# krlong014/PySolvers

Hardware: AMD Instinct MI355X
Metric: CG iterations/sec + SpMV GB/s vs HBM roofline, 5-pt Laplacian N=10M (higher is better)
Workload: dtype f64

## Files before the change

### include/psk_lab.h

```cpp
#ifndef PSK_LAB_H
#define PSK_LAB_H

#include "psk.h"

#ifdef __cplusplus
extern "C" {
#endif

int psk_lab_occupy_begin(int32_t wgs, int32_t lds_bytes, double seconds);
int psk_lab_occupy_end(int32_t *timed_out);
int psk_lab_dispatch_probe(int32_t nwg, int32_t lds_bytes, double usec, int64_t *rec_out);
int psk_lab_occupy_xcc(int32_t *counts);
int psk_lab_trisolve_workers(const psk_prec *M, int32_t which, int32_t *enrolled, int32_t *grid);
int psk_lab_trisolve_plan(int64_t n, const int32_t *rowptr, const int32_t *colidx, const double *vals, int32_t upper,
                          int32_t unit, const int32_t *nat, int32_t num_cus, int64_t syncfree_waves, int32_t *schedule,
                          double *est, int64_t *info);
int psk_lab_dist_plan(int64_t n_global, const int64_t *row_starts, int32_t P, int32_t rank, const int64_t *rowptr,
                      const int32_t *colidx, int32_t *lcol, int64_t *halo, int64_t *nhalo, int32_t *pack, int64_t *npack,
                      int64_t *peers, int32_t *npeers);
int psk_lab_amg_gs_pair(psk_prec *M, int32_t set, int32_t *levels_on, int32_t *levels_eligible);
int psk_lab_spmv_rotate(const psk_csr *A, const double *const *xs, double *const *ys, int32_t nbuf, int32_t reps,
                        int32_t dot, double *avg_ms);
int psk_lab_spmv_after_write(const psk_csr *A, double *x, double *y, const double *src, double *scratch,
                             int32_t target, int32_t reps, int32_t dot, double *avg_ms);
int psk_lab_cheby_ab(const psk_prec *M, const double *v, int32_t reps, double *fused_ms, double *pieces_ms);
int psk_lab_pcg_stagger(int32_t *blocks, int32_t *ring);
int psk_lab_pcg_staggers(const psk_csr *A, const psk_prec *M, int32_t *on);
int psk_lab_pcg_flush_schedule(int32_t S, int64_t nv, int64_t tile, int64_t k, int32_t in_spmv, int32_t *blk,
                               int64_t *first_last);
int psk_lab_pcg_flush(int64_t n, int64_t k, int32_t stag, double *x, const double *ring, const double *alphas);
#define PSK_LAB_SOLVER_PCG 0
#define PSK_LAB_SOLVER_GMRES 1
#define PSK_LAB_SOLVER_VCYCLE 2
#define PSK_LAB_SOLVER_BICGSTAB 3
#define PSK_LAB_SOLVER_MINRES 5
#define PSK_LAB_SOLVER_PCG_MULTI 6
#define PSK_LAB_LAYOUT_GEN 1
#define PSK_LAB_LAYOUT_OWN_X 2
#define PSK_LAB_LAYOUT_DEV_IO 4
int psk_lab_solver_layout(int32_t solver, int64_t n, int64_t ncols, int64_t maxiter, int64_t restart, int32_t flags,
                          int32_t P, int64_t *offsets, int32_t *count, int64_t *bytes);
int psk_lab_gmres_internals(const psk_csr *A, int64_t maxiter, int32_t restart, int32_t gen, int32_t cols, double *Q,
                            double *H, double *R, double *CS, double *g, double *y, double *state);
int psk_lab_gmres_prefill(psk_csr *A, int64_t maxiter, int32_t restart, int32_t gen, int32_t byte);
int psk_lab_pcg_internals(const psk_csr *A, int64_t maxiter, int32_t gen, int32_t own_x, double *r, double *ring,
                          double *Ap, double *u, double *x, double *alphas, double *udr, double *hist, double *sums,
                          double *state);
int psk_lab_pcg_prefill(psk_csr *A, int64_t maxiter, int32_t gen, int32_t own_x, int32_t byte);
int psk_lab_pcg_multi_internals(const psk_csr *A, int64_t maxiter, int32_t nrhs, double *alphas, double *udr, double *pap,
                                double *r, double *p, double *Ap, double *x, double *state);
int psk_lab_ilu0_timing(double *out);
int psk_lab_iluk_timing(double *out);
#ifdef __cplusplus
}
#endif

#endif
```

### pysolvers_amd/_native.py

```python
import atexit
import ctypes
import os
import sys

import numpy as np

_HERE = os.path.dirname(os.path.abspath(__file__))
LIB_PATH = os.environ.get("PSK_LIBRARY", os.path.join(_HERE, "_lib", "libpsk.so"))

PSK_OK = 0
PSK_ERR_ARG, PSK_ERR_HIP, PSK_ERR_RCCL, PSK_ERR_ALLOC, PSK_ERR_UNSUPPORTED = -1, -2, -3, -4, -5
ABI_VERSION = 4
PSK_CONVERGED, PSK_MAXITER, PSK_BREAKDOWN, PSK_TRUE_RESID_FAIL = 0, 1, 2, 3
PSK_EXIT_NONE, PSK_EXIT_TOLERANCE, PSK_EXIT_ARNOLDI_BREAKDOWN, PSK_EXIT_MAXITER, PSK_EXIT_DOT_BREAKDOWN = 0, 1, 2, 3, 4
PSK_HOST, PSK_DEVICE = 0, 1
PSK_VCYCLE_X0_GIVEN = 1
PSK_PREC_IDENTITY, PSK_PREC_JACOBI, PSK_PREC_ILU, PSK_PREC_AMG, PSK_PREC_DENSE, PSK_PREC_CHEBYSHEV = 0, 1, 2, 3, 4, 5
PSK_PREC_FSAI = 6
PSK_FSAI_ROW_CAP = 64
PSK_FSAI_WAVE_ONLY = 1
PSK_PREC_MCGS = 7
PSK_MCGS_MAX_COLORS = 64
PSK_MCGS_SYMMETRIC = 1
PSK_LAYOUT_CSR, PSK_LAYOUT_SLICED, PSK_LAYOUT_SLICED_WIDE, PSK_LAYOUT_SLICED_DICT, PSK_LAYOUT_DIAG = 0, 1, 2, 3, 4
# ... 45 lines not shown
    "psk_csr_download": (ctypes.c_int, [P, P, P, P]),
    "psk_csr_destroy": (ctypes.c_int, [P]),
    "psk_spmv": (ctypes.c_int, [P, P, P, I32]),
    "psk_spmv_timed": (ctypes.c_int, [P, P, P, I32, ctypes.POINTER(F64)]),
    "psk_dot": (ctypes.c_int, [I64, P, P, I32, ctypes.POINTER(F64)]),
    "psk_nrm2": (ctypes.c_int, [I64, P, I32, ctypes.POINTER(F64)]),
    "psk_axpy": (ctypes.c_int, [I64, F64, P, P, I32]),
    "psk_prec_create": (ctypes.c_int, [P, I32, PP]),
    "psk_prec_apply": (ctypes.c_int, [P, I64, P, P, I32]),
    "psk_prec_jacobi_uniform": (ctypes.c_int, [P, ctypes.POINTER(I32), ctypes.POINTER(ctypes.c_double)]),
    "psk_prec_create_ilu": (ctypes.c_int, [I64, P, P, P, P, P, P, P, P, PP]),
    "psk_prec_destroy": (ctypes.c_int, [P]),
    "psk_prec_create_trisolve": (ctypes.c_int, [I64, P, P, P, I32, P, P, P, I32, P, P, PP]),
    "psk_prec_create_amg": (ctypes.c_int, [I32, PP, PP, PP, PP, P, I32, I32, I32, F64, PP]),
    "psk_prec_create_dense_inverse": (ctypes.c_int, [P, I32, PP]),
    "psk_prec_create_chebyshev": (ctypes.c_int, [P, I32, F64, F64, PP]),
    "psk_prec_chebyshev_info": (ctypes.c_int, [P, ctypes.POINTER(I32), ctypes.POINTER(F64), ctypes.POINTER(F64), P]),
    "psk_prec_trisolve_schedule": (ctypes.c_int, [P, I32, I32, ctypes.POINTER(I32), ctypes.POINTER(I64),
                                                   ctypes.POINTER(I32), ctypes.POINTER(F64), ctypes.POINTER(F64)]),
    "psk_prec_trisolve_grid_info": (ctypes.c_int, [P, I32, ctypes.POINTER(I64)]),
    "psk_prec_trisolve_sweeps": (ctypes.c_int, [P, I32, I32, ctypes.POINTER(I32)]),
    "psk_trisolve_grid_plan": (ctypes.c_int, [I64, P, P, P, I32, ctypes.POINTER(I64)]),
    "psk_prec_info": (ctypes.c_int, [P, ctypes.POINTER(I32)] + [ctypes.POINTER(I64)] * 5),
    "psk_mm_info": (ctypes.c_int, [ctypes.c_char_p] + [ctypes.POINTER(I64)] * 3),
    "psk_mm_read": (ctypes.c_int, [ctypes.c_char_p, P, P, P, ctypes.POINTER(I64)]),
    "psk_csr_create_mm": (ctypes.c_int, [ctypes.c_char_p, PP]),
    "psk_sa_aggregate": (ctypes.c_int, [I64, P, P, P, F64, P, ctypes.POINTER(I64), P]),
    "psk_csr_matmat": (ctypes.c_int, [P, P, PP]),
    "psk_csr_transpose": (ctypes.c_int, [P, PP]),
    "psk_sa_prolongator": (ctypes.c_int, [P, P, I64, P, F64, I32, PP]),
    "psk_csr_ilu0": (ctypes.c_int, [P, PP]),
    "psk_prec_create_ilu0": (ctypes.c_int, [P, PP]),
    "psk_csr_iluk_pattern": (ctypes.c_int, [P, I32, PP, PP]),
    "psk_prec_create_iluk": (ctypes.c_int, [P, I32, PP]),
    "psk_csr_fsai": (ctypes.c_int, [P, P, I32, PP, ctypes.POINTER(I32)]),
    "psk_prec_create_fsai": (ctypes.c_int, [P, P, I32, PP]),
    "psk_prec_fsai_info": (ctypes.c_int, [P, ctypes.POINTER(I32), ctypes.POINTER(I64), ctypes.POINTER(I32)]),
    "psk_color_plan": (ctypes.c_int, [I64, P, P, P, ctypes.POINTER(I32)]),
    "psk_prec_create_mcgs": (ctypes.c_int, [P, I32, I32, PP]),
    "psk_prec_mcgs_info": (ctypes.c_int, [P, ctypes.POINTER(I32), ctypes.POINTER(I32), ctypes.POINTER(I32), P]),
    "psk_pcg": (ctypes.c_int, [P, P, P, P, ctypes.POINTER(PskCtl), ctypes.POINTER(PskResult), P, I32]),
    "psk_gmres": (ctypes.c_int, [P, P, P, P, ctypes.POINTER(PskCtl), ctypes.POINTER(PskResult), P, I32]),
    "psk_bicgstab": (ctypes.c_int, [P, P, P, P, ctypes.POINTER(PskCtl), ctypes.POINTER(PskResult), P, I32]),
    "psk_minres": (ctypes.c_int, [P, P, P, P, ctypes.POINTER(PskCtl), ctypes.POINTER(PskResult), P, I32]),
    "psk_idrs": (ctypes.c_int, [P, P, P, P, ctypes.POINTER(PskCtl), I32, ctypes.POINTER(PskResult), P, I32]),
    "psk_pcg_multi": (ctypes.c_int, [P, P, I32, P, P, ctypes.POINTER(PskCtl), ctypes.POINTER(PskResult), P, I32]),
    "psk_vcycle": (ctypes.c_int, [P, P, P, ctypes.POINTER(PskCtl), ctypes.POINTER(PskResult), P, I32, I32]),
    "psk_comm_unique_id": (ctypes.c_int, [P]),
    "psk_comm_init": (ctypes.c_int, [I32, I32, P, PP]),
    "psk_comm_destroy": (ctypes.c_int, [P]),
    "psk_comm_init_dry": (ctypes.c_int, [I32, I32, PP]),
    "psk_comm_init_host": (ctypes.c_int, [I32, I32, ctypes.c_char_p, PP]),
    "psk_comm_mailbox": (ctypes.c_int, [P, ctypes.c_char_p]),
    "psk_comm_mailbox_check": (ctypes.c_int, [P, I32]),
    "psk_csr_create_fd2d_dist": (ctypes.c_int, [F64, F64, I64, P, PP, ctypes.POINTER(I64),
                                                ctypes.POINTER(I64)]),
    "psk_csr_create_dist": (ctypes.c_int, [I64, P, P, P, P, P, PP]),
    "psk_csr_halo_cols": (ctypes.c_int, [P, P, ctypes.POINTER(I64)]),
    "psk_csr_halo_peers": (ctypes.c_int, [P, P, P, P, P, ctypes.POINTER(I32)]),
    "psk_csr_halo_pack": (ctypes.c_int, [P, P, P]),
    "psk_fd2d_dist_plan": (ctypes.c_int, [I64, I32, I32] + [ctypes.POINTER(I64)] * 5),
}


LAB_PATH = os.path.join(os.path.dirname(LIB_PATH), "libpsk_lab.so")
LAB_SIGNATURES = {
    "psk_lab_occupy_begin": (ctypes.c_int, [I32, I32, F64]),
    "psk_lab_occupy_end": (ctypes.c_int, [ctypes.POINTER(I32)]),
    "psk_lab_occupy_xcc": (ctypes.c_int, [ctypes.POINTER(I32)]),
    "psk_lab_dispatch_probe": (ctypes.c_int, [I32, I32, F64, P]),
    "psk_lab_trisolve_workers": (ctypes.c_int, [P, I32, ctypes.POINTER(I32), ctypes.POINTER(I32)]),
    "psk_lab_trisolve_plan": (ctypes.c_int, [I64, P, P, P, I32, I32, P, I32, I64, ctypes.POINTER(I32),
                                             ctypes.POINTER(F64), ctypes.POINTER(I64)]),
    "psk_lab_dist_plan": (ctypes.c_int, [I64, P, I32, I32, P, P, P, P, ctypes.POINTER(I64), P, ctypes.POINTER(I64), P,
                                         ctypes.POINTER(I32)]),
    "psk_lab_amg_gs_pair": (ctypes.c_int, [P, I32, ctypes.POINTER(I32), ctypes.POINTER(I32)]),
    "psk_lab_spmv_rotate": (ctypes.c_int, [P, ctypes.POINTER(P), ctypes.POINTER(P), I32, I32, I32, ctypes.POINTER(F64)]),
    "psk_lab_cheby_ab": (ctypes.c_int, [P, P, I32, ctypes.POINTER(F64), ctypes.POINTER(F64)]),
    "psk_lab_spmv_after_write": (ctypes.c_int, [P, P, P, P, P, I32, I32, I32, ctypes.POINTER(F64)]),
    "psk_lab_pcg_stagger": (ctypes.c_int, [ctypes.POINTER(I32), ctypes.POINTER(I32)]),
    "psk_lab_pcg_staggers": (ctypes.c_int, [P, P, ctypes.POINTER(I32)]),
    "psk_lab_pcg_flush_schedule": (ctypes.c_int, [I32, I64, I64, I64, I32, ctypes.POINTER(I32), ctypes.POINTER(I64)]),
    "psk_lab_pcg_flush": (ctypes.c_int, [I64, I64, I32, P, P, P]),
    "psk_lab_solver_layout": (ctypes.c_int, [I32, I64, I64, I64, I64, I32, I32, ctypes.POINTER(I64),
                                            ctypes.POINTER(I32), ctypes.POINTER(I64)]),
    "psk_lab_gmres_internals": (ctypes.c_int, [P, I64, I32, I32, I32, P, P, P, P, P, P, P]),
    "psk_lab_gmres_prefill": (ctypes.c_int, [P, I64, I32, I32, I32]),
    "psk_lab_pcg_internals": (ctypes.c_int, [P, I64, I32, I32, P, P, P, P, P, P, P, P, P, P]),
    "psk_lab_pcg_prefill": (ctypes.c_int, [P, I64, I32, I32, I32]),
    "psk_lab_pcg_multi_internals": (ctypes.c_int, [P, I64, I32, P, P, P, P, P, P, P, P]),
    "psk_lab_ilu0_timing": (ctypes.c_int, [ctypes.POINTER(F64)]),
    "psk_lab_iluk_timing": (ctypes.c_int, [ctypes.POINTER(F64)]),
}
_lab = None


def load_lab():
    global _lab
    if _lab is None:
        if not os.path.exists(LAB_PATH):
            raise ImportError("libpsk_lab.so not found at %s (make -C pysolvers_amd/csrc)" % LAB_PATH)
        lab = ctypes.CDLL(LAB_PATH)
        for name, (res, args) in LAB_SIGNATURES.items():
            fn = getattr(lab, name)
            fn.restype = res
            fn.argtypes = args
        _lab = lab
    return _lab


def prec_info(h):
    k = I32()
    v = [I64() for _ in range(5)]
    check(lib.psk_prec_info(h, ctypes.byref(k), *[ctypes.byref(x) for x in v]), "psk_prec_info")
    return dict(kind=k.value, n=v[0].value, nnz_l=v[1].value, nnz_u=v[2].value, levels_l=v[3].value,
                levels_u=v[4].value)


def handle_array(hs):
    arr = (ctypes.c_void_p * max(len(hs), 1))()
    for i, h in enumerate(hs):
        arr[i] = h.value if isinstance(h, ctypes.c_void_p) else h
    return ctypes.cast(arr, PP), arr


def fd2d_dist_plan(m, nranks, rank):
    v = [I64() for _ in range(5)]
    check(lib.psk_fd2d_dist_plan(m, nranks, rank, *[ctypes.byref(x) for x in v]), "psk_fd2d_dist_plan")
    return tuple(x.value for x in v)


class PskError(RuntimeError):

    def __init__(self, code, where, text):
        super().__init__("%s failed (%d): %s" % (where, code, text))
        self.code = code


def _pin_runtime():
    import importlib.util
    if os.environ.get("PSK_NO_TORCH") == "1":
        return
    if importlib.util.find_spec("torch") is not None:
        import torch


def _load():
    if not os.path.exists(LIB_PATH):
        raise ImportError("libpsk.so not found at %s — build it with `python -c 'import __graft_entry__ as "
                          "g; g.build()'` (make -C pysolvers_amd/csrc)" % LIB_PATH)
    _pin_runtime()
    lib = ctypes.CDLL(LIB_PATH, mode=ctypes.RTLD_GLOBAL)
    for name, (res, args) in SIGNATURES.items():
        fn = getattr(lib, name)
        fn.restype = res
        fn.argtypes = args
    if lib.psk_abi_version() != ABI_VERSION:
        raise ImportError("libpsk ABI version mismatch (library %d, bindings %d)" % (lib.psk_abi_version(), ABI_VERSION))
    return lib


PSK_SHUTDOWN_RESET_DEVICE = 1
lib = _load()
shut_down = False


# ... 33 lines not shown
```

### pysolvers_amd/csrc/lab.hip

```cpp
#include "amg.hpp"
#include "dist.hpp"
#include "trisolve.hpp"
#include "pcg_state.hpp"
#include "solve_loop.hpp"
#include "../../include/psk_lab.h"

#include <algorithm>
#include <chrono>
#include <string>

namespace psk {

__global__ __launch_bounds__(1024) void occupy_kernel(uint32_t *flag, int64_t *started, uint64_t ticks,
                                                      int32_t *timed_out) {
    extern __shared__ unsigned char occ_lds[];
    if (threadIdx.x == 0) {
        occ_lds[0] = 1;
        __hip_atomic_fetch_add(started, (int64_t)1, __ATOMIC_RELAXED, __HIP_MEMORY_SCOPE_SYSTEM);
        const uint32_t xcc = __builtin_amdgcn_s_getreg((3 << 11) | 20) & 7u;
        __hip_atomic_fetch_add(reinterpret_cast<uint32_t *>(timed_out) + 32 + xcc, 1u, __ATOMIC_RELAXED,
                               __HIP_MEMORY_SCOPE_AGENT);
    }
    const uint64_t t0 = __builtin_amdgcn_s_memrealtime();
    while (__hip_atomic_load(flag, __ATOMIC_RELAXED, __HIP_MEMORY_SCOPE_AGENT) == 0) {
// ... 232 lines not shown
        rc = launch_spmv(A, mode, xs[r % nbuf], ys[r % nbuf], nullptr, nullptr, pp, nullptr, c->stream);
    if (rc == PSK_OK && hipEventRecord(e1, c->stream) != hipSuccess) rc = fail(PSK_ERR_HIP, "event record");
    float ms = 0.f;
    if (rc == PSK_OK && hipEventSynchronize(e1) != hipSuccess) rc = fail(PSK_ERR_HIP, "event sync");
    if (rc == PSK_OK && hipEventElapsedTime(&ms, e0, e1) != hipSuccess) rc = fail(PSK_ERR_HIP, "event time");
    (void)hipStreamSynchronize(c->stream);
    (void)hipEventDestroy(e0);
    (void)hipEventDestroy(e1);
    part.release();
    if (rc == PSK_OK) *avg_ms = (double)ms / reps;
    return rc;
}

extern "C" int psk_lab_spmv_after_write(const psk_csr *A, double *x, double *y, const double *src, double *scratch,
                                        int32_t target, int32_t reps, int32_t dot, double *avg_ms) {
    using namespace psk;
    if (!A || !x || !y || !src || !scratch || reps < 1 || reps > 256 || !avg_ms)
        return fail(PSK_ERR_ARG, "psk_lab_spmv_after_write: bad arguments");
    if (A->comm || A->ncols != A->n) return fail(PSK_ERR_UNSUPPORTED, "psk_lab_spmv_after_write: square unsharded only");
    Context *c;
    PSK_TRY(ctx(&c));
    std::vector<hipEvent_t> ea((size_t)reps), eb((size_t)reps);
    for (int32_t r = 0; r < reps; ++r) {
        PSK_HIP(hipEventCreateWithFlags(&ea[(size_t)r], hipEventDisableSystemFence));
        PSK_HIP(hipEventCreateWithFlags(&eb[(size_t)r], hipEventDisableSystemFence));
    }
    const int mode = dot ? kSpmvDot : kSpmvPlain;
    DevBuf part;
    int rc = part.ensure(64);
    double *pp = dot ? part.as<double>() : nullptr;
    const int64_t n = A->n;
    const unsigned g = (unsigned)((n + 511) / 512);
    double *dst = target == 1 ? x : scratch;
    rc = launch_spmv(A, mode, x, y, nullptr, nullptr, pp, nullptr, c->stream);
    for (int32_t r = 0; r < reps && rc == PSK_OK; ++r) {
        if (target > 0) {
            hipLaunchKernelGGL(lab_copy_kernel, dim3(g), dim3(256), 0, c->stream, n, src, dst);
            if (hipGetLastError() != hipSuccess) rc = fail(PSK_ERR_HIP, "lab copy");
        }
        if (rc == PSK_OK)
            rc = launch_spmv(A, mode, x, y, nullptr, nullptr, pp, nullptr, c->stream, ea[(size_t)r], eb[(size_t)r]);
    }
    double tot = 0.0;
    if (rc == PSK_OK && hipStreamSynchronize(c->stream) != hipSuccess) rc = fail(PSK_ERR_HIP, "sync");
    for (int32_t r = 0; r < reps && rc == PSK_OK; ++r) {
        float ms = 0.f;
        if (hipEventElapsedTime(&ms, ea[(size_t)r], eb[(size_t)r]) != hipSuccess) rc = fail(PSK_ERR_HIP, "event time");
        tot += ms;
    }
    (void)hipStreamSynchronize(c->stream);
    for (int32_t r = 0; r < reps; ++r) {
        (void)hipEventDestroy(ea[(size_t)r]);
        (void)hipEventDestroy(eb[(size_t)r]);
    }
    part.release();
    if (rc == PSK_OK) *avg_ms = tot / reps;
    return rc;
}

extern "C" int psk_lab_pcg_stagger(int32_t *blocks, int32_t *ring) {
    if (blocks) *blocks = psk::kPcgStagger;
    if (ring) *ring = psk::kPcgDefer;
    return PSK_OK;
}

extern "C" int psk_lab_pcg_staggers(const psk_csr *A, const psk_prec *M, int32_t *on) {
    if (!A || !on) return psk::fail(PSK_ERR_ARG, "psk_lab_pcg_staggers: NULL argument");
    *on = psk::pcg_staggers(A, M) ? 1 : 0;
    return PSK_OK;
}

extern "C" int psk_lab_pcg_flush_schedule(int32_t S, int64_t nv, int64_t tile, int64_t k, int32_t in_spmv,
                                          int32_t *blk, int64_t *first_last) {
    using namespace psk;
    if (S < 1 || nv < 1 || tile < 0 || tile >= nv || k < 0 || !blk || !first_last)
        return fail(PSK_ERR_ARG, "psk_lab_pcg_flush_schedule: bad arguments");
    *blk = pcg_block_of_tile(tile, nv, S);
    const PcgPend pd = pcg_flush_pending(S, *blk, k, in_spmv != 0);
    first_last[0] = pd.first;
    first_last[1] = pd.last;
    return PSK_OK;
}

extern "C" int psk_lab_pcg_flush(int64_t n, int64_t k, int32_t stag, double *x, const double *ring,
                                 const double *alphas) {
    using namespace psk;
    if (n < 1 || k < 1 || !x || !ring || !alphas) return fail(PSK_ERR_ARG, "psk_lab_pcg_flush: bad arguments");
    if (stag && kPcgStagger == 0) return fail(PSK_ERR_UNSUPPORTED, "psk_lab_pcg_flush: built without the staggered flush");
    Context *c;
    PSK_TRY(ctx(&c));
    const size_t vec = ((size_t)n * 8 + 255) / 256 * 256, al = ((size_t)k * 8 + 255) / 256 * 256;
    DevBuf buf;
    PSK_TRY(buf.ensure((kPcgDefer + 1) * vec + al));
    char *d = buf.as<char>();
    double *dx = reinterpret_cast<double *>(d), *da = reinterpret_cast<double *>(d + (kPcgDefer + 1) * vec);
    PRing pr;
    for (int t = 0; t < kPcgDefer; ++t) pr.b[t] = reinterpret_cast<double *>(d + (size_t)(t + 1) * vec);
    int rc = PSK_OK;
    if (hipMemcpyAsync(dx, x, (size_t)n * 8, hipMemcpyHostToDevice, c->stream) != hipSuccess ||
        hipMemcpyAsync(da, alphas, (size_t)k * 8, hipMemcpyHostToDevice, c->stream) != hipSuccess)
        rc = fail(PSK_ERR_HIP, "psk_lab_pcg_flush: copy");
    for (int t = 0; t < kPcgDefer && rc == PSK_OK; ++t)
        if (hipMemcpyAsync(pr.b[t], ring + (size_t)t * (size_t)n, (size_t)n * 8, hipMemcpyHostToDevice, c->stream) != hipSuccess)
            rc = fail(PSK_ERR_HIP, "psk_lab_pcg_flush: copy");
    if (rc == PSK_OK) rc = launch_pcg_flush(n, dx, pr, da, k, stag != 0, c->stream);
    if (rc == PSK_OK && hipMemcpyAsync(x, dx, (size_t)n * 8, hipMemcpyDeviceToHost, c->stream) != hipSuccess)
        rc = fail(PSK_ERR_HIP, "psk_lab_pcg_flush: copy back");
    if (hipStreamSynchronize(c->stream) != hipSuccess && rc == PSK_OK) rc = fail(PSK_ERR_HIP, "psk_lab_pcg_flush: sync");
    buf.release();
    return rc;
}

extern "C" int psk_lab_pcg_internals(const psk_csr *A, int64_t maxiter, int32_t gen, int32_t own_x, double *r,
                                     double *ring, double *Ap, double *u, double *x, double *alphas, double *udr,
                                     double *hist, double *sums, double *state) {
    using namespace psk;
    if (!A) return fail(PSK_ERR_ARG, "psk_lab_pcg_internals: bad arguments");
    PcgView v;
    PSK_TRY(pcg_work_view(const_cast<psk_csr *>(A), maxiter, gen != 0, own_x != 0, false, &v));
    Context *c;
    PSK_TRY(ctx(&c));
    PSK_HIP(hipStreamSynchronize(c->stream));
    const size_t vec = (size_t)v.n * 8, vecc = (size_t)v.ncols * 8, it = (size_t)(maxiter + 1) * 8;
    if (r && vec) PSK_HIP(hipMemcpy(r, v.r, vec, hipMemcpyDeviceToHost));
    if (Ap && vec) PSK_HIP(hipMemcpy(Ap, v.Ap, vec, hipMemcpyDeviceToHost));
    if (u && v.u && vec) PSK_HIP(hipMemcpy(u, v.u, vec, hipMemcpyDeviceToHost));
    if (x && v.x && vec) PSK_HIP(hipMemcpy(x, v.x, vec, hipMemcpyDeviceToHost));
    for (int t = 0; t < kPcgDefer; ++t)
        if (ring && v.ring[t] && vecc)
            PSK_HIP(hipMemcpy(ring + (size_t)t * (size_t)v.ncols, v.ring[t], vecc, hipMemcpyDeviceToHost));
    if (alphas) PSK_HIP(hipMemcpy(alphas, v.alphas, it, hipMemcpyDeviceToHost));
    if (udr) PSK_HIP(hipMemcpy(udr, v.udr, it, hipMemcpyDeviceToHost));
    if (hist) PSK_HIP(hipMemcpy(hist, v.hist, it, hipMemcpyDeviceToHost));
    if (sums) {
        PSK_HIP(hipMemcpy(&sums[0], v.part1, 8, hipMemcpyDeviceToHost));
        PSK_HIP(hipMemcpy(&sums[1], v.part2, 8, hipMemcpyDeviceToHost));
        PSK_HIP(hipMemcpy(&sums[2], gen ? v.part3 : v.part2 + 1, 8, hipMemcpyDeviceToHost));
    }
    if (state) {
        PcgState hs;
        PSK_HIP(hipMemcpy(&hs, v.st, sizeof(hs), hipMemcpyDeviceToHost));
        state[0] = (double)hs.done;
        state[1] = (double)hs.brk_kind;
        state[2] = (double)hs.iters;
        state[3] = hs.resid;
        state[4] = hs.normB;
        state[5] = hs.tauNormB;
        state[6] = (double)hs.live;
        state[7] = (double)hs.x_written;
    }
    return PSK_OK;
}

extern "C" int psk_lab_pcg_prefill(psk_csr *A, int64_t maxiter, int32_t gen, int32_t own_x, int32_t byte) {
    using namespace psk;
    if (!A || byte < 0 || byte > 255) return fail(PSK_ERR_ARG, "psk_lab_pcg_prefill: bad arguments");
    Context *c;
    PSK_TRY(ctx(&c));
    PSK_HIP(hipStreamSynchronize(c->stream));
    PcgView v;
    PSK_TRY(pcg_work_view(A, maxiter, gen != 0, own_x != 0, true, &v));
    PSK_HIP(hipMemsetAsync(v.big, byte, v.big_bytes, c->stream));
    PSK_HIP(hipMemsetAsync(v.small, byte, v.small_bytes, c->stream));
    PSK_HIP(hipStreamSynchronize(c->stream));
    return PSK_OK;
}
// ... 95 lines not shown
```

### pysolvers_amd/csrc/pcg.hip

```cpp
#include "psk_internal.hpp"
#include "dist.hpp"
#include "pcg_state.hpp"

#include <cstdlib>

#include <climits>
#include <cmath>
#include <cstdio>
#include <type_traits>

namespace psk {

template <int JAC, bool FUSED>
__global__ __launch_bounds__(kBlock) void pcg_init_kernel(int64_t n, const double *__restrict__ b,
                                                          const double *__restrict__ dinv, double ds,
                                                          double *__restrict__ p, GridSum gs, PcgInitFin fin,
                                                          int64_t ntiles) {
    constexpr int TPW = 2;
    const int tid = threadIdx.x;
    int64_t tl[TPW];
    bool tv[TPW];
    double acc[TPW][2];
    uint32_t ticket[TPW];
#pragma unroll
    for (int q = 0; q < TPW; ++q) {
        const int64_t t = (int64_t)blockIdx.x * TPW + q;
        tv[q] = t < ntiles;
        tl[q] = tv[q] ? t : ntiles - 1;
        const int64_t row = tl[q] * kBlock + tid;
        const bool has = tv[q] && row < n;
        const double bi = has ? __builtin_nontemporal_load(b + row) : 0.0;
        const double d = JAC == 1 ? (has ? dinv[row] : 0.0) : ds;
        const double u = JAC ? d * bi : bi;
        if (has) p[row] = u;
        acc[q][0] = has ? bi * bi : 0.0;
        acc[q][1] = has ? u * bi : 0.0;
    }
    __shared__ GridSumTile<2> gsl[TPW];
#pragma unroll
    for (int q = 0; q < TPW; ++q) {
        ticket[q] = 0;
        if (tv[q] && gs.grp_log2 >= 0 && tid == 0)
            ticket[q] = gridsum_draw(gridsum_counter(gs, gridsum_group_of(tl[q], gs.grp_log2)));
    }
    if (tid < TPW) gsl[tid].cnt = 0;
    if (tid == 0 && blockIdx.x == 0 && (gs.nt + TPW - 1) / TPW != gridDim.x) atomicOr(gs.err, 2);
    __syncthreads();
    if (FUSED)
        gridsum_tiles_publish<TPW, 2>(gs, gsl, acc, ticket, tl, tv, fin);
    else
        gridsum_tiles_publish<TPW, 2>(gs, gsl, acc, ticket, tl, tv);
}

__global__ void pcg_init_finish_kernel(const double *g, int P, double tau, PcgState *st, double *udr,
                                       int64_t *hdone, int64_t hgen) {
    if (threadIdx.x == 0) pcg_init_state(rank_sum(g, P, 2, 0), rank_sum(g, P, 2, 1), tau, st, udr, hdone, hgen, 0);
}

template <int JAC, bool FIRST>
__global__ __launch_bounds__(kBlock) void pcg_update_kernel(
    int64_t n, double *__restrict__ r, const double *__restrict__ b, const double *__restrict__ Ap,
    const double *__restrict__ dinv, double ds, const double *__restrict__ pap, int nparts, GridSum gs, PcgState *st,
    const double *__restrict__ udr, int64_t k, TileMap tm) {
    const double udk = udr[k];
    const int32_t dn = st->done;
    const double pap0 = pap[0];
    __asm__ volatile("" ::"s"(dn), "s"(pap0), "s"(udk));
    if (dn) return;
    double pTAp = pap0;
    for (int q = 1; q < nparts; ++q) pTAp += pap[q];
    __shared__ double sh[2 * kWaves];
    if (pTAp == 0.0) {
        if (blockIdx.x == 0 && threadIdx.x == 0) {
            st->brk_kind = 2;
            st->iters = k;
            set_done(st, 2, k + 2);
        }
        return;
    }
    const double alpha = udk / pTAp;
    if (blockIdx.x == 0 && threadIdx.x == 0) st->live = k;
    const int64_t tile = tile_of_block(tm);
    const int64_t i = tile * kVecTile + 2 * threadIdx.x;
    const bool pair = i + 1 < n;
    uint32_t ticket = 0;
    double rr = 0.0, ur = 0.0;
    if (pair) {
        const dv2 ro = FIRST ? ld2nt(b + i) : ld2(r + i), a = ld2nt(Ap + i);
        dv2 d{ds, ds};
        if (JAC == 1) d = ld2(dinv + i);
        ticket = gridsum_ticket(gs, tile);
        dv2 rn;
        rn.x = ro.x - alpha * a.x;
        rn.y = ro.y - alpha * a.y;
        double u0 = rn.x, u1 = rn.y;
        if (JAC) {
            u0 = d.x * rn.x;
            u1 = d.y * rn.y;
        }
        st2(r + i, rn);
        rr = fma(rn.x, rn.x, rr);
        rr = fma(rn.y, rn.y, rr);
        ur = fma(u0, rn.x, ur);
        ur = fma(u1, rn.y, ur);
    } else if (i < n) {
        ticket = gridsum_ticket(gs, tile);
        const double rn = (FIRST ? b[i] : r[i]) - alpha * Ap[i];
        const double u0 = JAC == 2 ? ds * rn : JAC ? dinv[i] * rn : rn;
        r[i] = rn;
        rr = rn * rn;
        ur = u0 * rn;
    }
    block_sum2(rr, ur, sh);
    const double v[2] = {rr, ur};
    if (threadIdx.x >= 64) return;
    const bool lane0 = threadIdx.x == 0;
    if (gs.grp_log2 < 0) {
        if (lane0) {
            gridsum_put(gs.gslots + tile * 2, v[0]);
            gridsum_put(gs.gslots + tile * 2 + 1, v[1]);
        }
        gridsum_final_wave<2>(gs);
        return;
    }
    if (lane0) {
        gridsum_put(gs.slots + gridsum_slot(gs, tile) * 2, v[0]);
        gridsum_put(gs.slots + gridsum_slot(gs, tile) * 2 + 1, v[1]);
    }
    const uint32_t tk = __builtin_amdgcn_readfirstlane(ticket);
    const int64_t g = gridsum_group_of(tile, gs.grp_log2);
    int64_t base;
    const int64_t cnt = gridsum_members(gs, g, base);
    if (tk != (uint32_t)(cnt - 1)) return;
    double gr[2];
// ... 23 lines not shown
        rr += rrur[2 * q];
        ur += rrur[2 * q + 1];
    }
    const int64_t tile = tile_base + tile_of_block(tm);
    const double *pcur = pr.b[k % kPcgDefer];
    double *pnext = pr.b[(k + 1) % kPcgDefer];
    constexpr int S = kPcgStagger > 0 ? kPcgStagger : 1;
    const PcgPend pd = STAG ? pcg_flush_pending(S, pcg_block_of_tile(tile, (n + kVecTile - 1) / kVecTile, S), k, false)
                            : pcg_uniform_pending(k);
    const int q = (int)(k - pd.first);
    double alpha, beta;
    if (!pcg_direction_scalars(n, x, pcur, pTAp, rr, ur, udk, tauNB, st, udr, hist, k, maxiter, fail_on_maxiter,
                               alpha, beta, tile, &pr, alphas, pd))
        return;
    const bool flush = (!STAG && q == kPcgDefer - 1) || k == maxiter - 1;
    const bool x0 = pd.first == 0;
    if (tile == 0 && threadIdx.x == 0) {
        alphas[k] = alpha;
        if (flush) st->x_written = 1;
    }
    const int64_t i = tile * kVecTile + 2 * threadIdx.x;
    if (i + 1 < n) {
        const dv2 ro = ld2nt(r + i), po = ld2(pcur + i);
        dv2 d{ds, ds};
        if (JAC == 1) d = ld2nt(dinv + i);
        double u0 = ro.x, u1 = ro.y;
        if (JAC) {
            u0 = d.x * ro.x;
            u1 = d.y * ro.y;
        }
        if (flush) {
            dv2 xo{0.0, 0.0};
            if (!x0) xo = ld2nt(x + i);
            dv2 pp[kPcgDefer > 1 ? kPcgDefer - 1 : 1];
#pragma unroll
            for (int t = 1; t < kPcgDefer; ++t)
                if (t <= q) pp[t - 1] = ld2nt(pr.b[(k - t) % kPcgDefer] + i);
#pragma unroll
            for (int t = kPcgDefer - 1; t >= 1; --t)
                if (t <= q) {
                    const double a = alphas[k - t];
                    xo.x = xo.x + a * pp[t - 1].x;
                    xo.y = xo.y + a * pp[t - 1].y;
                }
            dv2 xn;
            xn.x = xo.x + alpha * po.x;
            xn.y = xo.y + alpha * po.y;
            st2nt(x + i, xn);
        }
        dv2 pn;
        pn.x = u0 + beta * po.x;
        pn.y = u1 + beta * po.y;
        st2(pnext + i, pn);
    } else if (i < n) {
        const double u0 = JAC == 2 ? ds * r[i] : JAC ? dinv[i] * r[i] : r[i];
        const double pi = pcur[i];
        if (flush) x[i] = pcg_catch_up(x0 ? 0.0 : x[i], &pr, pd.first, k, alphas, i) + alpha * pi;
        pnext[i] = u0 + beta * pi;
    }
}

template <bool STAG>
__global__ void pcg_flush_kernel(int64_t n, double *__restrict__ x, PRing pr, const double *__restrict__ alphas,
                                 int64_t k) {
    const int64_t i = (int64_t)blockIdx.x * kBlock + threadIdx.x;
    constexpr int S = kPcgStagger > 0 ? kPcgStagger : 1;
    const PcgPend pd = STAG ? pcg_flush_pending(S, pcg_block_of_tile(i / kVecTile, (n + kVecTile - 1) / kVecTile, S), k,
                                                false)
                            : pcg_uniform_pending(k);
    if (i < n && pd.first <= pd.last) x[i] = pcg_catch_up(pd.first == 0 ? 0.0 : x[i], &pr, pd.first, k, alphas, i);
}

int launch_pcg_flush(int64_t n, double *x, const PRing &pr, const double *alphas, int64_t k, bool stag, hipStream_t s) {
    if (n <= 0) return PSK_OK;
    const dim3 g((unsigned)((n + kBlock - 1) / kBlock));
    if (stag && kPcgStagger > 0) hipLaunchKernelGGL(pcg_flush_kernel<true>, g, dim3(kBlock), 0, s, n, x, pr, alphas, k);
    else hipLaunchKernelGGL(pcg_flush_kernel<false>, g, dim3(kBlock), 0, s, n, x, pr, alphas, k);
    PSK_HIP(hipGetLastError());
    return PSK_OK;
}

constexpr int kPcgStateWords = (int)(sizeof(PcgState) / 8);
constexpr int kPcgFinishWord = 8;
static_assert(sizeof(PcgState) % 8 == 0 && kPcgFinishWord + kPcgStateWords + 1 <= 64, "SolveKit::hmap words");
__global__ __launch_bounds__(kBlock) void pcg_finish_kernel(const PcgState *st, const uint32_t *cnt, const int32_t *err,
                                                            int64_t *hw) {
    constexpr int kPer = (kGridSumMaxGroups + kBlock) / kBlock;
    uint32_t v[kPer];
#pragma unroll
    for (int i = 0; i < kPer; ++i) {
        const int g = (int)threadIdx.x + i * kBlock;
        v[i] = cnt[(int64_t)(g < kGridSumMaxGroups ? g : kGridSumMaxGroups) * kGridSumCntStride];
    }
    uint32_t any = 0;
#pragma unroll
    for (int i = 0; i < kPer; ++i) any |= v[i];
    const bool bad = __syncthreads_or(any != 0);
    if (threadIdx.x < kPcgStateWords)
        __hip_atomic_store(hw + threadIdx.x, reinterpret_cast<const int64_t *>(st)[threadIdx.x], __ATOMIC_RELAXED,
                           __HIP_MEMORY_SCOPE_SYSTEM);
    if (threadIdx.x == 0)
        __hip_atomic_store(hw + kPcgStateWords, (int64_t)(*err | (bad ? 4 : 0)), __ATOMIC_RELAXED,
                           __HIP_MEMORY_SCOPE_SYSTEM);
}

__global__ __launch_bounds__(kBlock) void pcg_gen_init_kernel(int64_t n, const double *__restrict__ b,
                                                              double *__restrict__ x, double *__restrict__ r) {
    const int64_t i = (int64_t)blockIdx.x * kBlock + threadIdx.x;
    if (i < n) {
        r[i] = b[i];
        x[i] = 0.0;
    }
}

__global__ __launch_bounds__(kBlock) void pcg_gen_init2_kernel(int64_t n, const double *__restrict__ r,
                                                               const double *__restrict__ u, double *__restrict__ p,
                                                               GridSum gs, PcgInitFin fin) {
    __shared__ double sh[kWaves];
    const int64_t i = (int64_t)blockIdx.x * kVecTile + 2 * threadIdx.x;
    const uint32_t ticket = gridsum_ticket(gs);
    double bb = 0.0, ur = 0.0;
    for (int64_t j = i; j < i + 2 && j < n; ++j) {
        const double rj = r[j], uj = u[j];
        p[j] = uj;
        bb = fma(rj, rj, bb);
        ur = fma(uj, rj, ur);
    }
    const double v[2] = {block_sum(bb, sh), block_sum(ur, sh)};
    gridsum_publish<2>(gs, v, sh, ticket, fin);
}

__global__ __launch_bounds__(kBlock) void pcg_dot_kernel(int64_t n, const double *__restrict__ a,
                                                         const double *__restrict__ c, GridSum gs,
                                                         const PcgState *st) {
    if (st->done) return;
    __shared__ double sh[kWaves];
    const int64_t i = (int64_t)blockIdx.x * kVecTile + threadIdx.x;
    const uint32_t ticket = gridsum_ticket(gs);
    double acc = 0.0;
    if (i < n) acc = a[i] * c[i];
    if (i + kBlock < n) acc = fma(a[i + kBlock], c[i + kBlock], acc);
    const double v = block_sum(acc, sh);
    gridsum_publish<1>(gs, &v, sh, ticket);
}

__global__ __launch_bounds__(kBlock) void pcg_gen_direction_kernel(
    int64_t n, double *__restrict__ x, const double *__restrict__ u, double *__restrict__ p,
    const double *__restrict__ pap, const double *__restrict__ rrur, const double *__restrict__ ur_gen, PcgState *st,
    double *__restrict__ udr, double *__restrict__ hist, int64_t k, int64_t maxiter, int fail_on_maxiter) {
    if (st->live != k) return;
    double alpha, beta;
    if (!pcg_direction_scalars(n, x, p, *pap, rrur[0], *ur_gen, udr[k], st->tauNormB, st, udr, hist, k, maxiter,
                               fail_on_maxiter, alpha, beta, blockIdx.x))
        return;
    const int64_t i = (int64_t)blockIdx.x * kVecTile + 2 * threadIdx.x;
    for (int64_t j = i; j < i + 2 && j < n; ++j) {
        const double pj = p[j];
        x[j] = x[j] + alpha * pj;
        p[j] = u[j] + beta * pj;
    }
}


struct PcgWork {
    double *x, *r, *p, *Ap, *u, *part1, *part2, *part3, *udr, *hist;
    PRing pr;
    double *alphas;
    double *pinit;
    double *part1g, *part2g, *initg;
    PcgState *st;
};

static void pcg_layout(Carve &big, Carve &sm, int64_t n, int64_t ncols, int64_t maxiter, bool gen, bool own_x, int P,
                       PcgWork &w) {
    const size_t vec = (size_t)n * 8, vecc = (size_t)ncols * 8, it = (size_t)(maxiter + 1) * 8;
    w.r = big.take<double>(vec);
    w.Ap = big.take<double>(vec);
    w.x = own_x ? big.take<double>(vec) : nullptr;
    for (int t = 0; t < kPcgDefer; ++t) w.pr.b[t] = gen && t > 0 ? nullptr : big.take<double>(vecc);
    w.p = w.pr.b[0];
    w.u = gen ? big.take<double>(vec) : nullptr;
    w.st = sm.take<PcgState>(sizeof(PcgState));
    w.part1 = sm.take<double>(kMaxGrid * 8);
    w.part3 = sm.take<double>(kMaxGrid * 8);
    w.part2 = sm.take<double>(2 * kMaxGrid * 8);
    w.udr = sm.take<double>(it + 8);
    w.hist = sm.take<double>(it);
    w.alphas = sm.take<double>(it);
    w.pinit = sm.take<double>(256);
    w.part1g = P > 1 ? sm.take<double>((size_t)P * 8) : w.part1;
    w.part2g = P > 1 ? sm.take<double>((size_t)P * 16) : w.part2;
    w.initg = P > 1 ? sm.take<double>((size_t)P * 16) : w.pinit;
}

void pcg_layout_probe(int64_t n, int64_t ncols, int64_t maxiter, bool gen, bool own_x, int P, std::vector<int64_t> *log,
                      int64_t *bytes) {
    Carve big, sm;
    big.log = sm.log = log;
    PcgWork w;
    pcg_layout(big, sm, n, ncols, maxiter, gen, own_x, P, w);
    bytes[0] = big.off > 0 ? (int64_t)big.off : 256;
    bytes[1] = (int64_t)sm.off;
}

static int pcg_workspace(psk_csr *A, int64_t maxiter, bool gen, bool own_x, int P, PcgWork &w) {
    int64_t need[2];
    pcg_layout_probe(A->n, A->ncols, maxiter, gen, own_x, P, nullptr, need);
    PSK_TRY(A->ws.ensure((size_t)need[0]));
    PSK_TRY(A->ws_small.ensure((size_t)need[1]));
    Carve big{A->ws.as<char>()}, sm{A->ws_small.as<char>()};
    pcg_layout(big, sm, A->n, A->ncols, maxiter, gen, own_x, P, w);
    return PSK_OK;
// ... 27 lines not shown
    v->hist = w.hist;
    v->alphas = w.alphas;
    v->st = w.st;
    v->big = A->ws.p;
    v->big_bytes = (size_t)need[0];
    v->small = A->ws_small.p;
    v->small_bytes = (size_t)need[1];
    return PSK_OK;
}

bool pcg_staggers(const psk_csr *A, const psk_prec *M) {
    return kPcgStagger > 0 && !prec_is_general(M) && !A->comm && A->n > 0 && spmv_flush_eligible(A);
}

struct PcgPlan {
    int64_t n, maxiter;
    bool gen;
    bool sharded;
    bool dev_io;
    int P, jac;
    const double *dinv;
    double ds;
    int64_t nv, nsl;
    bool init_diag;
    bool stag;
    bool overlap;
    int64_t ov_lo, ov_hi;
    int C;
    psk_comm *mbc;
};

static int pcg_plan(const psk_csr *A, const psk_prec *M, const psk_ctl *ctl, int32_t loc, PcgPlan &pl) {
    pl.n = A->n;
    pl.maxiter = ctl->maxiter;
    pl.gen = prec_is_general(M);
    if (pl.gen && A->comm) return fail(PSK_ERR_UNSUPPORTED, "psk_pcg: ILU preconditioning of a sharded matrix");
    pl.sharded = A->comm != nullptr;
    pl.P = pl.sharded ? A->comm->nranks : 1;
    pl.dev_io = loc == PSK_DEVICE;
    pl.dinv = (M && M->kind == PSK_PREC_JACOBI) ? M->dinv : nullptr;
    pl.jac = !pl.dinv ? 0 : M->dinv_uniform ? 2 : 1;
    pl.ds = pl.jac == 2 ? M->dinv_value : 0.0;
    pl.nv = pl.n > 0 ? (pl.n + kVecTile - 1) / kVecTile : 1;
    if (pl.nv > INT32_MAX) return fail(PSK_ERR_UNSUPPORTED, "psk_pcg: vector too long for a one-shot grid");
    pl.nsl = pl.n > 0 ? (pl.n + kBlock - 1) / kBlock : 1;
    pl.init_diag = !pl.gen && !pl.sharded && (pl.jac == 0 || pl.jac == 2) && pcg_init_diag_eligible(A);
    pl.stag = pcg_staggers(A, M);
    pl.C = ctl->check_every > 0 ? ctl->check_every : (pl.n >= (1 << 20) ? 2 : 16);
    static const bool overlap_on = [] {
        const char *e = std::getenv("PSK_HALO_OVERLAP");
        return !(e && std::atoi(e) == 0);
    }();
    pl.ov_lo = 0;
    pl.ov_hi = pl.nv;
    pl.overlap = overlap_on && pl.sharded && !pl.gen && halo_split(A, kVecTile, pl.nv, pl.ov_lo, pl.ov_hi);
    pl.mbc = pl.sharded && A->comm->mb ? A->comm : nullptr;
    return PSK_OK;
}

struct PcgRun {
    psk_csr *A;
    const psk_prec *M;
    const psk_ctl *ctl;
    Context *c;
    SolveKit *kit;
    hipStream_t s, cs;
    PcgPlan pl;
    PcgWork w;
    GridSum gs2, gs3;
    const double *bd;
    bool halo_pending = false;
};

template <class F> static void pcg_dispatch(int jac, bool flag, F &&f) {
    auto on = [&](auto J) {
        if (flag) f(J, std::true_type{});
        else f(J, std::false_type{});
    };
    if (jac == 2) on(std::integral_constant<int, 2>{});
    else if (jac == 1) on(std::integral_constant<int, 1>{});
    else on(std::integral_constant<int, 0>{});
}

struct PcgTimers {
    SolveKit *kit;
    int S;
    bool skip0;
    int64_t tk[kTimedSlots];
    bool tgat[kTimedSlots], thalo[kTimedSlots];
    std::vector<float> spmv_ms;
    double gat_sum = 0.0, halo_sum = 0.0;
    int64_t gat_n = 0, halo_n = 0;
    PcgTimers(SolveKit *k, int stride, bool init_diag, int64_t maxiter) : kit(k), S(stride > 0 ? stride : 0), skip0(init_diag) {
        for (int i = 0; i < kTimedSlots; ++i) {
            tk[i] = -1;
            tgat[i] = thalo[i] = false;
        }
        if (S) spmv_ms.assign((size_t)maxiter, -1.0f);
    }
    int sample(hipEvent_t a, hipEvent_t b, float *ms) {
        PSK_HIP(hipEventSynchronize(b));
        PSK_HIP(hipEventElapsedTime(ms, a, b));
        return PSK_OK;
    }
    int harvest(int slot) {
        if (tk[slot] < 0) return PSK_OK;
        float ms = 0.f;
        PSK_TRY(sample(kit->ta[slot], kit->tb[slot], &ms));
        spmv_ms[(size_t)tk[slot]] = ms;
        tk[slot] = -1;
        if (tgat[slot]) {
            PSK_TRY(sample(kit->ga[slot], kit->gb[slot], &ms));
            gat_sum += ms;
            ++gat_n;
            tgat[slot] = false;
        }
        if (thalo[slot]) {
            PSK_TRY(sample(kit->ha[slot], kit->hb[slot], &ms));
            halo_sum += ms;
            ++halo_n;
            thalo[slot] = false;
        }
        return PSK_OK;
    }
    int begin(int64_t k, int *slot, bool *timed) {
        *timed = S > 0 && k % S == 0 && !(skip0 && k == 0);
        *slot = (int)((k / (S > 0 ? S : 1)) % kTimedSlots);
        if (*timed) {
            PSK_TRY(harvest(*slot));
            tk[*slot] = k;
        }
        return PSK_OK;
    }
    void finish(int64_t nk, psk_result *res) const {
        if (!S) return;
        double tot = 0.0;
        const int64_t cnt = nk < (int64_t)spmv_ms.size() ? nk : (int64_t)spmv_ms.size();
        int64_t nt = 0;
        for (int64_t i = 0; i < cnt; i += S)
            if (spmv_ms[(size_t)i] >= 0.0f) {
                tot += spmv_ms[(size_t)i];
                ++nt;
            }
        res->spmv_launches = nt;
        res->spmv_ms = nt > 0 ? tot / (double)nt : 0.0;
        res->gather_ms = gat_n > 0 ? gat_sum / (double)gat_n : 0.0;
        res->halo_ms = halo_n > 0 ? halo_sum / (double)halo_n : 0.0;
        res->comm_samples = gat_n;
    }
};

static int pcg_init(PcgRun &r, const StampPoll &poll, const double *b, int32_t loc) {
    const PcgPlan &pl = r.pl;
    PcgWork &w = r.w;
    const int64_t n = pl.n;
    hipStream_t s = r.s;
    GridSum gs0;
    if (!pl.init_diag) PSK_TRY(gridsum_prepare(r.c, pl.gen ? pl.nv : pl.nsl, 2, w.pinit, &gs0));
    PSK_TRY(gridsum_prepare(r.c, pl.nv, 2, w.part2, &r.gs2));
    PSK_TRY(gridsum_prepare(r.c, pl.nv, 1, w.part3, &r.gs3));
    const PcgInitFin fin{r.ctl->tau, w.st, w.udr, poll.hdone(), poll.hgen(), pl.gen ? 1 : 0, 0};
    r.bd = b;
    if (!pl.dev_io) {
        PSK_TRY(to_device_vec(b, loc, n, pl.gen ? w.Ap : w.r, s));
        r.bd = pl.gen ? w.Ap : w.r;
    }
    const uint64_t seq0 = pl.mbc ? mbox_next(pl.mbc, &gs0) : 0;
    PSK_HIP(hipEventRecord(r.kit->ev0, s));
    if (pl.gen) {
        const unsigned nb = (unsigned)((n + kBlock - 1) / kBlock);
        if (n > 0) hipLaunchKernelGGL(pcg_gen_init_kernel, dim3(nb), dim3(kBlock), 0, s, n, r.bd, w.x, w.r);
        PSK_TRY(prec_apply_dev(r.M, n, w.r, w.u, s));
        hipLaunchKernelGGL(pcg_gen_init2_kernel, dim3((unsigned)pl.nv), dim3(kBlock), 0, s, n, w.r, w.u, w.p, gs0, fin);
    } else if (pl.init_diag) {
        PcgInitFin fin3 = fin;
        fin3.off = 1;
        PSK_TRY(launch_pcg_init_diag(r.A, r.bd, pl.jac == 2 ? pl.ds : 1.0, w.p, w.Ap, w.part1, fin3, s));
    } else {
        const dim3 gi((unsigned)((pl.nsl + 1) / 2));
        pcg_dispatch(pl.jac, !pl.sharded, [&](auto J, auto FUSED) {
            hipLaunchKernelGGL((pcg_init_kernel<decltype(J)::value, decltype(FUSED)::value>), gi, dim3(kBlock), 0, s, n,
                               r.bd, pl.dinv, pl.ds, w.p, gs0, fin, pl.nsl);
        });
    }
    PSK_HIP(hipGetLastError());
    if (pl.sharded) {
        if (pl.mbc) PSK_TRY(mbox_gather(pl.mbc, seq0, 2, w.initg, nullptr, s));
        else PSK_TRY(allgather(r.A, w.pinit, w.initg, 2, s));
        hipLaunchKernelGGL(pcg_init_finish_kernel, dim3(1), dim3(64), 0, s, w.initg, pl.P, r.ctl->tau, w.st, w.udr,
                           poll.hdone(), poll.hgen());
        PSK_HIP(hipGetLastError());
    }
    return PSK_OK;
}

static void pcg_k3(PcgRun &r, int64_t k, int64_t t0, int64_t t1) {
    if (t1 <= t0) return;
    const PcgPlan &pl = r.pl;
    PcgWork &w = r.w;
    const dim3 g3((unsigned)(t1 - t0));
    const TileMap tm3 = tile_map_for(t1 - t0, false);
    pcg_dispatch(pl.jac, pl.stag, [&](auto J, auto SG) {
        hipLaunchKernelGGL((pcg_direction_kernel<decltype(J)::value, decltype(SG)::value && (kPcgStagger > 0)>), g3,
                           dim3(kBlock), 0, r.s, pl.n, w.x, w.r, w.pr, pl.dinv, pl.ds, w.part1g, w.part2g, pl.P, w.st, w.udr,
                           w.hist, w.alphas, k, pl.maxiter, r.ctl->fail_on_maxiter, t0, tm3);
    });
}

static int pcg_iteration(PcgRun &r, PcgTimers &tm, int64_t k) {
    const PcgPlan &pl = r.pl;
    PcgWork &w = r.w;
    psk_csr *A = r.A;
    SolveKit *kit = r.kit;
    hipStream_t s = r.s;
    const int64_t n = pl.n;
    double *pk = pl.gen ? w.p : w.pr.b[k % kPcgDefer];
    double *pn = pl.gen ? w.p : w.pr.b[(k + 1) % kPcgDefer];
    int slot;
    bool timed;
    PSK_TRY(tm.begin(k, &slot, &timed));
    if (r.halo_pending) {
        PSK_HIP(hipStreamWaitEvent(s, kit->ev_b, 0));
        r.halo_pending = false;
    } else if (A->comm) {
        const bool th = timed && !A->comm->dry && !A->peers.empty();
        if (th) PSK_HIP(hipEventRecord(kit->ha[slot], s));
        PSK_TRY(halo_exchange(A, pk, s));
        if (th) {
            PSK_HIP(hipEventRecord(kit->hb[slot], s));
            tm.thalo[slot] = true;
        }
    }
    uint64_t seq1 = 0;
    const SpmvFlush fl{w.x, w.alphas, w.pr, k, pl.nv, 0, 0, 0, 0};
    if (!(pl.init_diag && k == 0))
        PSK_TRY(launch_spmv(A, kSpmvDot, pk, w.Ap, nullptr, nullptr, w.part1, &w.st->done, s, timed ? kit->ta[slot] : nullptr,
                            timed ? kit->tb[slot] : nullptr, 0, pl.mbc ? &seq1 : nullptr, pl.stag && k >= 1 ? &fl : nullptr));
    const TileMap tm2 = tile_map_for(pl.nv, false);
    if (pl.sharded) {
        hipEvent_t g0 = timed ? kit->ga[slot] : nullptr, g1 = timed ? kit->gb[slot] : nullptr;
        if (pl.mbc) {
            PSK_TRY(mbox_gather(pl.mbc, seq1, 1, w.part1g, &w.st->done, s, g0, g1));
        } else {
            if (g0) PSK_HIP(hipEventRecord(g0, s));
            PSK_TRY(allgather(A, w.part1, w.part1g, 1, s));
            if (g1) PSK_HIP(hipEventRecord(g1, s));
        }
        if (timed) tm.tgat[slot] = true;
    }
    GridSum gs2k = r.gs2;
    const uint64_t seq2 = pl.mbc ? mbox_next(pl.mbc, &gs2k) : 0;
    const dim3 gk((unsigned)pl.nv);
    pcg_dispatch(pl.jac, k == 0 && !pl.gen && pl.dev_io, [&](auto J, auto FIRST) {
        hipLaunchKernelGGL((pcg_update_kernel<decltype(J)::value, decltype(FIRST)::value>), gk, dim3(kBlock), 0, s, n, w.r,
                           r.bd, w.Ap, pl.dinv, pl.ds, w.part1g, pl.P, gs2k, w.st, w.udr, k, tm2);
    });
    if (pl.sharded) {
        if (pl.mbc) PSK_TRY(mbox_gather(pl.mbc, seq2, 2, w.part2g, &w.st->done, s));
        else PSK_TRY(allgather(A, w.part2, w.part2g, 2, s));
    }
    if (pl.gen) {
        PSK_TRY(prec_apply_dev(r.M, n, w.r, w.u, s));
        hipLaunchKernelGGL(pcg_dot_kernel, gk, dim3(kBlock), 0, s, n, w.u, w.r, r.gs3, w.st);
        hipLaunchKernelGGL(pcg_gen_direction_kernel, gk, dim3(kBlock), 0, s, n, w.x, w.u, w.p, w.part1, w.part2,
                           w.part3, w.st, w.udr, w.hist, k, pl.maxiter, r.ctl->fail_on_maxiter);
    } else if (pl.overlap && k + 1 < pl.maxiter) {
        pcg_k3(r, k, 0, pl.ov_lo);
        pcg_k3(r, k, pl.ov_hi, pl.nv);
        PSK_TRY(halo_exchange_async(A, pn, s, r.cs, kit->ev_a, kit->ev_b, timed ? kit->ha[slot] : nullptr,
                                    timed ? kit->hb[slot] : nullptr));
        if (timed) tm.thalo[slot] = true;
        pcg_k3(r, k, pl.ov_lo, pl.ov_hi);
        r.halo_pending = true;
    } else {
        pcg_k3(r, k, 0, pl.nv);
    }
    PSK_HIP(hipGetLastError());
    return PSK_OK;
}

static int pcg_finish(PcgRun &r, PcgTimers &tm, PcgState *hs, psk_result *res) {
    SolveKit *kit = r.kit;
    if (r.halo_pending) PSK_HIP(hipStreamWaitEvent(r.s, kit->ev_b, 0));
    r.halo_pending = false;
    PSK_HIP(hipEventRecord(kit->ev1, r.s));
    int64_t *hw = kit->hmap + kPcgFinishWord;
    hipLaunchKernelGGL(pcg_finish_kernel, dim3(1), dim3(kBlock), 0, r.s, r.w.st, r.c->gs_cnt, r.c->gs_err, hw);
    PSK_HIP(hipGetLastError());
    PSK_HIP(hipStreamSynchronize(r.s));
    std::memcpy(hs, hw, sizeof(PcgState));
    PSK_TRY(gridsum_check_result(r.c, (int32_t)hw[kPcgStateWords]));
    if (r.pl.gen) PSK_TRY(prec_check_error(r.M, r.s));
    for (int i = 0; i < kTimedSlots; ++i) PSK_TRY(tm.harvest(i));
    res->loop_ms = loop_ms(kit);
    return PSK_OK;
}

static int pcg_report(const PcgState &hs, const PcgPlan &pl, int64_t launched, const psk_ctl *ctl, const PcgWork &w,
                      hipStream_t s, psk_result *res, double *hist, double *xout, int32_t loc, int64_t *nk) {
    const int64_t n = pl.n, maxiter = pl.maxiter;
    res->norm_b = hs.normB;
    int64_t nhist = 0;
    if (hs.done == 1) {
        res->status = PSK_CONVERGED;
        res->success = 1;
        res->iters = hs.iters;
        res->resid = hs.resid;
        res->exit = hs.normB == 0.0 ? PSK_EXIT_NONE : hs.resid <= hs.tauNormB ? PSK_EXIT_TOLERANCE : PSK_EXIT_MAXITER;
        *nk = nhist = hs.normB == 0.0 ? 0 : hs.iters;
    } else if (hs.done == 2) {
        res->status = PSK_BREAKDOWN;
        res->exit = PSK_EXIT_DOT_BREAKDOWN;
        res->success = 0;
        res->iters = hs.iters;
        res->resid = NAN;
        result_msg(res, hs.brk_kind == 1 ? "breakdown dot(u,r)==0" : "breakdown dot(p, Ap)==0");
        *nk = hs.brk_kind == 1 ? 0 : hs.iters + 1;
        nhist = hs.brk_kind == 1 ? 0 : hs.iters;
    } else {
        res->status = PSK_MAXITER;
        res->exit = PSK_EXIT_MAXITER;
        res->success = 0;
        res->iters = maxiter > 0 ? maxiter - 1 : 0;
        result_msg(res, "failure to converge");
        *nk = nhist = launched;
    }
    const int64_t nh = nhist < maxiter ? nhist : maxiter;
    if (hist && nh > 0) PSK_HIP(hipMemcpy(hist, w.hist, (size_t)nh * 8, hipMemcpyDeviceToHost));
    res->hist_len = nh;
    res->resid_recursive = nh > 0 ? hs.last_hist : hs.normB;
    if (res->status == PSK_MAXITER) res->resid = maxiter > 0 ? res->resid_recursive : hs.normB;
    bool x_written = hs.x_written != 0;
    bool more = !pl.dev_io;
    if (!pl.gen && hs.done == 2 && hs.brk_kind != 1 && n > 0) {
        bool pending = false;
        const int nblk = pl.stag ? kPcgStagger : 1;
        for (int b = 0; b < nblk; ++b) {
            if (pl.stag && (int64_t)b * pcg_block_tiles(pl.nv, kPcgStagger) >= pl.nv) continue;
            const PcgPend pd = pl.stag ? pcg_flush_pending(kPcgStagger, b, hs.iters, false) : pcg_uniform_pending(hs.iters);
            pending = pending || pd.first <= pd.last;
            x_written = x_written || pd.first > 0;
        }
        if (pending) {
            PSK_TRY(launch_pcg_flush(n, w.x, w.pr, w.alphas, (int64_t)hs.iters, pl.stag, s));
            x_written = true;
            more = true;
        }
    }
    if (!x_written && n > 0) {
        PSK_HIP(hipMemsetAsync(w.x, 0, (size_t)n * 8, s));
        more = true;
    }
    if (!pl.dev_io) PSK_TRY(from_device_vec(w.x, loc, n, xout, s));
    if (more) PSK_HIP(hipStreamSynchronize(s));
    return PSK_OK;
}

static int pcg_solve(PcgRun &r, const double *b, double *xout, psk_result *res, double *hist, int32_t loc) {
    const PcgPlan &pl = r.pl;
    PSK_TRY(pcg_workspace(r.A, pl.maxiter, pl.gen, !pl.dev_io, pl.P, r.w));
    if (pl.dev_io) r.w.x = xout;
    PSK_TRY(solve_kit(r.c, r.ctl->time_kernels > 0, &r.kit));
    if (pl.overlap) PSK_TRY(comm_stream(r.c, &r.cs));
    StampPoll poll(r.kit);
    PcgTimers tm(r.kit, r.ctl->time_kernels, pl.init_diag, pl.maxiter);
    PSK_TRY(pcg_init(r, poll, b, loc));
    int64_t launched = 0, nk = 0;
    for (int64_t k = 0; k < pl.maxiter; ++k) {
        bool stop;
        PSK_TRY(poll.step<2>(k, pl.C, r.s, &stop));
        if (stop) break;
        PSK_TRY(pcg_iteration(r, tm, k));
        launched = k + 1;
    }
    PcgState hs;
    PSK_TRY(pcg_finish(r, tm, &hs, res));
    PSK_TRY(pcg_report(hs, pl, launched, r.ctl, r.w, r.s, res, hist, xout, loc, &nk));
    tm.finish(nk, res);
    return PSK_OK;
}

}

using namespace psk;

extern "C" int psk_pcg(const psk_csr *Ac, const psk_prec *M, const double *b, double *xout,
                       const psk_ctl *ctl, psk_result *res, double *hist, int32_t loc) {
    if (!Ac || !b || !xout || !ctl || !res) return fail(PSK_ERR_ARG, "psk_pcg: NULL argument");
    if (ctl->maxiter < 0) return fail(PSK_ERR_ARG, "psk_pcg: maxiter < 0");
    if (M && M->n != Ac->n) return fail(PSK_ERR_ARG, "psk_pcg: preconditioner size mismatch");
    if (!Ac->comm && Ac->ncols != Ac->n) return fail(PSK_ERR_ARG, "psk_pcg: matrix must be square");
    PcgRun r{};
    r.A = const_cast<psk_csr *>(Ac);
    r.M = M;
    r.ctl = ctl;
    PSK_TRY(ctx(&r.c));
    std::lock_guard<std::mutex> solve_lock(r.c->solve_mu);
    r.s = r.c->stream;
    std::memset(res, 0, sizeof(*res));
    PSK_TRY(pcg_plan(Ac, M, ctl, loc, r.pl));
    const int rc = pcg_solve(r, b, xout, res, hist, loc);
    if (rc != PSK_OK) {
        if (r.halo_pending) (void)hipStreamWaitEvent(r.s, r.kit->ev_b, 0);
        (void)hipStreamSynchronize(r.s);
    }
    return rc;
}
```

### pysolvers_amd/csrc/pcg_state.hpp

```cpp
#pragma once
#include "psk_internal.hpp"
#include "solve_loop.hpp"

namespace psk {

struct PcgState {
    int32_t done;
    int32_t brk_kind;
    int64_t iters;
    double resid;
    double normB;
    double tauNormB;
    int64_t live;
    int64_t *hdone;
    int64_t hgen;
    double last_hist;
    int32_t x_written;
    int32_t pad;
};

__device__ __forceinline__ void set_done(PcgState *st, int32_t v, int64_t stamp) {
    st->done = v;
    if (st->hdone) done_stamp_store(st->hdone, st->hgen, stamp);
}
// ... 45 lines not shown
struct PRing {
    double *b[kPcgDefer];
};
__host__ __device__ inline int pcg_pending(int64_t k) { return (int)(k % kPcgDefer); }

#ifndef PSK_PCG_STAGGER
#define PSK_PCG_STAGGER 1
#endif
#define PSK_PCG_STAGGER_ON (PSK_PCG_STAGGER && PSK_PCG_DEFER >= 2)
constexpr int kPcgStagger = PSK_PCG_STAGGER_ON ? kPcgDefer - 1 : 0;
static_assert(kPcgStagger >= 0 && kPcgStagger < kPcgDefer, "SpMV k reads p_{k-S} after K3 k-1 wrote p_k: S < ring");

struct PcgPend {
    int64_t first, last;
};
__host__ __device__ inline int64_t pcg_block_tiles(int64_t nv, int S) { return (nv + S - 1) / S; }
__host__ __device__ inline int pcg_block_of_tile(int64_t tile, int64_t nv, int S) {
    return (int)(tile / pcg_block_tiles(nv, S));
}
__host__ __device__ inline PcgPend pcg_flush_pending(int S, int blk, int64_t k, bool in_spmv) {
    const int64_t kk = in_spmv ? k - 1 : k;
    int64_t f = kk - ((kk - blk) % S + S) % S;
    if (f < 1) f = 0;
    return PcgPend{f, k - 1};
}
__host__ __device__ inline PcgPend pcg_uniform_pending(int64_t k) { return PcgPend{k - pcg_pending(k), k - 1}; }

__device__ __forceinline__ double pcg_catch_up(double xj, const PRing *pr, int64_t first, int64_t k,
                                               const double *__restrict__ alphas, int64_t j) {
    for (int64_t t = first; t < k; ++t) xj = xj + alphas[t] * pr->b[t % kPcgDefer][j];
    return xj;
}

struct SpmvFlush {
    double *x;
    const double *alphas;
    PRing pr;
    int64_t k;
    int64_t nv;
    uint32_t ost, ofl;
    uint32_t nfl;
    uint32_t mul;
};

__device__ inline bool pcg_direction_scalars(int64_t n, double *__restrict__ x, const double *__restrict__ p,
                                             double pTAp, double rr, double ur, double udk, double tauNB,
                                             PcgState *st, double *__restrict__ udr, double *__restrict__ hist, int64_t k,
                                             int64_t maxiter, int fail_on_maxiter, double &alpha, double &beta,
                                             int64_t tile, const PRing *pr = nullptr,
                                             const double *__restrict__ alphas = nullptr,
                                             PcgPend pd = PcgPend{0, -1}) {
    alpha = udk / pTAp;
    const double normR = sqrt(rr);
    if (tile == 0 && threadIdx.x == 0) {
        hist[k] = normR;
        st->last_hist = normR;
    }
    if (normR <= tauNB || (!fail_on_maxiter && k == maxiter - 1)) {
        const int64_t i = tile * kVecTile + 2 * threadIdx.x;
        const bool x0 = pr && pd.first == 0;
        for (int64_t j = i; j < i + 2 && j < n; ++j) {
            double xj = x0 ? 0.0 : x[j];
            if (pr) xj = pcg_catch_up(xj, pr, pd.first, k, alphas, j);
            x[j] = xj + alpha * p[j];
        }
        if (tile == 0 && threadIdx.x == 0) {
            st->iters = k + 1;
            st->resid = normR;
            st->x_written = 1;
            set_done(st, 1, k + 2);
        }
        return false;
    }
    beta = ur / udk;
    if (tile == 0 && threadIdx.x == 0) udr[k + 1] = ur;
    return true;
}

bool pcg_init_diag_eligible(const psk_csr *A);
bool spmv_flush_eligible(const psk_csr *A);
bool pcg_staggers(const psk_csr *A, const psk_prec *M);
int launch_pcg_flush(int64_t n, double *x, const PRing &pr, const double *alphas, int64_t k, bool stag, hipStream_t s);
int launch_pcg_init_diag(const psk_csr *A, const double *b, double xs, double *p, double *Ap, double *out3,
                         const PcgInitFin &fin, hipStream_t s);

struct PcgView {
    int64_t n, ncols;
    double *r, *Ap, *x, *u, *ring[kPcgDefer];
    double *part1, *part2, *part3, *udr, *hist, *alphas;
    const PcgState *st;
    void *big, *small;
    size_t big_bytes, small_bytes;
};
int pcg_work_view(psk_csr *A, int64_t maxiter, bool gen, bool own_x, bool grow, PcgView *v);

}
```

### pysolvers_amd/csrc/psk_internal.hpp

```cpp
#pragma once

#include <hip/hip_runtime.h>

#include <cstdint>
#include <cstring>
#include <mutex>
#include <string>
#include <vector>

#include "../../include/psk.h"

namespace psk {

constexpr int kBlock = 256;
constexpr int kWaves = kBlock / 64;
constexpr int kChunk = 1280;
constexpr int kMaxGrid = 2048;
constexpr int kVecTile = 2 * kBlock;
constexpr int64_t kMaxNnz = (int64_t)INT32_MAX - kChunk - kBlock;

void set_error(int code, const std::string &msg);
int fail(int code, const std::string &msg);
const char *hip_err_str(hipError_t e);

#define PSK_HIP(call)                                                                         \
    do {                                                                                      \
        hipError_t _e = (call);                                                               \
        if (_e != hipSuccess)                                                                 \
            return ::psk::fail(PSK_ERR_HIP, std::string(#call) + ": " + hipGetErrorString(_e)); \
    } while (0)

#define PSK_TRY(call)              \
    do {                           \
        int _rc = (call);          \
        if (_rc != PSK_OK) return _rc; \
    } while (0)

constexpr int kPollSlots = 4;
constexpr int kTimedSlots = 64;
struct SolveKit {
    bool ready = false;
    uint64_t solve_gen = 0;
    int64_t *hmap = nullptr;
    void *hstage = nullptr;
    hipEvent_t ev0 = nullptr, ev1 = nullptr;
    hipEvent_t fev[kPollSlots] = {};
    hipEvent_t ev_a = nullptr, ev_b = nullptr;
    bool timed_ready = false;
    hipEvent_t ta[kTimedSlots] = {}, tb[kTimedSlots] = {};
    hipEvent_t ga[kTimedSlots] = {}, gb[kTimedSlots] = {}, ha[kTimedSlots] = {}, hb[kTimedSlots] = {};
};
constexpr size_t kStageBytes = 4096;
struct Context {
    int device = -1;
    hipStream_t stream = nullptr;
    int num_cus = 256;
    int grid_cap = kMaxGrid;
    uint64_t *gs_slots = nullptr;
    int64_t gs_cap = 0;
    uint64_t *gs_gslots = nullptr;
    uint32_t *gs_cnt = nullptr;
    std::vector<uint64_t *> gs_retired;
    int32_t *gs_err = nullptr;
    hipStream_t comm_stream = nullptr;
    SolveKit kit;
    std::mutex solve_mu;
};
int ctx(Context **out);
int comm_stream(Context *c, hipStream_t *out);
int solve_kit(Context *c, bool timed, SolveKit **out);
bool lib_shut_down();

struct DevBuf {
    void *p = nullptr;
    size_t bytes = 0;
    int ensure(size_t need);
    void release();
    template <class T> T *as() const { return static_cast<T *>(p); }
};
struct DevBufRelease {
    DevBuf &b;
    ~DevBufRelease() { b.release(); }
};

struct HaloPeer {
    int rank;
    int64_t send_count;
    int64_t recv_count;
    int64_t recv_offset;
    bool packed;
    int64_t send_begin;
    int64_t pack_off;
};

struct DenseInverse;
struct Chebyshev;
struct Fsai;
struct Mcgs;
constexpr int64_t kDenseMaxN = 32768;

struct ShmComm;
struct Mailbox;
}

struct psk_comm;

struct psk_csr {
    int64_t n = 0;
    int64_t ncols = 0;
    int64_t nnz = 0;
    int tile_rows = 256;
    int32_t *rowptr = nullptr;
    int32_t *colidx = nullptr;
    double *vals = nullptr;
    int device = 0;
    int64_t *sl_off = nullptr;
    int64_t *sl_woff = nullptr;
    int8_t *sl_fmt = nullptr;
    int32_t *sl_col = nullptr;
    int32_t *sl_pcol = nullptr;
    double *sl_val = nullptr;
    double *sl_dict = nullptr;
    int32_t sl_dict_n = 0;
    int32_t sl_uniform_w = 0;
    int32_t sl_compact = 0;
    int64_t sl_slots = 0, sl_packed_slots = 0, sl_stream_bytes = 0;
    uint8_t *dg_mask = nullptr;
    int32_t dg_K = 0, dg_jd = -1;
    int32_t dg_d[8] = {};
    double dg_v[8] = {};
    int64_t dg_lo = 0, dg_hi = 0;
    psk_comm *comm = nullptr;
    int64_t n_global = 0, row_begin = 0, row_end = 0;
    std::vector<psk::HaloPeer> peers;
// ... 90 lines not shown
    psk::Mcgs *mcgs = nullptr;
};

namespace psk {


__device__ __forceinline__ double wave_sum(double v) {
#pragma unroll
    for (int o = 32; o > 0; o >>= 1) v += __shfl_xor(v, o, 64);
    return v;
}

template <int CTRL>
__device__ __forceinline__ double dpp_f64(double v) {
    const int lo = __builtin_amdgcn_update_dpp(0, __double2loint(v), CTRL, 0xF, 0xF, false);
    const int hi = __builtin_amdgcn_update_dpp(0, __double2hiint(v), CTRL, 0xF, 0xF, false);
    return __hiloint2double(hi, lo);
}

__device__ __forceinline__ double wave_total(double v) {
    v += dpp_f64<0xB1>(v);
    v += dpp_f64<0x4E>(v);
    v += dpp_f64<0x124>(v);
    v += dpp_f64<0x128>(v);
    auto lane = [](double x, int l) {
        return __hiloint2double(__builtin_amdgcn_readlane(__double2hiint(x), l),
                                __builtin_amdgcn_readlane(__double2loint(x), l));
    };
    return ((lane(v, 0) + lane(v, 16)) + lane(v, 32)) + lane(v, 48);
}

__device__ __forceinline__ double block_sum(double v, double *sh) {
    v = wave_sum(v);
    const int w = threadIdx.x >> 6;
    __syncthreads();
    if ((threadIdx.x & 63) == 0) sh[w] = v;
    __syncthreads();
    double r = sh[0];
#pragma unroll
    for (int i = 1; i < kWaves; ++i) r += sh[i];
    return r;
}

__device__ __forceinline__ void block_sum2(double &a, double &b, double *sh) {
#pragma unroll
    for (int o = 32; o > 0; o >>= 1) {
        a += __shfl_xor(a, o, 64);
        b += __shfl_xor(b, o, 64);
    }
    const int w = threadIdx.x >> 6;
    __syncthreads();
    if ((threadIdx.x & 63) == 0) {
        sh[2 * w] = a;
        sh[2 * w + 1] = b;
    }
    __syncthreads();
    double ra = sh[0], rb = sh[1];
#pragma unroll
    for (int i = 1; i < kWaves; ++i) {
        ra += sh[2 * i];
        rb += sh[2 * i + 1];
    }
    a = ra;
    b = rb;
}

__device__ __forceinline__ double rank_sum(const double *g, int nparts, int W, int c) {
    double s = g[c];
    for (int q = 1; q < nparts; ++q) s += g[q * W + c];
    return s;
}

__device__ __forceinline__ double reduce_partials(const double *part, int np, int stride, double *sh) {
    double v = 0.0;
    for (int i = threadIdx.x; i < np; i += kBlock) v += part[(int64_t)i * stride];
    return block_sum(v, sh);
}

__device__ __forceinline__ void done_stamp_store(int64_t *hdone, int64_t hgen, int64_t stamp) {
    __hip_atomic_store(hdone, hgen | stamp, __ATOMIC_RELAXED, __HIP_MEMORY_SCOPE_SYSTEM);
    __threadfence_system();
}

constexpr int kGridSumLLog = 8;
constexpr int64_t kGridSumL = (int64_t)1 << kGridSumLLog;
constexpr int kGridSumCntStride = 64;
constexpr uint64_t kGridSumSentinel = 0x7FF0000000000001ull;
constexpr int kGridSumMaxW = 8;
constexpr int64_t kGridSumMaxGroups = kMaxGrid;
constexpr uint64_t kGridSumWaitTicks = (uint64_t)1 << 27;

struct GridSum {
    uint64_t *slots;
    uint64_t *gslots;
    uint32_t *cnt;
    double *out;
    int64_t nt;
    int64_t ngroups;
    int32_t grp_log2;
    int32_t *err;
    uint64_t *mb;
    int64_t mb_q;
    int32_t mb_P;
};

template <int W>
__device__ __forceinline__ void gridsum_mail(const GridSum &gs, const double *r) {
    if (!gs.mb) return;
    for (int q = 0; q < gs.mb_P; ++q)
#pragma unroll
        for (int c = 0; c < W; ++c)
            __hip_atomic_store(gs.mb + q * gs.mb_q + c, (uint64_t)__double_as_longlong(r[c]), __ATOMIC_RELAXED,
                               __HIP_MEMORY_SCOPE_SYSTEM);
}

inline int32_t gridsum_grp_log2(int64_t nt) {
    if (nt <= kBlock) return -1;
    int32_t l = 0;
    while (((int64_t)1 << (2 * l)) < nt) ++l;
    auto ng = [&](int32_t g) { return ((nt + (kGridSumL << g) - 1) >> (kGridSumLLog + g)) * kGridSumL; };
    while (ng(l) > kGridSumMaxGroups) ++l;
    return l;
}
inline int64_t gridsum_ngroups(int64_t nt, int32_t gl) {
    if (gl < 0) return nt;
    const int64_t S = kGridSumL << gl, full = nt / S, tail = nt - full * S;
    return full * kGridSumL + (tail < kGridSumL ? tail : kGridSumL);
}

__device__ __forceinline__ int64_t gridsum_group_of(int64_t t, int32_t gl) {
    return ((t >> (kGridSumLLog + gl)) << kGridSumLLog) | (t & (kGridSumL - 1));
}
__device__ __forceinline__ int64_t gridsum_members(const GridSum &gs, int64_t g, int64_t &base) {
    const int32_t gl = gs.grp_log2;
    const int64_t sb = g >> kGridSumLLog, l = g & (kGridSumL - 1), S = kGridSumL << gl;
    base = sb * S + l;
    const int64_t t = gs.nt - sb * S;
    return t >= S ? ((int64_t)1 << gl) : (t - l + kGridSumL - 1) >> kGridSumLLog;
}

__device__ __forceinline__ void gridsum_put(uint64_t *sl, double v) {
    __hip_atomic_store(sl, (uint64_t)__double_as_longlong(v), __ATOMIC_RELAXED, __HIP_MEMORY_SCOPE_AGENT);
}
__device__ __forceinline__ uint32_t gridsum_draw(uint32_t *c) {
    return __hip_atomic_fetch_add(c, 1u, __ATOMIC_RELAXED, __HIP_MEMORY_SCOPE_AGENT);
}
__device__ __forceinline__ void gridsum_reset(uint32_t *c) {
    __hip_atomic_store(c, 0u, __ATOMIC_RELAXED, __HIP_MEMORY_SCOPE_AGENT);
}
__device__ __forceinline__ uint32_t *gridsum_counter(const GridSum &gs, int64_t g) {
    return gs.cnt + g * kGridSumCntStride;
}
__device__ __forceinline__ uint64_t gridsum_wait(const uint64_t *sl, int32_t *err) {
    uint64_t bits = __hip_atomic_load(sl, __ATOMIC_RELAXED, __HIP_MEMORY_SCOPE_AGENT);
    if (bits != kGridSumSentinel) return bits;
    const uint64_t t0 = __builtin_amdgcn_s_memrealtime();
    while ((bits = __hip_atomic_load(sl, __ATOMIC_RELAXED, __HIP_MEMORY_SCOPE_AGENT)) == kGridSumSentinel) {
        if (__builtin_amdgcn_s_memrealtime() - t0 > kGridSumWaitTicks) {
            atomicOr(err, 1);
            return 0x7FF8000000000000ull;
        }
        __builtin_amdgcn_s_sleep(1);
    }
    return bits;
}

// ... 288 lines not shown
__device__ __forceinline__ dv2 ld2(const double *p) { return *reinterpret_cast<const dv2 *>(p); }
__device__ __forceinline__ dv2 ld2nt(const double *p) {
    return __builtin_nontemporal_load(reinterpret_cast<const dv2 *>(p));
}
__device__ __forceinline__ void st2(double *p, dv2 v) { *reinterpret_cast<dv2 *>(p) = v; }
__device__ __forceinline__ void st2nt(double *p, dv2 v) { __builtin_nontemporal_store(v, reinterpret_cast<dv2 *>(p)); }

__device__ __forceinline__ void block_range(int64_t ntiles, int64_t &t0, int64_t &t1) {
    const int64_t g = gridDim.x, b = blockIdx.x;
    t0 = ntiles * b / g;
    t1 = ntiles * (b + 1) / g;
}

inline int grid_for_rows(const Context *c, int64_t rows, int per_tile) {
    int64_t tiles = (rows + per_tile - 1) / per_tile;
    if (tiles < 1) tiles = 1;
    return (int)(tiles < c->grid_cap ? tiles : c->grid_cap);
}

int to_device_vec(const double *src, int32_t loc, int64_t n, double *dst, hipStream_t s);
int from_device_vec(const double *src, int32_t loc, int64_t n, double *dst, hipStream_t s);

enum SpmvMode : int {
    kSpmvPlain = 0,
    kSpmvDot = 1,
    kSpmvJacobiDot = 2,
    kSpmvPlainDot = 3,
    kSpmvResid = 4,
    kSpmvAdd = 5,
};
int fd2d_fill(psk_csr *A, int64_t m, double a, double b, int64_t row_begin, int64_t row_end,
              int64_t halo_lo_start, hipStream_t s);
int prec_apply_dev(const psk_prec *M, int64_t n, const double *v, double *out, hipStream_t s);
int ilu_apply(const psk_prec *M, const double *v, double *out, hipStream_t s);
int ilu_apply_add(const psk_prec *M, const double *v, double *x, hipStream_t s);
int ilu_check_error(const psk_prec *M, hipStream_t s);
int dense_apply(const psk_prec *M, const double *v, double *out, hipStream_t s);
int dense_check_error(const psk_prec *M, hipStream_t s);
void dense_free(DenseInverse *d);
int cheby_apply(const psk_prec *M, const double *v, double *out, hipStream_t s);
void cheby_free(Chebyshev *ch);
int cheby_ab(const psk_prec *M, const double *v, int reps, double *fused_ms, double *pieces_ms);
int fsai_apply(const psk_prec *M, const double *v, double *out, hipStream_t s);
void fsai_free(Fsai *f);
int64_t fsai_nnz(const Fsai *f);
int mcgs_apply(const psk_prec *M, const double *v, double *out, hipStream_t s);
void mcgs_free(Mcgs *m);
int64_t mcgs_nnz(const Mcgs *m);
int64_t mcgs_ncolors(const Mcgs *m);
struct Ilu0Timing {
    double sort_ms = 0.0, levels_ms = 0.0, numeric_ms = 0.0, split_ms = 0.0, plan_ms = 0.0;
    int64_t levels = 0;
    int width = 0;
};
const Ilu0Timing &ilu0_last_timing();
struct IlukTiming {
    double symbolic_ms = 0.0;
    int32_t level = 0, rounds = 0, wide_rounds = 0;
    int width = 0;
    int64_t nnz_a = 0, nnz_p = 0;
};
const IlukTiming &iluk_last_timing();
inline bool prec_is_general(const psk_prec *M) {
    return M && (M->kind == PSK_PREC_ILU || M->kind == PSK_PREC_AMG || M->kind == PSK_PREC_DENSE ||
                 M->kind == PSK_PREC_CHEBYSHEV || M->kind == PSK_PREC_FSAI || M->kind == PSK_PREC_MCGS);
}
inline const double *prec_jacobi_dinv(const psk_prec *M) {
    return (M && M->kind == PSK_PREC_JACOBI) ? M->dinv : nullptr;
}
int prec_check_error(const psk_prec *M, hipStream_t s);
int tile_rows_for(int64_t n, int64_t nnz);
int csr_choose_layout(psk_csr *A, hipStream_t s);
int csr_new_device(int64_t n, int64_t ncols, int64_t nnz, psk_csr **out);
int csr_finish_device(psk_csr *A, hipStream_t s);
void csr_discard(psk_csr *A);
constexpr int kScanTile = 4 * kBlock;
inline int64_t exscan_tiles(int64_t n) { return (n + kScanTile - 1) / kScanTile; }
int exscan_total(int64_t n, const int32_t *counts, int64_t *tiles, int64_t nt, hipStream_t s, int64_t *total);
int exscan_finish(int64_t n, const int32_t *counts, const int64_t *tiles, int64_t nt, int32_t *rowptr, hipStream_t s);
struct SpmvFlush;
int launch_spmv(const psk_csr *A, int mode, const double *x, double *y, const double *aux_d,
                const double *aux_q, double *partial, const int32_t *done_flag, hipStream_t s,
                hipEvent_t ev0 = nullptr, hipEvent_t ev1 = nullptr, int rev = 0, uint64_t *mail_seq = nullptr,
                const SpmvFlush *flush = nullptr);

}
```

### pysolvers_amd/csrc/runtime.hip

```cpp
#include "psk_internal.hpp"
#include "dist.hpp"

#include <mutex>
#include <atomic>

namespace psk {

static thread_local std::string g_last_error;

void set_error(int code, const std::string &msg) {
    g_last_error = "psk error " + std::to_string(code) + ": " + msg;
}

int fail(int code, const std::string &msg) {
    set_error(code, msg);
    return code;
}

static std::mutex g_ctx_mu;
static Context g_ctx[64];
static std::atomic<bool> g_shut{false};

bool lib_shut_down() { return g_shut.load(std::memory_order_acquire); }
static std::atomic<int> g_live_rccl{0};
void rccl_comm_count(int delta) { g_live_rccl += delta; }

int solve_kit(Context *c, bool timed, SolveKit **out) {
    SolveKit &k = c->kit;
    if (!k.ready) {
        PSK_HIP(hipHostMalloc(&k.hmap, 64 * sizeof(int64_t), hipHostMallocCoherent));
        std::memset(k.hmap, 0, 64 * sizeof(int64_t));
        PSK_HIP(hipHostMalloc(&k.hstage, kStageBytes, hipHostMallocDefault));
        PSK_HIP(hipEventCreate(&k.ev0));
        PSK_HIP(hipEventCreate(&k.ev1));
        for (auto &e : k.fev) PSK_HIP(hipEventCreateWithFlags(&e, hipEventDisableTiming));
        PSK_HIP(hipEventCreateWithFlags(&k.ev_a, hipEventDisableTiming));
        PSK_HIP(hipEventCreateWithFlags(&k.ev_b, hipEventDisableTiming));
        k.ready = true;
    }
    if (timed && !k.timed_ready) {
        for (int i = 0; i < kTimedSlots; ++i) {
            PSK_HIP(hipEventCreateWithFlags(&k.ta[i], hipEventDisableSystemFence));
            PSK_HIP(hipEventCreateWithFlags(&k.tb[i], hipEventDisableSystemFence));
            for (hipEvent_t *e : {&k.ga[i], &k.gb[i], &k.ha[i], &k.hb[i]})
                PSK_HIP(hipEventCreateWithFlags(e, hipEventDisableSystemFence));
        }
        k.timed_ready = true;
    }
    *out = &k;
    return PSK_OK;
}

int comm_stream(Context *c, hipStream_t *out) {
    std::lock_guard<std::mutex> lk(g_ctx_mu);
    if (c->comm_stream == nullptr) PSK_HIP(hipStreamCreateWithFlags(&c->comm_stream, hipStreamNonBlocking));
    *out = c->comm_stream;
    return PSK_OK;
}

int ctx(Context **out) {
    if (g_shut) return fail(PSK_ERR_ARG, "libpsk was shut down (psk_shutdown)");
    int dev = 0;
    PSK_HIP(hipGetDevice(&dev));
    if (dev < 0 || dev >= 64) return fail(PSK_ERR_ARG, "device index out of range");
    std::lock_guard<std::mutex> lk(g_ctx_mu);
    if (g_shut) return fail(PSK_ERR_ARG, "libpsk was shut down (psk_shutdown)");
    Context &c = g_ctx[dev];
    if (c.stream == nullptr) {
        PSK_HIP(hipStreamCreateWithFlags(&c.stream, hipStreamNonBlocking));
        hipDeviceProp_t prop;
        PSK_HIP(hipGetDeviceProperties(&prop, dev));
        c.device = dev;
        c.num_cus = prop.multiProcessorCount;
        int cap = c.num_cus * 4;
        c.grid_cap = cap < kMaxGrid ? cap : kMaxGrid;
        c.grid_cap -= c.grid_cap % 8;
        if (c.grid_cap < 8) c.grid_cap = 8;
    }
    *out = &c;
    return PSK_OK;
}

int DevBuf::ensure(size_t need) {
    if (need <= bytes && p != nullptr) return PSK_OK;
    if (p) {
        hipError_t e = hipFree(p);
        p = nullptr;
        bytes = 0;
        if (e != hipSuccess) return fail(PSK_ERR_HIP, std::string("hipFree: ") + hipGetErrorString(e));
    }
    if (need == 0) return PSK_OK;
    hipError_t e = hipMalloc(&p, need);
    if (e != hipSuccess) {
        p = nullptr;
        return fail(PSK_ERR_ALLOC, "hipMalloc(" + std::to_string(need) + "): " + hipGetErrorString(e));
    }
    bytes = need;
    return PSK_OK;
}

void DevBuf::release() {
    if (p) (void)hipFree(p);
    p = nullptr;
    bytes = 0;
}

__global__ void gridsum_arm_kernel(uint64_t *slots, int64_t n) {
    const int64_t i = (int64_t)blockIdx.x * blockDim.x + threadIdx.x;
    if (i < n) slots[i] = kGridSumSentinel;
}

// ... 91 lines not shown
    return PSK_OK;
}

int from_device_vec(const double *src, int32_t loc, int64_t n, double *dst, hipStream_t s) {
    if (n <= 0) return PSK_OK;
    PSK_HIP(hipMemcpyAsync(dst, src, (size_t)n * sizeof(double),
                           loc == PSK_HOST ? hipMemcpyDeviceToHost : hipMemcpyDeviceToDevice, s));
    return PSK_OK;
}

}

using namespace psk;

extern "C" {

int psk_abi_version(void) { return PSK_ABI_VERSION; }

const char *psk_last_error(void) { return g_last_error.c_str(); }

int psk_device_count(int32_t *n) {
    if (!n) return fail(PSK_ERR_ARG, "n is NULL");
    int c = 0;
    hipError_t e = hipGetDeviceCount(&c);
    if (e != hipSuccess) c = 0;
    *n = c;
    return PSK_OK;
}

int psk_set_device(int32_t dev) {
    PSK_HIP(hipSetDevice(dev));
    return PSK_OK;
}

int psk_synchronize(void) {
    Context *c;
    PSK_TRY(ctx(&c));
    PSK_HIP(hipStreamSynchronize(c->stream));
    return PSK_OK;
}

int psk_dmalloc(int64_t bytes, void **dptr) {
    if (!dptr || bytes < 0) return fail(PSK_ERR_ARG, "psk_dmalloc: bad arguments");
    *dptr = nullptr;
    if (bytes == 0) return PSK_OK;
    hipError_t e = hipMalloc(dptr, (size_t)bytes);
    if (e != hipSuccess) return fail(PSK_ERR_ALLOC, std::string("hipMalloc: ") + hipGetErrorString(e));
    return PSK_OK;
}

int psk_dfree(void *dptr) {
    if (g_shut) return PSK_OK;
    if (dptr) PSK_HIP(hipFree(dptr));
    return PSK_OK;
}

int psk_shutdown(void) { return psk_shutdown_ex(0); }

int psk_shutdown_ex(int32_t flags) {
    {
        std::lock_guard<std::mutex> lk(g_ctx_mu);
        if (g_shut.exchange(true, std::memory_order_acq_rel)) return PSK_OK;
    }
    int rc = PSK_OK;
    int cur = 0;
    (void)hipGetDevice(&cur);
    for (int d = 0; d < 64; ++d) {
        Context &c = g_ctx[d];
        if (c.stream == nullptr) continue;
        if (hipSetDevice(d) != hipSuccess) continue;
        std::lock_guard<std::mutex> solve_lk(c.solve_mu);
        if (hipStreamSynchronize(c.stream) != hipSuccess && rc == PSK_OK) rc = fail(PSK_ERR_HIP, "psk_shutdown: sync");
        if (c.comm_stream) (void)hipStreamSynchronize(c.comm_stream);
        SolveKit &k = c.kit;
        if (k.ready) {
            (void)hipEventDestroy(k.ev0);
            (void)hipEventDestroy(k.ev1);
            for (auto e : k.fev) (void)hipEventDestroy(e);
            (void)hipEventDestroy(k.ev_a);
            (void)hipEventDestroy(k.ev_b);
            (void)hipHostFree(k.hmap);
            (void)hipHostFree(k.hstage);
        }
        if (k.timed_ready)
            for (int i = 0; i < kTimedSlots; ++i) {
                (void)hipEventDestroy(k.ta[i]);
                (void)hipEventDestroy(k.tb[i]);
                for (hipEvent_t e : {k.ga[i], k.gb[i], k.ha[i], k.hb[i]}) (void)hipEventDestroy(e);
            }
        k = SolveKit{};
        for (uint64_t *p : c.gs_retired) (void)hipFree(p);
        c.gs_retired.clear();
        void *bufs[] = {c.gs_slots, c.gs_gslots, c.gs_cnt, c.gs_err};
        for (void *p : bufs)
            if (p) (void)hipFree(p);
        c.gs_slots = nullptr;
        c.gs_gslots = nullptr;
        c.gs_cnt = nullptr;
        c.gs_err = nullptr;
        c.gs_cap = 0;
        if (c.comm_stream) (void)hipStreamDestroy(c.comm_stream);
        (void)hipStreamDestroy(c.stream);
        c.comm_stream = nullptr;
        c.stream = nullptr;
        if ((flags & PSK_SHUTDOWN_RESET_DEVICE) && g_live_rccl.load() == 0) (void)hipDeviceReset();
    }
    (void)hipSetDevice(cur);
    return rc;
}

int psk_h2d(void *dst, const void *src, int64_t bytes) {
    Context *c;
    PSK_TRY(ctx(&c));
    if (bytes <= 0) return PSK_OK;
    PSK_HIP(hipMemcpyAsync(dst, src, (size_t)bytes, hipMemcpyHostToDevice, c->stream));
    PSK_HIP(hipStreamSynchronize(c->stream));
    return PSK_OK;
}

int psk_d2h(void *dst, const void *src, int64_t bytes) {
    Context *c;
    PSK_TRY(ctx(&c));
    if (bytes <= 0) return PSK_OK;
    PSK_HIP(hipMemcpyAsync(dst, src, (size_t)bytes, hipMemcpyDeviceToHost, c->stream));
    PSK_HIP(hipStreamSynchronize(c->stream));
    return PSK_OK;
}

int psk_dmemset0(void *dst, int64_t bytes) {
    Context *c;
    PSK_TRY(ctx(&c));
    if (bytes <= 0) return PSK_OK;
    PSK_HIP(hipMemsetAsync(dst, 0, (size_t)bytes, c->stream));
    PSK_HIP(hipStreamSynchronize(c->stream));
    return PSK_OK;
}

}
```

### pysolvers_amd/csrc/spmv.hip

```cpp
#include "spmv.hpp"
#include "dist.hpp"
#include "pcg_state.hpp"

#include <cstdlib>

namespace psk {

int csr_choose_layout(psk_csr *A, hipStream_t s) {
    const char *e = std::getenv("PSK_SPMV_LAYOUT");
    if (e && std::strcmp(e, "csr") == 0) return PSK_OK;
    const char *de = std::getenv("PSK_SPMV_DIAG");
    const bool diag_env = e && std::strcmp(e, "diag") == 0;
    if ((!e || diag_env) && !(de && std::atoi(de) == 0)) {
        PSK_TRY(diag_build(A, s, false));
        if (A->dg_mask) return PSK_OK;
    }
    if (diag_env) e = nullptr;
    const bool wide = e && std::strcmp(e, "sliced_wide") == 0;
    const bool plain = e && std::strcmp(e, "sliced") == 0;
    const bool force = e && (plain || wide || std::strcmp(e, "sliced_dict") == 0);
    int rc = sliced_build(A, s, force, !wide, !wide && !plain, false);
    if (rc != PSK_OK) sliced_free(A);
    return rc;
}

int tile_rows_for(int64_t n, int64_t nnz) {
    const double avg = n > 0 ? (double)nnz / (double)n : 1.0;
    int r = kBlock;
    while (r > 32 && avg * r > kChunk) r >>= 1;
    return r;
}

__global__ void spmv_empty_dot_kernel(GridSum gs, const int32_t *done) {
    if (threadIdx.x != 0 || (done && *done)) return;
    const double z[1] = {0.0};
    gs.out[0] = 0.0;
    gridsum_mail<1>(gs, z);
}

int launch_spmv(const psk_csr *A, int mode, const double *x, double *y, const double *aux_d,
                const double *aux_q, double *partial, const int32_t *done_flag, hipStream_t s, hipEvent_t ev0,
                hipEvent_t ev1, int rev, uint64_t *mail_seq, const SpmvFlush *flush) {
    Context *c;
    PSK_TRY(ctx(&c));
    if (flush && (mode != kSpmvDot || !partial || !spmv_flush_eligible(A) || kPcgStagger == 0 || flush->k < 1))
        return fail(PSK_ERR_ARG, "launch_spmv: the flush role needs the PCG loop's launch in the diagonal pair layout");
    const bool sliced = A->sl_off != nullptr || A->dg_mask != nullptr;
    const int64_t nwg = sliced ? (A->n + kSlice - 1) / kSlice : (A->n + A->tile_rows - 1) / A->tile_rows;
    GridSum gs{nullptr, nullptr, nullptr, nullptr, 0, 0, -1, nullptr, nullptr, 0, 0};
    if (partial && nwg > 0) PSK_TRY(gridsum_prepare(c, nwg, 1, partial, &gs));
    if (partial && nwg == 0) gs.out = partial;
    if (mail_seq) {
        if (!partial || !A->comm || !A->comm->mb) return fail(PSK_ERR_ARG, "launch_spmv: mailbox without a dot");
        *mail_seq = mbox_next(A->comm, &gs);
    }
    if (A->n == 0) {
        if (partial) {
            hipLaunchKernelGGL(spmv_empty_dot_kernel, dim3(1), dim3(64), 0, s, gs, done_flag);
            PSK_HIP(hipGetLastError());
        }
        return PSK_OK;
    }
    const SpmvLaunch L{x, y, aux_d, aux_q, gs, done_flag, s, ev0, ev1, rev != 0, nwg};
    if (A->dg_mask) return launch_spmv_diag(A, mode, L, flush);
    if (A->sl_off) return launch_spmv_sliced(A, mode, L);
    return launch_spmv_csr(A, mode, L);
}

}

using namespace psk;

extern "C" {

int psk_spmv(const psk_csr *Ac, const double *x, double *y, int32_t loc) {
    if (!Ac || !x || !y) return fail(PSK_ERR_ARG, "psk_spmv: NULL argument");
    psk_csr *A = const_cast<psk_csr *>(Ac);
    Context *c;
    PSK_TRY(ctx(&c));
    const double *dx = x;
    double *dy = y;
    DevBuf tmp;
    if (loc == PSK_HOST || A->comm) {
        PSK_TRY(tmp.ensure((size_t)(A->ncols + A->n) * sizeof(double)));
        double *tx = tmp.as<double>();
        const bool dry = A->comm && A->comm->dry;
        const int64_t nx = (A->comm && !dry) ? A->n : A->ncols;
        PSK_TRY(to_device_vec(x, loc, nx, tx, c->stream));
        if (A->comm) PSK_TRY(halo_exchange(A, tx, c->stream));
        dx = tx;
        dy = (loc == PSK_HOST) ? tx + A->ncols : y;
    }
    PSK_TRY(launch_spmv(A, kSpmvPlain, dx, dy, nullptr, nullptr, nullptr, nullptr, c->stream));
    if (loc == PSK_HOST) PSK_TRY(from_device_vec(dy, PSK_HOST, A->n, y, c->stream));
    PSK_HIP(hipStreamSynchronize(c->stream));
    tmp.release();
    return PSK_OK;
}

int psk_spmv_timed(const psk_csr *A, const double *x, double *y, int32_t reps, double *avg_ms) {
    if (!A || !x || !y || reps < 1 || !avg_ms) return fail(PSK_ERR_ARG, "psk_spmv_timed: bad arguments");
    if (A->comm) return fail(PSK_ERR_UNSUPPORTED, "psk_spmv_timed: sharded matrix");
    Context *c;
    PSK_TRY(ctx(&c));
    hipEvent_t e0, e1;
    PSK_HIP(hipEventCreateWithFlags(&e0, hipEventDisableSystemFence));
    PSK_HIP(hipEventCreateWithFlags(&e1, hipEventDisableSystemFence));
    constexpr int mode = kSpmvPlain;
    DevBuf part;
    if (mode == kSpmvDot) PSK_TRY(part.ensure(64));
    double *pp = mode == kSpmvDot ? part.as<double>() : nullptr;
    int rc = launch_spmv(A, mode, x, y, nullptr, nullptr, pp, nullptr, c->stream);
    if (rc == PSK_OK && hipEventRecord(e0, c->stream) != hipSuccess) rc = fail(PSK_ERR_HIP, "event record");
    for (int r = 0; r < reps && rc == PSK_OK; ++r)
        rc = launch_spmv(A, mode, x, y, nullptr, nullptr, pp, nullptr, c->stream);
    if (rc == PSK_OK && hipEventRecord(e1, c->stream) != hipSuccess) rc = fail(PSK_ERR_HIP, "event record");
    float ms = 0.f;
    if (rc == PSK_OK && hipEventSynchronize(e1) != hipSuccess) rc = fail(PSK_ERR_HIP, "event sync");
    if (rc == PSK_OK && hipEventElapsedTime(&ms, e0, e1) != hipSuccess) rc = fail(PSK_ERR_HIP, "event time");
    (void)hipEventDestroy(e0);
    (void)hipEventDestroy(e1);
    if (mode == kSpmvDot) (void)hipStreamSynchronize(c->stream);
    part.release();
    if (rc == PSK_OK) *avg_ms = (double)ms / reps;
    return rc;
}

}
```

### pysolvers_amd/csrc/spmv.hpp

```cpp
#pragma once
#include "psk_internal.hpp"

#include <hip/hip_ext.h>

#include <type_traits>

namespace psk {

constexpr int kSlice = kBlock;

__device__ __forceinline__ bool same_bits(double a, double b) {
    return __double_as_longlong(a) == __double_as_longlong(b);
}

struct SpmvLaunch {
    const double *x;
    double *y;
    const double *aux_d, *aux_q;
    GridSum gs;
    const int32_t *done;
    hipStream_t s;
    hipEvent_t ev0, ev1;
    bool rev;
    int64_t nwg;
};
struct SpmvFlush;
int launch_spmv_csr(const psk_csr *A, int mode, const SpmvLaunch &L);
int launch_spmv_sliced(const psk_csr *A, int mode, const SpmvLaunch &L);
int launch_spmv_diag(const psk_csr *A, int mode, const SpmvLaunch &L, const SpmvFlush *flush);

int sliced_build(psk_csr *A, hipStream_t s, bool force, bool pack, bool use_dict, bool force_dict);
void sliced_free(psk_csr *A);
int sliced_shape(const psk_csr *A, hipStream_t s, int32_t *width, int32_t *span);
int diag_build(psk_csr *A, hipStream_t s, bool force);
void diag_free(psk_csr *A);

template <int V>
using SpmvInt = std::integral_constant<int, V>;
template <class F>
int spmv_for_mode(int mode, F &&f) {
    switch (mode) {
    case kSpmvPlain: f(SpmvInt<kSpmvPlain>{}); break;
    case kSpmvDot: f(SpmvInt<kSpmvDot>{}); break;
    case kSpmvJacobiDot: f(SpmvInt<kSpmvJacobiDot>{}); break;
    case kSpmvPlainDot: f(SpmvInt<kSpmvPlainDot>{}); break;
    case kSpmvResid: f(SpmvInt<kSpmvResid>{}); break;
    case kSpmvAdd: f(SpmvInt<kSpmvAdd>{}); break;
    default:
        return fail(PSK_ERR_ARG, "unknown spmv mode");
    }
    PSK_HIP(hipGetLastError());
    return PSK_OK;
}


__device__ __forceinline__ int32_t ld_stream(const int32_t *p) { return __builtin_nontemporal_load(p); }
__device__ __forceinline__ double ld_stream(const double *p) { return __builtin_nontemporal_load(p); }

template <int MODE>
__device__ __forceinline__ bool spmv_publishes(const GridSum &gs) {
    return MODE != kSpmvPlain && MODE != kSpmvAdd && (MODE != kSpmvResid || gs.out != nullptr);
}
template <int MODE>
__device__ __forceinline__ uint32_t spmv_begin(const GridSum &gs, GridSumTile<1> &L, int64_t t) {
    return spmv_publishes<MODE>(gs) ? gridsum_tile_begin<1>(gs, L, t) : 0u;
}
__device__ __forceinline__ void spmv_publish(const GridSum &gs, GridSumTile<1> &L, double acc, uint32_t ticket,
                                             int64_t t) {
    const double ws = wave_total(acc);
    gridsum_tile_publish<1>(gs, L, &ws, ticket, t);
}

template <int MODE>
__device__ __forceinline__ double spmv_row_value(bool has, double sum, double eq, double &acc) {
    const double yv = MODE == kSpmvResid ? eq - sum : MODE == kSpmvAdd ? eq + sum : sum;
    acc = 0.0;
    if (has && MODE != kSpmvPlain && MODE != kSpmvAdd) acc = MODE == kSpmvResid ? yv * yv : eq * sum;
    return yv;
}
template <int MODE>
__device__ __forceinline__ void spmv_store_row(bool has, int64_t row, double yv, double *__restrict__ y) {
    if (!has) return;
    if (MODE == kSpmvResid || MODE == kSpmvAdd) y[row] = yv;
    else __builtin_nontemporal_store(yv, y + row);
}

template <int TPW>
__device__ __forceinline__ void spmv_publish_multi(const GridSum &gs, GridSumTile<1> *L, const double *acc,
                                                   const uint32_t *ticket, const int64_t *tl, const bool *tv) {
    const bool lane0 = (threadIdx.x & 63) == 0;
    const int wave = __builtin_amdgcn_readfirstlane(threadIdx.x >> 6);
    bool mine[TPW];
    uint32_t tk[TPW];
#pragma unroll
    for (int q = 0; q < TPW; ++q) {
        mine[q] = false;
        tk[q] = 0;
        if (!tv[q]) continue;
        const double ws = wave_total(acc[q]);
        uint32_t old = 0;
        if (lane0) {
            L[q].part[wave] = ws;
            if (threadIdx.x == 0) L[q].ticket = ticket[q];
            __builtin_amdgcn_fence(__ATOMIC_RELEASE, "workgroup", "local");
            old = atomicAdd(&L[q].cnt, 1u);
        }
        if (__builtin_amdgcn_readfirstlane(old) != kWaves - 1) continue;
// ... 32 lines not shown
```

### pysolvers_amd/csrc/spmv_csr.hip

```cpp
#include "spmv.hpp"

namespace psk {

template <int MODE>
__global__ __launch_bounds__(kBlock) void spmv_kernel(
    int64_t n, int trows, const int32_t *__restrict__ rowptr, const int32_t *__restrict__ colidx,
    const double *__restrict__ vals, const double *__restrict__ x, double *__restrict__ y,
    const double *__restrict__ aux_d, const double *__restrict__ aux_q, GridSum gs,
    const int32_t *__restrict__ done, int32_t nnz, TileMap tm) {
    if (done != nullptr && *done != 0) return;
    constexpr int KU = kChunk / kBlock;
    __shared__ double prod[kChunk + kBlock];
    const int tid = threadIdx.x;
    const int64_t t = tile_of_block(tm);
    const int64_t r0 = t * trows;
    const int64_t r1 = (r0 + trows < n) ? r0 + trows : n;
    const int32_t last = nnz > 0 ? nnz - 1 : 0;
    const int32_t e0 = rowptr[r0], e1 = rowptr[r1];
    int32_t cc[KU];
    double vv[KU];
    {
        const int32_t c1 = (e1 - e0 > kChunk) ? e0 + kChunk : e1;
        const int32_t base = e0 < last ? e0 : last;
#pragma unroll
        for (int k = 0; k < KU; ++k) {
            const int32_t e = e0 + k * kBlock + tid;
            const int32_t ee = e < c1 ? e : base;
            cc[k] = ld_stream(colidx + ee);
            vv[k] = ld_stream(vals + ee);
        }
    }
    __shared__ GridSumTile<1> gsl;
    const uint32_t ticket = spmv_begin<MODE>(gs, gsl, t);
    const int64_t row = r0 + tid;
    const bool has = tid < trows && row < r1;
    const int64_t rowc = has ? row : r0;
    const int32_t rs = rowptr[rowc], re = rowptr[rowc + 1];
    double eq = 0.0;
    if (MODE == kSpmvDot) eq = x[rowc];
    if (MODE == kSpmvResid || MODE == kSpmvAdd || MODE == kSpmvJacobiDot || MODE == kSpmvPlainDot)
        eq = aux_q[rowc];
    double sum = 0.0;
    {
        const int32_t c0 = e0, c1 = (e1 - c0 > kChunk) ? c0 + kChunk : e1;
        double pv[KU];
#pragma unroll
        for (int k = 0; k < KU; ++k) {
            double xx = x[cc[k]];
            if (MODE == kSpmvJacobiDot) xx = aux_d[cc[k]] * xx;
            pv[k] = vv[k] * xx;
        }
#pragma unroll
        for (int k = 0; k < KU; ++k) {
            const int32_t e = c0 + k * kBlock + tid;
            prod[(e < c1 ? k * kBlock : kChunk) + tid] = pv[k];
        }
        __syncthreads();
        const int32_t a = rs > c0 ? rs : c0;
        const int32_t bnd = re < c1 ? re : c1;
        if (has)
            for (int32_t e = a; e < bnd; ++e) sum = sum + prod[e - c0];
        __syncthreads();
    }
    for (int32_t c0 = e0 + kChunk; c0 < e1; c0 += kChunk) {
        const int32_t c1 = (e1 - c0 > kChunk) ? c0 + kChunk : e1;
        double pv[KU];
#pragma unroll
        for (int k = 0; k < KU; ++k) {
            const int32_t e = c0 + k * kBlock + tid;
            const int32_t ee = e < c1 ? e : c0;
            const int32_t c = ld_stream(colidx + ee);
            double xx = x[c];
            if (MODE == kSpmvJacobiDot) xx = aux_d[c] * xx;
            pv[k] = ld_stream(vals + ee) * xx;
        }
#pragma unroll
        for (int k = 0; k < KU; ++k) {
            const int32_t e = c0 + k * kBlock + tid;
            if (e < c1) prod[k * kBlock + tid] = pv[k];
        }
        __syncthreads();
        const int32_t a = rs > c0 ? rs : c0;
        const int32_t bnd = re < c1 ? re : c1;
        if (has)
            for (int32_t e = a; e < bnd; ++e) sum = sum + prod[e - c0];
        __syncthreads();
    }
    double acc;
    const double yv = spmv_row_value<MODE>(has, sum, eq, acc);
    if (spmv_publishes<MODE>(gs)) spmv_publish(gs, gsl, acc, ticket, t);
    spmv_store_row<MODE>(has, row, yv, y);
}

constexpr int64_t kCsrChunk = 128;

int launch_spmv_csr(const psk_csr *A, int mode, const SpmvLaunch &L) {
    const dim3 gd((unsigned)L.nwg), bd(kBlock);
    const TileMap tm = tile_map_chunked(L.nwg, kCsrChunk);
    const int tr = A->tile_rows;
    const int32_t nz = (int32_t)A->nnz;
    return spmv_for_mode(mode, [&](auto m) {
        hipExtLaunchKernelGGL(spmv_kernel<decltype(m)::value>, gd, bd, 0, L.s, L.ev0, L.ev1, 0, A->n, tr, A->rowptr,
                              A->colidx, A->vals, L.x, L.y, L.aux_d, L.aux_q, L.gs, L.done, nz, tm);
    });
}

}
```

### pysolvers_amd/csrc/spmv_diag.hip

```cpp
#include "spmv.hpp"
#include "pcg_state.hpp"

#include <algorithm>
#include <climits>

namespace psk {

static __device__ int32_t g_spmv_never_done = 0;

constexpr int kDiagMax = 8;
constexpr int kDiagTpw = 2;
struct DiagDesc {
    int32_t d[kDiagMax];
    double v[kDiagMax];
    int64_t lo, hi;
    int64_t ncols;
    int32_t K, jd;
};

__device__ __forceinline__ int64_t diag_col(const DiagDesc &dd, int64_t n, int64_t row, int j) {
    int64_t c = row + dd.d[j];
    c += c < 0 ? dd.lo : (c >= n ? dd.hi : 0);
    return c < 0 ? 0 : (c >= dd.ncols ? dd.ncols - 1 : c);
}

__device__ __forceinline__ int32_t spmv_vzero() {
    int32_t z;
    __asm__ volatile("v_mov_b32 %0, 0" : "=v"(z));
    return z;
}

template <bool SHR>
__device__ __forceinline__ double wave_shift1(double v, double edge) {
    constexpr int ctrl = SHR ? 0x138 : 0x130;
    const int lo = __builtin_amdgcn_update_dpp(__double2loint(edge), __double2loint(v), ctrl, 0xF, 0xF, false);
    const int hi = __builtin_amdgcn_update_dpp(__double2hiint(edge), __double2hiint(v), ctrl, 0xF, 0xF, false);
    return __hiloint2double(hi, lo);
}

__device__ __forceinline__ int64_t diag_col_off(const DiagDesc &dd, int64_t n, int64_t row, int64_t off) {
    int64_t c = row + off;
    c += c < 0 ? dd.lo : (c >= n ? dd.hi : 0);
    return c < 0 ? 0 : (c >= dd.ncols ? dd.ncols - 1 : c);
}

template <int MODE, int KM, int TPW, int NB = 0>
__global__ __launch_bounds__(kBlock) void spmv_diag_kernel(
    int64_t n, const uint8_t *__restrict__ mask, DiagDesc dd, const double *__restrict__ x, double *__restrict__ y,
    const double *__restrict__ aux_d, const double *__restrict__ aux_q, GridSum gs, const int32_t *__restrict__ done,
    TileMap tm, int64_t ntiles) {
    constexpr int JD = NB == 1 ? 0 : NB == 2 ? 2 : -1, JM1 = NB == 1 ? 3 : NB == 2 ? 1 : -1,
                  JP1 = NB == 1 ? 4 : NB == 2 ? 3 : -1;
    static_assert(NB == 0 || KM == 5, "NB: the 5-diagonal patterns only");
    const int32_t dnv = (done ? done : &g_spmv_never_done)[spmv_vzero()];
    const int tid = threadIdx.x;
    const int64_t grp = tile_of_block(tm);
    int64_t tl[TPW];
    bool tv[TPW];
    uint32_t mk[TPW];
    double xv[TPW][KM], eq[TPW], xe[TPW];
#pragma unroll
    for (int q = 0; q < TPW; ++q) {
        const int64_t t = grp * TPW + q;
        tv[q] = t < ntiles;
        tl[q] = tv[q] ? t : ntiles - 1;
        mk[q] = __builtin_nontemporal_load(mask + tl[q] * kSlice + tid);
    }
#pragma unroll
    for (int q = 0; q < TPW; ++q) {
        const int64_t row = tl[q] * kSlice + tid;
#pragma unroll
        for (int j = 0; j < KM; ++j) {
            if (NB && (j == JM1 || j == JP1)) continue;
            const int64_t c = diag_col(dd, n, row, j);
            xv[q][j] = x[c];
            if (MODE == kSpmvJacobiDot) xv[q][j] = aux_d[c] * xv[q][j];
        }
        if (NB) {
            const int lane = tid & 63;
            const int64_t c = diag_col_off(dd, n, row, lane == 0 ? -1 : (lane == 63 ? 1 : 0));
            xe[q] = x[c];
            if (MODE == kSpmvJacobiDot) xe[q] = aux_d[c] * xe[q];
        }
        eq[q] = 0.0;
        if (MODE == kSpmvResid || MODE == kSpmvAdd || MODE == kSpmvJacobiDot || MODE == kSpmvPlainDot)
            eq[q] = aux_q[row < n ? row : 0];
    }
    constexpr bool PUB = MODE != kSpmvPlain && MODE != kSpmvAdd;
    const bool pub = PUB && spmv_publishes<MODE>(gs);
    uint32_t ticket[TPW];
#pragma unroll
    for (int q = 0; q < TPW; ++q) {
        ticket[q] = 0;
        if (pub && tv[q] && gs.grp_log2 >= 0 && tid == 0)
            ticket[q] = gridsum_draw(gridsum_counter(gs, gridsum_group_of(tl[q], gs.grp_log2)));
    }
    if (__builtin_amdgcn_readfirstlane(dnv) != 0) {
#pragma unroll
        for (int q = 0; q < TPW; ++q) {
            __asm__ volatile("" ::"v"(mk[q]));
            if (NB) __asm__ volatile("" ::"v"(xe[q]));
#pragma unroll
            for (int j = 0; j < KM; ++j)
                if (!(NB && (j == JM1 || j == JP1))) __asm__ volatile("" ::"v"(xv[q][j]));
            if (pub && tv[q] && gs.grp_log2 >= 0 && tid == 0)
                __hip_atomic_fetch_sub(gridsum_counter(gs, gridsum_group_of(tl[q], gs.grp_log2)), 1u, __ATOMIC_RELAXED,
                                       __HIP_MEMORY_SCOPE_AGENT);
        }
        return;
    }
    __shared__ GridSumTile<1> gsl[TPW];
    if (pub) {
        if (tid < TPW) gsl[tid].cnt = 0;
        if (tid == 0 && blockIdx.x == 0 && (gs.nt + TPW - 1) / TPW != gridDim.x) atomicOr(gs.err, 2);
        __syncthreads();
    }
    double acc[TPW], yv[TPW];
    if (NB) {
#pragma unroll
        for (int q = 0; q < TPW; ++q) {
            xv[q][JM1] = wave_shift1<true>(xv[q][JD], xe[q]);
            xv[q][JP1] = wave_shift1<false>(xv[q][JD], xe[q]);
        }
    }
#pragma unroll
    for (int q = 0; q < TPW; ++q) {
        const int64_t row = tl[q] * kSlice + tid;
        const bool has = tv[q] && row < n;
        double sum = 0.0;
#pragma unroll
        for (int j = 0; j < KM; ++j) {
            const double t = sum + dd.v[j] * xv[q][j];
            sum = ((mk[q] >> j) & 1u) ? t : sum;
        }
        if (MODE == kSpmvDot) {
            double d = 0.0;
            bool found = false;
#pragma unroll
            for (int j = 0; j < KM; ++j) {
                const bool here = j == dd.jd && ((mk[q] >> j) & 1u);
                d = here ? xv[q][j] : d;
                found = found || here;
            }
            if (!found && has) d = x[row];
            eq[q] = d;
        }
        yv[q] = spmv_row_value<MODE>(has, sum, eq[q], acc[q]);
    }
    if (pub) spmv_publish_multi<TPW>(gs, gsl, acc, ticket, tl, tv);
#pragma unroll
    for (int q = 0; q < TPW; ++q) {
        const int64_t row = tl[q] * kSlice + tid;
        spmv_store_row<MODE>(tv[q] && row < n, row, yv[q], y);
    }
}


typedef double dv2u __attribute__((ext_vector_type(2), aligned(8)));
__device__ __forceinline__ dv2 ldu2(const double *p) {
    const dv2u v = *reinterpret_cast<const dv2u *>(p);
    return dv2{v.x, v.y};
}
__device__ __forceinline__ dv2 ldu2nt(const double *p) {
    const dv2u v = __builtin_nontemporal_load(reinterpret_cast<const dv2u *>(p));
    return dv2{v.x, v.y};
}
__device__ __forceinline__ void stu2(double *p, dv2 v) { *reinterpret_cast<dv2u *>(p) = dv2u{v.x, v.y}; }
__device__ __forceinline__ void stu2nt(double *p, dv2 v) {
    __builtin_nontemporal_store(dv2u{v.x, v.y}, reinterpret_cast<dv2u *>(p));
}

__device__ __forceinline__ double lane_f64(double x, int l) {
    return __hiloint2double(__builtin_amdgcn_readlane(__double2hiint(x), l),
                            __builtin_amdgcn_readlane(__double2loint(x), l));
}
__device__ __forceinline__ void diag_pair_totals(double v, double &t0, double &t1) {
    v += dpp_f64<0xB1>(v);
    v += dpp_f64<0x141>(v);
    v += dpp_f64<0x104>(v);
    t0 = ((lane_f64(v, 0) + lane_f64(v, 8)) + lane_f64(v, 16)) + lane_f64(v, 24);
    t1 = ((lane_f64(v, 32) + lane_f64(v, 40)) + lane_f64(v, 48)) + lane_f64(v, 56);
}

struct PairFix {
    int64_t c0, c1;
    bool bad;
};
__device__ __forceinline__ dv2 diag_pair_x(const DiagDesc &dd, int64_t n, int64_t r, int64_t d,
                                           const double *__restrict__ x, PairFix &f) {
    int64_t c0 = r + d, c1 = c0 + 1;
    c0 += c0 < 0 ? dd.lo : (c0 >= n ? dd.hi : 0);
    c1 += c1 < 0 ? dd.lo : (c1 >= n ? dd.hi : 0);
    f.bad = !(c1 == c0 + 1 && c0 >= 0 && c1 < dd.ncols);
    f.c0 = c0 < 0 ? 0 : (c0 >= dd.ncols ? dd.ncols - 1 : c0);
    f.c1 = c1 < 0 ? 0 : (c1 >= dd.ncols ? dd.ncols - 1 : c1);
    const int64_t a = c0 < 0 ? 0 : (c0 > dd.ncols - 2 ? dd.ncols - 2 : c0);
    return ldu2(x + a);
}
__device__ __forceinline__ void diag_pair_fix(dv2 &v, const PairFix &f, const double *__restrict__ x) {
    if (f.bad) {
        v.x = x[f.c0];
        v.y = x[f.c1];
    }
}

__host__ __device__ inline uint32_t spmv_flush_octets_before(const SpmvFlush &f, uint32_t o) {
    if (f.mul == 0) return o > f.ost ? o - f.ost : 0;
    return (uint32_t)(((uint64_t)o * f.mul) >> 16);
}
__device__ __forceinline__ const SpmvFlush &spmv_flush_arg(const SpmvFlush &f) { return f; }

template <int S>
__device__ __forceinline__ void spmv_flush_tile(const SpmvFlush &fl, uint32_t f, int64_t n) {
    const int64_t k = fl.k;
    const int blk = (int)(k % S);
    const PcgPend pd = pcg_flush_pending(S, blk, k, true);
    const int q = (int)(k - pd.first);
    const bool x0 = pd.first == 0;
    const int64_t i = ((int64_t)blk * pcg_block_tiles(fl.nv, S) + f) * kVecTile + 2 * threadIdx.x;
    double *__restrict__ x = fl.x;
    if (i + 1 < n) {
        dv2 xo{0.0, 0.0};
        if (!x0) xo = ld2nt(x + i);
        dv2 pp[S];
#pragma unroll
        for (int t = 1; t <= S; ++t)
            if (t <= q) pp[t - 1] = ld2nt(fl.pr.b[(k - t) % kPcgDefer] + i);
#pragma unroll
        for (int t = S; t >= 1; --t)
            if (t <= q) {
                const double a = fl.alphas[k - t];
                xo.x = xo.x + a * pp[t - 1].x;
                xo.y = xo.y + a * pp[t - 1].y;
            }
        st2nt(x + i, xo);
    } else if (i < n) {
        x[i] = pcg_catch_up(x0 ? 0.0 : x[i], &fl.pr, pd.first, k, fl.alphas, i);
    }
}

template <int MODE, int NB, typename... FLUSH>
__global__ __launch_bounds__(kBlock, (MODE != kSpmvPlain && MODE != kSpmvDot) ? 4 : 8) void spmv_diagp_kernel(
    int64_t n, const uint8_t *__restrict__ mask, DiagDesc dd, const double *__restrict__ x, double *__restrict__ y,
    const double *__restrict__ aux_d, const double *__restrict__ aux_q, GridSum gs, const int32_t *__restrict__ done,
    TileMap tm, int64_t ntiles, FLUSH... flush) {
    constexpr int KM = 5;
    constexpr int H = 2;
    constexpr bool FL = sizeof...(FLUSH) == 1;
    static_assert(sizeof...(FLUSH) <= 1 && (!FL || (MODE == kSpmvDot && kPcgStagger > 0)),
                  "the flush role rides on the PCG loop's launch only");
    static_assert(NB == 1 || NB == 2, "the 5-diagonal DPP orders");
    constexpr int JD = NB == 1 ? 0 : 2, JM1 = NB == 1 ? 3 : 1, JP1 = NB == 1 ? 4 : 3;
    constexpr int GD = NB == 1 ? 0 : 1;
    constexpr int TPB = kWaves;
    constexpr bool JX = MODE == kSpmvJacobiDot;
    constexpr bool EQ = MODE == kSpmvResid || MODE == kSpmvAdd || MODE == kSpmvJacobiDot || MODE == kSpmvPlainDot;
    const int32_t dnv = (done ? done : &g_spmv_never_done)[spmv_vzero()];
    const int lane = threadIdx.x & 63;
    const int wave = __builtin_amdgcn_readfirstlane(threadIdx.x >> 6);
    int64_t sidx = blockIdx.x, scnt = gridDim.x;
    if constexpr (FL) {
        const SpmvFlush &fl = spmv_flush_arg(flush...);
        const uint32_t o = blockIdx.x >> 3, fb = spmv_flush_octets_before(fl, o);
        if (spmv_flush_octets_before(fl, o + 1) != fb) {
            const uint32_t f = fb * 8 + (blockIdx.x & 7);
            if (f >= fl.nfl || __builtin_amdgcn_readfirstlane(dnv) != 0) return;
            spmv_flush_tile<kPcgStagger>(fl, f, n);
            return;
        }
        sidx = (int64_t)(o - fb) * 8 + (blockIdx.x & 7);
        scnt = (gs.nt + TPB - 1) / TPB;
        if (sidx >= scnt) return;
    }
    const int64_t grp = tile_of_index(tm, sidx, scnt);
    const int64_t t = grp * TPB + wave;
    const bool tv = t < ntiles;
    const int64_t tl = tv ? t : ntiles - 1;
    const int64_t r0 = tl * kSlice;
    uint32_t mk[H];
    dv2 xv[H][3], dg[H][3], eq[H];
    PairFix fx[H][3];
    double xe, de = 1.0;
#pragma unroll
    for (int h = 0; h < H; ++h) {
        const int64_t row = r0 + 128 * h + 2 * lane;
        mk[h] = __builtin_nontemporal_load(reinterpret_cast<const uint16_t *>(mask + row));
    }
#pragma unroll
    for (int h = 0; h < H; ++h) {
        const int64_t row = r0 + 128 * h + 2 * lane;
        int g = 0;
#pragma unroll
        for (int j = 0; j < KM; ++j) {
            if (j == JM1 || j == JP1) continue;
            xv[h][g] = diag_pair_x(dd, n, row, dd.d[j], x, fx[h][g]);
            if (JX) dg[h][g] = diag_pair_x(dd, n, row, dd.d[j], aux_d, fx[h][g]);
            ++g;
        }
        eq[h] = dv2{0.0, 0.0};
        if (EQ) eq[h] = ldu2(aux_q + (row + 1 < n ? row : (n >= 2 ? n - 2 : 0)));
    }
    {
        const int64_t er = lane == 0 ? r0 - 1 : (lane == 63 ? r0 + 128 * H : r0 + 2 * lane);
        const int64_t c = diag_col_off(dd, n, er, 0);
        xe = x[c];
        if (JX) de = aux_d[c];
    }
    constexpr bool PUB = MODE != kSpmvPlain && MODE != kSpmvAdd;
    const bool pub = PUB && spmv_publishes<MODE>(gs);
    uint32_t ticket = 0;
    if (pub && tv && gs.grp_log2 >= 0 && lane == 0)
        ticket = gridsum_draw(gridsum_counter(gs, gridsum_group_of(tl, gs.grp_log2)));
    if (__builtin_amdgcn_readfirstlane(dnv) != 0) {
#pragma unroll
        for (int h = 0; h < H; ++h) {
            __asm__ volatile("" ::"v"(mk[h]));
#pragma unroll
            for (int g = 0; g < 3; ++g) {
                __asm__ volatile("" ::"v"(xv[h][g].x), "v"(xv[h][g].y));
                if (JX) __asm__ volatile("" ::"v"(dg[h][g].x), "v"(dg[h][g].y));
            }
            if (EQ) __asm__ volatile("" ::"v"(eq[h].x), "v"(eq[h].y));
        }
        __asm__ volatile("" ::"v"(xe), "v"(de));
        if (pub && tv && gs.grp_log2 >= 0 && lane == 0)
            __hip_atomic_fetch_sub(gridsum_counter(gs, gridsum_group_of(tl, gs.grp_log2)), 1u, __ATOMIC_RELAXED,
                                   __HIP_MEMORY_SCOPE_AGENT);
        return;
    }
    if constexpr (FL) {
        const SpmvFlush &fl = spmv_flush_arg(flush...);
        const uint32_t ot = gridDim.x >> 3;
        if (pub && threadIdx.x == 0 && sidx == 0 &&
            ((gridDim.x & 7) != 0 || (scnt + 7) / 8 != (int64_t)(ot - spmv_flush_octets_before(fl, ot))))
            atomicOr(gs.err, 2);
    } else {
        if (pub && threadIdx.x == 0 && blockIdx.x == 0 && (gs.nt + TPB - 1) / TPB != gridDim.x) atomicOr(gs.err, 2);
    }
#pragma unroll
    for (int h = 0; h < H; ++h)
#pragma unroll
        for (int g = 0; g < 3; ++g) {
            diag_pair_fix(xv[h][g], fx[h][g], x);
            if (JX) {
                diag_pair_fix(dg[h][g], fx[h][g], aux_d);
                xv[h][g].x = dg[h][g].x * xv[h][g].x;
                xv[h][g].y = dg[h][g].y * xv[h][g].y;
            }
        }
    if (JX) xe = de * xe;
// ... 6 lines not shown
    double acc[H];
    dv2 yv[H];
#pragma unroll
    for (int h = 0; h < H; ++h) {
        const int64_t row = r0 + 128 * h + 2 * lane;
        double c0[KM], c1[KM];
        int g = 0;
#pragma unroll
        for (int j = 0; j < KM; ++j) {
            if (j == JM1) {
                c0[j] = xl[h];
                c1[j] = xv[h][GD].x;
            } else if (j == JP1) {
                c0[j] = xv[h][GD].y;
                c1[j] = xr[h];
            } else {
                c0[j] = xv[h][g].x;
                c1[j] = xv[h][g].y;
                ++g;
            }
        }
        const uint32_t m0 = mk[h] & 0xffu, m1 = mk[h] >> 8;
        double s0 = 0.0, s1 = 0.0;
#pragma unroll
        for (int j = 0; j < KM; ++j) {
            const double u0 = s0 + dd.v[j] * c0[j], u1 = s1 + dd.v[j] * c1[j];
            s0 = ((m0 >> j) & 1u) ? u0 : s0;
            s1 = ((m1 >> j) & 1u) ? u1 : s1;
        }
        const bool has0 = tv && row < n, has1 = tv && row + 1 < n;
        double e0 = eq[h].x, e1 = eq[h].y;
        if (EQ && row + 1 >= n) {
            e0 = eq[h].y;
            e1 = 0.0;
        }
        if (MODE == kSpmvDot) {
            const bool f0 = (m0 >> JD) & 1u, f1 = (m1 >> JD) & 1u;
            e0 = f0 ? c0[JD] : 0.0;
            e1 = f1 ? c1[JD] : 0.0;
            if (!f0 && has0) e0 = x[row];
            if (!f1 && has1) e1 = x[row + 1];
        }
        double a0, a1;
        yv[h].x = spmv_row_value<MODE>(has0, s0, e0, a0);
        yv[h].y = spmv_row_value<MODE>(has1, s1, e1, a1);
        acc[h] = a0 + a1;
    }
    if (pub && tv) {
        double w[2 * H];
#pragma unroll
        for (int h = 0; h < H; ++h) diag_pair_totals(acc[h], w[2 * h], w[2 * h + 1]);
        const double s = ((w[0] + w[1]) + w[2]) + w[3];
        const uint32_t tk = __builtin_amdgcn_readfirstlane(ticket);
        if (gs.grp_log2 < 0) {
            if (lane == 0) gridsum_put(gs.gslots + tl, s);
            gridsum_final_wave<1>(gs);
        } else {
            if (lane == 0) gridsum_put(gs.slots + gridsum_slot(gs, tl), s);
            const int64_t g = gridsum_group_of(tl, gs.grp_log2);
            int64_t base;
            const int64_t cnt = gridsum_members(gs, g, base);
            if (tk == (uint32_t)(cnt - 1)) {
                double r[1];
                gridsum_take<1, 64>(gs.slots, g << gs.grp_log2, cnt, gs.err, nullptr, r);
                if (lane == 0) {
                    gridsum_reset(gridsum_counter(gs, g));
                    gridsum_put(gs.gslots + g, r[0]);
                }
                gridsum_final_wave<1>(gs);
            }
        }
    }
#pragma unroll
    for (int h = 0; h < H; ++h) {
        const int64_t row = r0 + 128 * h + 2 * lane;
        if (!tv || row >= n) continue;
        if (row + 1 < n) {
            if (MODE == kSpmvResid || MODE == kSpmvAdd) stu2(y + row, yv[h]);
            else stu2nt(y + row, yv[h]);
        } else {
            spmv_store_row<MODE>(true, row, yv[h].x, y);
        }
    }
}

template <int NB>
__global__ __launch_bounds__(kBlock) void pcg_init_diag_kernel(int64_t n, const uint8_t *__restrict__ mask, DiagDesc dd,
                                                               const double *__restrict__ b, double xs,
                                                               double *__restrict__ p, double *__restrict__ y,
                                                               GridSum gs, PcgInitFin fin, TileMap tm, int64_t ntiles) {
    constexpr int TPW = kDiagTpw, KM = 5;
    static_assert(NB == 1 || NB == 2, "the DPP orders of spmv_diag_kernel");
    constexpr int JD = NB == 1 ? 0 : 2, JM1 = NB == 1 ? 3 : 1, JP1 = NB == 1 ? 4 : 3;
    const int tid = threadIdx.x, lane = tid & 63;
    const int64_t grp = tile_of_block(tm);
    int64_t tl[TPW];
    bool tv[TPW];
    uint32_t mk[TPW];
    double xv[TPW][KM], xe[TPW];
#pragma unroll
    for (int q = 0; q < TPW; ++q) {
        const int64_t t = grp * TPW + q;
        tv[q] = t < ntiles;
        tl[q] = tv[q] ? t : ntiles - 1;
        mk[q] = __builtin_nontemporal_load(mask + tl[q] * kSlice + tid);
    }
#pragma unroll
    for (int q = 0; q < TPW; ++q) {
        const int64_t row = tl[q] * kSlice + tid;
#pragma unroll
        for (int j = 0; j < KM; ++j) {
            if (j == JM1 || j == JP1) continue;
            xv[q][j] = b[diag_col(dd, n, row, j)];
        }
        xe[q] = b[diag_col_off(dd, n, row, lane == 0 ? -1 : (lane == 63 ? 1 : 0))];
    }
    uint32_t ticket[TPW];
#pragma unroll
    for (int q = 0; q < TPW; ++q) {
        ticket[q] = 0;
        if (tv[q] && gs.grp_log2 >= 0 && tid == 0)
            ticket[q] = gridsum_draw(gridsum_counter(gs, gridsum_group_of(tl[q], gs.grp_log2)));
    }
    __shared__ GridSumTile<3> gsl[TPW];
    if (tid < TPW) gsl[tid].cnt = 0;
    if (tid == 0 && blockIdx.x == 0 && (gs.nt + TPW - 1) / TPW != gridDim.x) atomicOr(gs.err, 2);
    __syncthreads();
    double acc[TPW][3], yv[TPW], pv[TPW];
#pragma unroll
    for (int q = 0; q < TPW; ++q) {
        const int64_t row = tl[q] * kSlice + tid;
        const bool has = tv[q] && row < n;
        const double braw = xv[q][JD];
#pragma unroll
        for (int j = 0; j < KM; ++j)
            if (j != JM1 && j != JP1) xv[q][j] = xs * xv[q][j];
        xe[q] = xs * xe[q];
        xv[q][JM1] = wave_shift1<true>(xv[q][JD], xe[q]);
        xv[q][JP1] = wave_shift1<false>(xv[q][JD], xe[q]);
        double sum = 0.0;
#pragma unroll
        for (int j = 0; j < KM; ++j) {
            const double t = sum + dd.v[j] * xv[q][j];
            sum = ((mk[q] >> j) & 1u) ? t : sum;
        }
        pv[q] = xv[q][JD];
        yv[q] = sum;
        acc[q][0] = has ? pv[q] * sum : 0.0;
        acc[q][1] = has ? braw * braw : 0.0;
        acc[q][2] = has ? pv[q] * braw : 0.0;
    }
    gridsum_tiles_publish<TPW, 3>(gs, gsl, acc, ticket, tl, tv, fin);
#pragma unroll
    for (int q = 0; q < TPW; ++q) {
        const int64_t row = tl[q] * kSlice + tid;
        if (tv[q] && row < n) {
            __builtin_nontemporal_store(yv[q], y + row);
            p[row] = pv[q];
        }
    }
}



__global__ __launch_bounds__(kBlock) void diag_detect_kernel(int64_t n, const int32_t *__restrict__ rowptr,
                                                             const int32_t *__restrict__ colidx,
                                                             const double *__restrict__ vals, DiagDesc dd,
                                                             uint8_t *__restrict__ mask, int64_t npad,
                                                             int32_t *__restrict__ bad) {
    const int64_t row = (int64_t)blockIdx.x * kBlock + threadIdx.x;
    if (row >= npad) return;
    uint32_t mk = 0;
    if (row < n) {
        int j = 0;
        bool ok = true;
        for (int32_t e = rowptr[row]; e < rowptr[row + 1] && ok; ++e) {
            const int64_t c = colidx[e];
            const double v = vals[e];
            while (j < dd.K) {
                int64_t cj = row + dd.d[j];
                cj += cj < 0 ? dd.lo : (cj >= n ? dd.hi : 0);
                if (cj == c && same_bits(v, dd.v[j])) break;
                ++j;
            }
            if (j == dd.K) ok = false;
            else mk |= 1u << j++;
        }
        if (!ok) atomicOr(bad, 1);
    }
    mask[row] = (uint8_t)mk;
}

void diag_free(psk_csr *A) {
    if (A->dg_mask) (void)hipFree(A->dg_mask);
    A->dg_mask = nullptr;
    A->dg_K = 0;
    A->dg_jd = -1;
}

static DiagDesc diag_desc(const psk_csr *A) {
    DiagDesc dd{};
    for (int j = 0; j < kDiagMax; ++j) {
        dd.d[j] = A->dg_d[j];
        dd.v[j] = A->dg_v[j];
    }
    dd.lo = A->dg_lo;
    dd.hi = A->dg_hi;
    dd.ncols = A->ncols;
    dd.K = A->dg_K;
    dd.jd = A->dg_jd;
    return dd;
}

int diag_build(psk_csr *A, hipStream_t s, bool force) {
    auto no = [&](const char *why) { return force ? fail(PSK_ERR_UNSUPPORTED, std::string("diagonal layout: ") + why) : PSK_OK; };
    const int64_t n = A->n, nt = (n + kSlice - 1) / kSlice;
    if (n == 0 || A->nnz == 0) return no("empty matrix");
    if (nt > INT32_MAX) return no("too many slices");
    DevBuf tmp;
    DevBufRelease rel{tmp};
    PSK_TRY(tmp.ensure((size_t)nt * 2 * sizeof(int32_t) + 64));
    int32_t *dw = tmp.as<int32_t>(), *dspan = dw + nt;
    int32_t *dbad = dw + 2 * nt;
    PSK_TRY(sliced_shape(A, s, dw, dspan));
    std::vector<int32_t> wd((size_t)nt);
    PSK_HIP(hipMemcpyAsync(wd.data(), dw, (size_t)nt * sizeof(int32_t), hipMemcpyDeviceToHost, s));
    PSK_HIP(hipStreamSynchronize(s));
    const int32_t K = *std::max_element(wd.begin(), wd.end());
    if (K < 1 || K > kDiagMax) return no("rows wider than 8 entries");
    std::vector<int32_t> rp(kSlice + 1), cols(K);
    std::vector<double> vals(K);
    int64_t trow = -1;
    for (int64_t tries = 0, i = 0; i < nt && tries < 64 && trow < 0; ++i) {
        const int64_t t = (nt / 2 + i) % nt;
        if (wd[(size_t)t] != K) continue;
        ++tries;
        const int64_t r0 = t * kSlice, nr = std::min<int64_t>(kSlice, n - r0);
        PSK_HIP(hipMemcpy(rp.data(), A->rowptr + r0, (size_t)(nr + 1) * sizeof(int32_t), hipMemcpyDeviceToHost));
        for (int64_t r = 0; r < nr && trow < 0; ++r) {
            if (rp[(size_t)r + 1] - rp[(size_t)r] != K) continue;
            PSK_HIP(hipMemcpy(cols.data(), A->colidx + rp[(size_t)r], (size_t)K * 4, hipMemcpyDeviceToHost));
            bool owned = true;
            for (int j = 0; j < K; ++j) owned = owned && cols[(size_t)j] >= 0 && cols[(size_t)j] < n;
// ... 20 lines not shown
    dd.lo = halo > 0 ? n - dmin : 0;
    dd.hi = halo > 0 && halo == -2 * dmin ? -dmin : 0;
    dd.ncols = A->ncols;
    uint8_t *mask = nullptr;
    if (hipMalloc(&mask, (size_t)nt * kSlice) != hipSuccess) {
        (void)hipGetLastError();
        return force ? fail(PSK_ERR_ALLOC, "diagonal layout: hipMalloc") : PSK_OK;
    }
    PSK_HIP(hipMemsetAsync(dbad, 0, sizeof(int32_t), s));
    hipLaunchKernelGGL(diag_detect_kernel, dim3((unsigned)nt), dim3(kBlock), 0, s, n, A->rowptr, A->colidx, A->vals, dd,
                       mask, nt * kSlice, dbad);
    int32_t bad = 0;
    hipError_t e = hipGetLastError();
    if (e == hipSuccess) e = hipMemcpyAsync(&bad, dbad, sizeof(int32_t), hipMemcpyDeviceToHost, s);
    if (e == hipSuccess) e = hipStreamSynchronize(s);
    if (e != hipSuccess || bad) {
        (void)hipFree(mask);
        if (e != hipSuccess) return fail(PSK_ERR_HIP, std::string("diagonal layout: ") + hipGetErrorString(e));
        return no("an entry off the diagonals or with another value");
    }
    sliced_free(A);
    diag_free(A);
    A->dg_mask = mask;
    A->dg_K = K;
    A->dg_jd = dd.jd;
    for (int j = 0; j < kDiagMax; ++j) {
        A->dg_d[j] = j < K ? dd.d[j] : 0;
        A->dg_v[j] = j < K ? dd.v[j] : 0.0;
    }
    A->dg_lo = dd.lo;
    A->dg_hi = dd.hi;
    return PSK_OK;
}

static int diag_nb(const psk_csr *A) {
    if (!A->dg_mask || A->dg_K != 5) return 0;
    if (A->dg_d[0] == 0 && A->dg_d[3] == -1 && A->dg_d[4] == 1) return 1;
    if (A->dg_d[2] == 0 && A->dg_d[1] == -1 && A->dg_d[3] == 1) return 2;
    return 0;
}

static bool diag_pair_rows(const psk_csr *A) { return diag_nb(A) != 0 && A->n >= 2 && A->ncols >= 2; }

bool pcg_init_diag_eligible(const psk_csr *A) { return !A->comm && A->n > 0 && diag_nb(A) != 0; }
bool spmv_flush_eligible(const psk_csr *A) { return !A->comm && diag_pair_rows(A); }

static uint32_t spmv_flush_grid(SpmvFlush &fl, int64_t nwgp) {
    constexpr int S = kPcgStagger > 0 ? kPcgStagger : 1;
    const int64_t per = pcg_block_tiles(fl.nv, S), t0 = (fl.k % S) * per;
    const int64_t nf = std::min(fl.nv, t0 + per) - t0;
    fl.nfl = nf > 0 ? (uint32_t)nf : 0;
    if (fl.nfl == 0) return 0;
    const int64_t ost = (nwgp + 7) / 8, ofl = (nf + 7) / 8;
    if ((ost + ofl + 2) * 8 > (int64_t)INT32_MAX) return 0;
    fl.ost = (uint32_t)ost;
    fl.ofl = (uint32_t)ofl;
    uint32_t ot = (uint32_t)(ost + ofl);
    const int64_t mul = (ofl * 65536 + ot - 1) / ot;
    fl.mul = (uint32_t)std::min<int64_t>(std::max<int64_t>(mul, 1), 65535);
    while (ot < (uint32_t)(ost + ofl + 2) * 2 &&
           (spmv_flush_octets_before(fl, ot) < fl.ofl || ot - spmv_flush_octets_before(fl, ot) < fl.ost))
        ++ot;
    if (spmv_flush_octets_before(fl, ot) < fl.ofl || ot - spmv_flush_octets_before(fl, ot) != fl.ost) {
        fl.mul = 0;
        ot = (uint32_t)(ost + ofl);
    }
    return ot * 8;
}

int launch_spmv_diag(const psk_csr *A, int mode, const SpmvLaunch &L, const SpmvFlush *flush) {
    const DiagDesc dd = diag_desc(A);
    const dim3 bd(kBlock);
    const int nb = diag_nb(A);
    if (diag_pair_rows(A)) {
        const int64_t nwgp = (L.nwg + kWaves - 1) / kWaves;
        const dim3 gdp((unsigned)nwgp);
        const TileMap tmp = tile_map_for(nwgp, true, L.rev);
#if PSK_PCG_STAGGER_ON
        if (flush) {
            SpmvFlush fl = *flush;
            const uint32_t grid = spmv_flush_grid(fl, nwgp);
            if (fl.nfl > 0) {
                if (grid == 0) return fail(PSK_ERR_UNSUPPORTED, "launch_spmv: grid too large for the flush role");
                if (nb == 1)
                    hipExtLaunchKernelGGL((spmv_diagp_kernel<kSpmvDot, 1, SpmvFlush>), dim3(grid), bd, 0, L.s, L.ev0,
                                          L.ev1, 0, A->n, A->dg_mask, dd, L.x, L.y, L.aux_d, L.aux_q, L.gs, L.done, tmp,
                                          L.nwg, fl);
                else
                    hipExtLaunchKernelGGL((spmv_diagp_kernel<kSpmvDot, 2, SpmvFlush>), dim3(grid), bd, 0, L.s, L.ev0,
                                          L.ev1, 0, A->n, A->dg_mask, dd, L.x, L.y, L.aux_d, L.aux_q, L.gs, L.done, tmp,
                                          L.nwg, fl);
                PSK_HIP(hipGetLastError());
                return PSK_OK;
            }
        }
#endif
        return spmv_for_mode(mode, [&](auto m) {
            constexpr int M = decltype(m)::value;
            if (nb == 1)
                hipExtLaunchKernelGGL((spmv_diagp_kernel<M, 1>), gdp, bd, 0, L.s, L.ev0, L.ev1, 0, A->n, A->dg_mask, dd,
                                      L.x, L.y, L.aux_d, L.aux_q, L.gs, L.done, tmp, L.nwg);
            else
                hipExtLaunchKernelGGL((spmv_diagp_kernel<M, 2>), gdp, bd, 0, L.s, L.ev0, L.ev1, 0, A->n, A->dg_mask, dd,
                                      L.x, L.y, L.aux_d, L.aux_q, L.gs, L.done, tmp, L.nwg);
        });
    }
    const int64_t nwgd = (L.nwg + kDiagTpw - 1) / kDiagTpw;
    const dim3 gdd((unsigned)(nwgd > 0 ? nwgd : 1));
    const TileMap tmd = tile_map_for(nwgd, true, L.rev);
    return spmv_for_mode(mode, [&](auto m) {
        constexpr int M = decltype(m)::value;
        auto one_row = [&](auto kmc, auto nbc) {
            hipExtLaunchKernelGGL((spmv_diag_kernel<M, decltype(kmc)::value, kDiagTpw, decltype(nbc)::value>), gdd, bd,
                                  0, L.s, L.ev0, L.ev1, 0, A->n, A->dg_mask, dd, L.x, L.y, L.aux_d, L.aux_q, L.gs,
                                  L.done, tmd, L.nwg);
        };
        if (nb == 1) one_row(SpmvInt<5>{}, SpmvInt<1>{});
        else if (nb == 2) one_row(SpmvInt<5>{}, SpmvInt<2>{});
        else if (A->dg_K <= 3) one_row(SpmvInt<3>{}, SpmvInt<0>{});
        else if (A->dg_K <= 5) one_row(SpmvInt<5>{}, SpmvInt<0>{});
        else one_row(SpmvInt<8>{}, SpmvInt<0>{});
    });
}

int launch_pcg_init_diag(const psk_csr *A, const double *b, double xs, double *p, double *Ap, double *out3,
                         const PcgInitFin &fin, hipStream_t s) {
    if (!pcg_init_diag_eligible(A)) return fail(PSK_ERR_ARG, "launch_pcg_init_diag: not eligible");
    Context *c;
    PSK_TRY(ctx(&c));
    const int64_t nwg = (A->n + kSlice - 1) / kSlice, nwgd = (nwg + kDiagTpw - 1) / kDiagTpw;
    GridSum gs;
    PSK_TRY(gridsum_prepare(c, nwg, 3, out3, &gs));
    const DiagDesc dd = diag_desc(A);
    const TileMap tmd = tile_map_for(nwgd, true);
    if (diag_nb(A) == 1)
        hipLaunchKernelGGL(pcg_init_diag_kernel<1>, dim3((unsigned)nwgd), dim3(kBlock), 0, s, A->n, A->dg_mask, dd, b, xs,
                           p, Ap, gs, fin, tmd, nwg);
    else
        hipLaunchKernelGGL(pcg_init_diag_kernel<2>, dim3((unsigned)nwgd), dim3(kBlock), 0, s, A->n, A->dg_mask, dd, b, xs,
                           p, Ap, gs, fin, tmd, nwg);
    PSK_HIP(hipGetLastError());
    return PSK_OK;
}

}
```

### pysolvers_amd/csrc/spmv_sliced.hip

```cpp
#include "spmv.hpp"

#include <algorithm>
#include <climits>

namespace psk {

constexpr int kDictMax = 8;
constexpr int kDictCand = 64;
constexpr int kSliceRegs = 8;
constexpr int16_t kPad16 = INT16_MIN;
constexpr int64_t kMaxDelta16 = 32767;

__device__ __forceinline__ int64_t sliced_vpos(int64_t o, int j, int w, int l) {
    return (j | 1) < w ? o + (int64_t)(j & ~1) * kSlice + 2 * l + (j & 1) : o + (int64_t)j * kSlice + l;
}

__device__ __forceinline__ int32_t unpack_delta(int32_t row, int16_t d) { return d == kPad16 ? -1 : row + (int32_t)d; }

struct DictRegs {
    double d0, d1, d2, d3, d4, d5, d6, d7;
};

template <int DK>
__device__ __forceinline__ double dict_pick(const DictRegs dv, uint32_t idx) {
    if (DK == 2) return (idx & 1) ? dv.d1 : dv.d0;
    const double a0 = (idx & 1) ? dv.d1 : dv.d0, a1 = (idx & 1) ? dv.d3 : dv.d2;
    const double b0 = (idx & 2) ? a1 : a0;
    if (DK == 4) return b0;
    const double a2 = (idx & 1) ? dv.d5 : dv.d4, a3 = (idx & 1) ? dv.d7 : dv.d6;
    const double b1 = (idx & 2) ? a3 : a2;
    return (idx & 4) ? b1 : b0;
}

static __device__ int32_t g_spmv_never_done = 0;

template <int DK>
__device__ __forceinline__ DictRegs load_dict(const double *__restrict__ sdict) {
    DictRegs dv{};
    if (DK >= 2) {
        dv.d0 = sdict[0];
        dv.d1 = sdict[1];
    }
    if (DK >= 4) {
        dv.d2 = sdict[2];
        dv.d3 = sdict[3];
    }
    if (DK >= 8) {
        dv.d4 = sdict[4];
        dv.d5 = sdict[5];
        dv.d6 = sdict[6];
        dv.d7 = sdict[7];
    }
    return dv;
}

template <int NS>
__device__ __forceinline__ double diag_x(const int32_t *cc, const double *xv, int32_t row, const double *__restrict__ x,
                                         bool has) {
    double d = 0.0;
    bool found = false;
#pragma unroll
    for (int j = 0; j < NS; ++j)
        if (cc[j] == row) {
            d = xv[j];
            found = true;
        }
    if (!found && has) d = x[row];
    return d;
}

template <int MODE, int DK, int UW>
__global__ __launch_bounds__(kBlock) void spmv_uniform_kernel(
    int64_t n, const int32_t *__restrict__ spcol, const double *__restrict__ sval, const double *__restrict__ sdict,
    const double *__restrict__ x, double *__restrict__ y, const double *__restrict__ aux_d,
    const double *__restrict__ aux_q, GridSum gs, const int32_t *__restrict__ done, TileMap tm) {
    constexpr int NP = (UW + 1) / 2;
    constexpr int NI = DK > 0 ? (UW + 3) / 4 : 0;
    const int32_t dn = *(done ? done : &g_spmv_never_done);
    const int tid = threadIdx.x;
    const int64_t t = tile_of_block(tm), row = t * kSlice + tid;
    const bool has = row < n;
    const int32_t *pword = spcol + t * (int64_t)((NP + NI) * kSlice) + tid;
    uint32_t cw[NP], iw[NI > 0 ? NI : 1];
    double vv[UW];
#pragma unroll
    for (int p = 0; p < NP; ++p) cw[p] = (uint32_t)ld_stream(pword + p * kSlice);
    if (DK > 0) {
#pragma unroll
        for (int q = 0; q < NI; ++q) iw[q] = (uint32_t)ld_stream(pword + (NP + q) * kSlice);
    } else {
        const double *v0 = sval + t * (int64_t)(UW * kSlice);
#pragma unroll
        for (int p = 0; p < UW / 2; ++p) {
            const dv2 v2 = __builtin_nontemporal_load(reinterpret_cast<const dv2 *>(v0 + 2 * p * kSlice) + tid);
            vv[2 * p] = v2.x;
            vv[2 * p + 1] = v2.y;
        }
        if (UW & 1) vv[UW - 1] = ld_stream(v0 + (UW - 1) * kSlice + tid);
    }
    const int64_t rowc = has ? row : 0;
    double eq = 0.0;
    if (MODE == kSpmvResid || MODE == kSpmvAdd || MODE == kSpmvJacobiDot || MODE == kSpmvPlainDot) eq = aux_q[rowc];
    const DictRegs dv = load_dict<DK>(sdict);
    if (dn != 0) {
#pragma unroll
        for (int p = 0; p < NP; ++p) __asm__ volatile("" ::"v"(cw[p]));
        if (DK > 0) {
#pragma unroll
            for (int q = 0; q < NI; ++q) __asm__ volatile("" ::"v"(iw[q]));
        } else {
#pragma unroll
            for (int j = 0; j < UW; ++j) __asm__ volatile("" ::"v"(vv[j]));
        }
        return;
    }
    __shared__ GridSumTile<1> gsl;
    const uint32_t ticket = spmv_begin<MODE>(gs, gsl, t);
    const int32_t row32 = (int32_t)row;
    int32_t cc[UW];
    double xv[UW];
#pragma unroll
    for (int j = 0; j < UW; ++j) {
        cc[j] = unpack_delta(row32, (int16_t)((j & 1) ? (cw[j >> 1] >> 16) : (cw[j >> 1] & 0xffff)));
        const int32_t cl = cc[j] >= 0 ? cc[j] : 0;
        xv[j] = x[cl];
        if (MODE == kSpmvJacobiDot) xv[j] = aux_d[cl] * xv[j];
    }
    if (DK > 0) {
#pragma unroll
        for (int j = 0; j < UW; ++j) vv[j] = dict_pick<DK>(dv, (iw[j >> 2] >> (8 * (j & 3))) & 0xff);
    }
    double sum = 0.0;
#pragma unroll
    for (int j = 0; j < UW; ++j)
        if (cc[j] >= 0) sum = sum + vv[j] * xv[j];
    if (MODE == kSpmvDot) eq = diag_x<UW>(cc, xv, row32, x, has);
    double acc;
    const double yv = spmv_row_value<MODE>(has, sum, eq, acc);
    if (spmv_publishes<MODE>(gs)) spmv_publish(gs, gsl, acc, ticket, t);
    spmv_store_row<MODE>(has, row, yv, y);
}

template <int MODE, int DK, int UW, int TPW>
__global__ __launch_bounds__(kBlock) void spmv_uniform_multi_kernel(
    int64_t n, const int32_t *__restrict__ spcol, const double *__restrict__ sval, const double *__restrict__ sdict,
    const double *__restrict__ x, double *__restrict__ y, const double *__restrict__ aux_d,
    const double *__restrict__ aux_q, GridSum gs, const int32_t *__restrict__ done, TileMap tm, int64_t ntiles) {
    constexpr int NP = (UW + 1) / 2;
    static_assert(DK == 2 && (UW & 1), "compact stream: odd width, 2-entry dictionary");
    const int32_t dn = *(done ? done : &g_spmv_never_done);
    const int tid = threadIdx.x;
    const int64_t grp = tile_of_block(tm);
    int64_t tl[TPW];
    bool tv[TPW];
#pragma unroll
    for (int q = 0; q < TPW; ++q) {
        const int64_t t = grp * TPW + q;
        tv[q] = t < ntiles;
        tl[q] = tv[q] ? t : ntiles - 1;
    }
    uint32_t cw[TPW][NP];
    double vv[TPW][UW];
#pragma unroll
    for (int q = 0; q < TPW; ++q) {
        const int32_t *pword = spcol + tl[q] * (int64_t)(NP * kSlice) + tid;
#pragma unroll
        for (int p = 0; p < NP; ++p) cw[q][p] = (uint32_t)ld_stream(pword + p * kSlice);
    }
    double eq[TPW];
#pragma unroll
    for (int q = 0; q < TPW; ++q) {
        const int64_t row = tl[q] * kSlice + tid;
        eq[q] = 0.0;
        if (MODE == kSpmvResid || MODE == kSpmvAdd || MODE == kSpmvJacobiDot || MODE == kSpmvPlainDot)
            eq[q] = aux_q[row < n ? row : 0];
    }
    const DictRegs dv = load_dict<DK>(sdict);
    if (dn != 0) {
#pragma unroll
        for (int q = 0; q < TPW; ++q) {
#pragma unroll
            for (int p = 0; p < NP; ++p) __asm__ volatile("" ::"v"(cw[q][p]));
        }
        return;
    }
    constexpr bool PUB = MODE != kSpmvPlain && MODE != kSpmvAdd;
    __shared__ GridSumTile<1> gsl[TPW];
    uint32_t ticket[TPW];
    const bool pub = PUB && spmv_publishes<MODE>(gs);
    if (pub) {
        if (tid < TPW) gsl[tid].cnt = 0;
        if (tid == 0 && blockIdx.x == 0 && (gs.nt + TPW - 1) / TPW != gridDim.x) atomicOr(gs.err, 2);
        __syncthreads();
#pragma unroll
        for (int q = 0; q < TPW; ++q) {
            ticket[q] = 0;
            if (tv[q] && gs.grp_log2 >= 0 && tid == 0)
                ticket[q] = gridsum_draw(gridsum_counter(gs, gridsum_group_of(tl[q], gs.grp_log2)));
        }
    }
    int32_t cc[TPW][UW];
    double xv[TPW][UW], acc[TPW], yv[TPW];
#pragma unroll
    for (int q = 0; q < TPW; ++q) {
        const int32_t row32 = (int32_t)(tl[q] * kSlice + tid);
#pragma unroll
        for (int j = 0; j < UW; ++j) {
            cc[q][j] = unpack_delta(row32, (int16_t)((j & 1) ? (cw[q][j >> 1] >> 16) : (cw[q][j >> 1] & 0xffff)));
            const int32_t cl = cc[q][j] >= 0 ? cc[q][j] : 0;
            xv[q][j] = x[cl];
            if (MODE == kSpmvJacobiDot) xv[q][j] = aux_d[cl] * xv[q][j];
        }
    }
#pragma unroll
    for (int q = 0; q < TPW; ++q) {
        const int64_t row = tl[q] * kSlice + tid;
        const bool has = tv[q] && row < n;
#pragma unroll
        for (int j = 0; j < UW; ++j) vv[q][j] = dict_pick<DK>(dv, (cw[q][NP - 1] >> (16 + j)) & 1u);
        double sum = 0.0;
#pragma unroll
        for (int j = 0; j < UW; ++j)
            if (cc[q][j] >= 0) sum = sum + vv[q][j] * xv[q][j];
        if (MODE == kSpmvDot) eq[q] = diag_x<UW>(cc[q], xv[q], (int32_t)row, x, has);
        yv[q] = spmv_row_value<MODE>(has, sum, eq[q], acc[q]);
    }
    if (pub) spmv_publish_multi<TPW>(gs, gsl, acc, ticket, tl, tv);
#pragma unroll
    for (int q = 0; q < TPW; ++q) {
        const int64_t row = tl[q] * kSlice + tid;
        spmv_store_row<MODE>(tv[q] && row < n, row, yv[q], y);
    }
}

template <int MODE, int DK>
__global__ __launch_bounds__(kBlock) void spmv_sliced_kernel(
    int64_t n, const int64_t *__restrict__ soff, const int64_t *__restrict__ swoff, const int8_t *__restrict__ sfmt,
    const int32_t *__restrict__ scol, const int32_t *__restrict__ spcol, const double *__restrict__ sval,
    const double *__restrict__ sdict,
    const double *__restrict__ x, double *__restrict__ y, const double *__restrict__ aux_d,
    const double *__restrict__ aux_q, GridSum gs, const int32_t *__restrict__ done, TileMap tm) {
    if (done != nullptr && *done != 0) return;
    const int tid = threadIdx.x;
    const int64_t t = tile_of_block(tm), row = t * kSlice + tid;
    const bool has = row < n;
    const int64_t o = soff[t];
    const int w = (int)((soff[t + 1] - o) / kSlice);
    const bool packed = sfmt[t] != 0;
    const int64_t wo = swoff[t];
    const int32_t *pword = spcol + wo;
    const int32_t *vword = pword + (packed ? (int64_t)((w + 1) / 2) * kSlice : 0);
    const DictRegs dv = load_dict<DK>(sdict);
    __shared__ GridSumTile<1> gsl;
    const uint32_t ticket = spmv_begin<MODE>(gs, gsl, t);
    const int32_t row32 = (int32_t)row;
    double eq = 0.0;
    if (has) {
        if (MODE == kSpmvDot && w > kSliceRegs) eq = x[row];
        if (MODE == kSpmvResid || MODE == kSpmvAdd || MODE == kSpmvJacobiDot || MODE == kSpmvPlainDot)
            eq = aux_q[row];
    }
    double sum = 0.0;
    if (w <= kSliceRegs) {
        int32_t cc[kSliceRegs];
        double vv[kSliceRegs], xv[kSliceRegs];
#pragma unroll
        for (int j = 0; j < kSliceRegs; ++j) {
            cc[j] = -1;
            vv[j] = 0.0;
        }
        int32_t vw[kSliceRegs / 4];
        if (DK > 0) {
#pragma unroll
            for (int q = 0; q < kSliceRegs / 4; ++q) vw[q] = 4 * q < w ? ld_stream(vword + q * kSlice + tid) : 0;
        } else {
#pragma unroll
            for (int p = 0; p < kSliceRegs / 2; ++p) {
                if (2 * p + 1 < w) {
                    const dv2 v2 =
                        __builtin_nontemporal_load(reinterpret_cast<const dv2 *>(sval + o + 2 * p * kSlice) + tid);
                    vv[2 * p] = v2.x;
                    vv[2 * p + 1] = v2.y;
                } else if (2 * p < w) {
                    vv[2 * p] = ld_stream(sval + o + 2 * p * kSlice + tid);
                }
            }
        }
        if (packed) {
#pragma unroll
            for (int p = 0; p < kSliceRegs / 2; ++p)
                if (2 * p < w) {
                    const int32_t word = ld_stream(pword + p * kSlice + tid);
                    cc[2 * p] = unpack_delta(row32, (int16_t)(word & 0xffff));
                    cc[2 * p + 1] = unpack_delta(row32, (int16_t)(word >> 16));
                }
        } else {
#pragma unroll
            for (int j = 0; j < kSliceRegs; ++j)
                if (j < w) cc[j] = ld_stream(scol + o + j * kSlice + tid);
        }
        if (DK > 0) {
#pragma unroll
            for (int j = 0; j < kSliceRegs; ++j)
                if (j < w) vv[j] = dict_pick<DK>(dv, ((uint32_t)vw[j >> 2] >> (8 * (j & 3))) & 0xff);
        }
#pragma unroll
        for (int j = 0; j < kSliceRegs; ++j) {
            xv[j] = 0.0;
            if (cc[j] >= 0) {
                xv[j] = x[cc[j]];
                if (MODE == kSpmvJacobiDot) xv[j] = aux_d[cc[j]] * xv[j];
            }
        }
#pragma unroll
        for (int j = 0; j < kSliceRegs; ++j)
            if (cc[j] >= 0) sum = sum + vv[j] * xv[j];
        if (MODE == kSpmvDot) eq = diag_x<kSliceRegs>(cc, xv, row32, x, has);
    } else {
        for (int j = 0; j < w; ++j) {
            int32_t c;
            if (packed) {
                const int32_t word = ld_stream(pword + (int64_t)(j >> 1) * kSlice + tid);
                c = unpack_delta(row32, (int16_t)((j & 1) ? (word >> 16) : (word & 0xffff)));
            } else {
                c = ld_stream(scol + o + (int64_t)j * kSlice + tid);
            }
            if (c < 0) break;
            double xx = x[c];
            if (MODE == kSpmvJacobiDot) xx = aux_d[c] * xx;
            const double v =
                DK > 0 ? dict_pick<DK>(dv, ((uint32_t)ld_stream(vword + (int64_t)(j >> 2) * kSlice + tid) >> (8 * (j & 3))) &
                                               0xff)
                       : ld_stream(sval + sliced_vpos(o, j, w, tid));
            sum = sum + v * xx;
        }
    }
    double acc;
    const double yv = spmv_row_value<MODE>(has, sum, eq, acc);
    if (spmv_publishes<MODE>(gs)) spmv_publish(gs, gsl, acc, ticket, t);
    spmv_store_row<MODE>(has, row, yv, y);
}

__global__ __launch_bounds__(kBlock) void sliced_shape_kernel(int64_t n, const int32_t *__restrict__ rowptr,
                                                              const int32_t *__restrict__ colidx,
                                                              int32_t *__restrict__ width, int32_t *__restrict__ span) {
    __shared__ int32_t sh[2 * kWaves];
    const int64_t row = (int64_t)blockIdx.x * kSlice + threadIdx.x;
    int32_t len = 0, dmax = 0;
    if (row < n) {
        const int32_t a = rowptr[row], b = rowptr[row + 1];
        len = b - a;
        for (int32_t e = a; e < b; ++e) {
            int64_t d = (int64_t)colidx[e] - row;
            d = d < 0 ? -d : d;
            const int32_t ds = d > INT32_MAX ? INT32_MAX : (int32_t)d;
            dmax = ds > dmax ? ds : dmax;
        }
    }
#pragma unroll
    for (int o = 32; o > 0; o >>= 1) {
        const int32_t v = __shfl_xor(len, o, 64), u = __shfl_xor(dmax, o, 64);
        len = v > len ? v : len;
        dmax = u > dmax ? u : dmax;
    }
    if ((threadIdx.x & 63) == 0) {
        sh[threadIdx.x >> 6] = len;
        sh[kWaves + (threadIdx.x >> 6)] = dmax;
    }
    __syncthreads();
    if (threadIdx.x == 0) {
        int32_t m = sh[0], dm = sh[kWaves];
        for (int i = 1; i < kWaves; ++i) {
            m = sh[i] > m ? sh[i] : m;
            dm = sh[kWaves + i] > dm ? sh[kWaves + i] : dm;
        }
        width[blockIdx.x] = m;
        span[blockIdx.x] = dm;
    }
}

int sliced_shape(const psk_csr *A, hipStream_t s, int32_t *width, int32_t *span) {
    const int64_t nt = (A->n + kSlice - 1) / kSlice;
    hipLaunchKernelGGL(sliced_shape_kernel, dim3((unsigned)nt), dim3(kBlock), 0, s, A->n, A->rowptr, A->colidx, width,
                       span);
    PSK_HIP(hipGetLastError());
    return PSK_OK;
}

__global__ __launch_bounds__(kBlock) void dict_scan_kernel(int64_t nnz, const double *__restrict__ vals,
                                                           const double *__restrict__ dict, int nd,
                                                           int32_t *__restrict__ ncand, double *__restrict__ cand) {
    __shared__ double dl[kDictMax];
    if (threadIdx.x < nd) dl[threadIdx.x] = dict[threadIdx.x];
    __syncthreads();
    double mine = 0.0;
    bool has = false;
    for (int64_t i = (int64_t)blockIdx.x * kBlock + threadIdx.x; i < nnz; i += (int64_t)gridDim.x * kBlock) {
        const double v = vals[i];
        bool found = false;
        for (int k = 0; k < nd && !found; ++k) found = same_bits(v, dl[k]);
        if (!found) {
            mine = v;
            has = true;
            break;
        }
    }
    const uint64_t m = __ballot(has);
    if (m != 0 && (threadIdx.x & 63) == __builtin_ctzll(m)) {
        const int32_t slot = atomicAdd(ncand, 1);
        if (slot < kDictCand) cand[slot] = mine;
    }
}

__global__ __launch_bounds__(kBlock) void sliced_fill_kernel(int64_t n, const int32_t *__restrict__ rowptr,
                                                             const int32_t *__restrict__ colidx,
                                                             const double *__restrict__ vals,
                                                             const int64_t *__restrict__ soff,
                                                             const int64_t *__restrict__ swoff,
                                                             const int8_t *__restrict__ sfmt, int32_t *__restrict__ scol,
                                                             int32_t *__restrict__ spcol, double *__restrict__ sval,
                                                             const double *__restrict__ sdict, int nd,
                                                             int compact) {
    const int tid = threadIdx.x;
// ... 106 lines not shown
    PSK_TRY(tmp.ensure((size_t)nt * 2 * sizeof(int32_t)));
    int32_t *dw = tmp.as<int32_t>(), *dspan = dw + nt;
    PSK_TRY(sliced_shape(A, s, dw, dspan));
    std::vector<int32_t> wd((size_t)nt * 2);
    PSK_HIP(hipMemcpyAsync(wd.data(), tmp.p, (size_t)nt * 2 * sizeof(int32_t), hipMemcpyDeviceToHost, s));
    PSK_HIP(hipStreamSynchronize(s));
    int64_t wmax = 0, wsum = 0;
    bool all_pack = pack;
    for (int64_t t = 0; t < nt; ++t) {
        wmax = std::max<int64_t>(wmax, wd[(size_t)t]);
        wsum += wd[(size_t)t];
        all_pack = all_pack && wd[(size_t)(nt + t)] <= kMaxDelta16;
    }
    const bool uniform = all_pack && wmax > 0 && wmax <= kSliceRegs && wmax * nt * 100 <= wsum * 101;
    if (uniform)
        for (int64_t t = 0; t < nt; ++t) wd[(size_t)t] = (int32_t)wmax;
    const bool compact = uniform && !dict.empty() && dict.size() <= 2 && (wmax & 1) && wmax <= 15;
    std::vector<int64_t> off((size_t)nt + 1), woff((size_t)nt + 1);
    std::vector<int8_t> fmt((size_t)nt);
    off[0] = 0;
    woff[0] = 0;
    int64_t packed_slots = 0, col_bytes = 0, val_bytes = 0;
    for (int64_t t = 0; t < nt; ++t) {
        const int64_t w = wd[(size_t)t];
        off[(size_t)t + 1] = off[(size_t)t] + w * kSlice;
        fmt[(size_t)t] = (pack && wd[(size_t)(nt + t)] <= kMaxDelta16) ? 1 : 0;
        if (fmt[(size_t)t]) packed_slots += w * kSlice;
        col_bytes += (fmt[(size_t)t] ? 4 * ((w + 1) / 2) : 4 * w) * kSlice;
        val_bytes += (dict.empty() ? 8 * w : compact ? 0 : 4 * ((w + 3) / 4)) * kSlice;
        const int64_t words = (fmt[(size_t)t] ? (w + 1) / 2 : 0) + (dict.empty() || compact ? 0 : (w + 3) / 4);
        woff[(size_t)t + 1] = woff[(size_t)t] + words * kSlice;
    }
    const int64_t slots = off[(size_t)nt], nwords = woff[(size_t)nt];
    const int64_t wide_slots = slots - packed_slots;
    const int64_t stream = val_bytes + 8 * (int64_t)dict.size() + col_bytes + (uniform ? 0 : 17 * nt + 16);
    if (!force && stream > 12 * A->nnz + 4 * (A->n + 1)) return PSK_OK;
    const size_t ms = slots > 0 ? (size_t)slots : 1;
    bool ok = hipMalloc(&A->sl_off, (size_t)(nt + 1) * 8) == hipSuccess &&
              hipMalloc(&A->sl_woff, (size_t)(nt + 1) * 8) == hipSuccess &&
              hipMalloc(&A->sl_fmt, (size_t)nt) == hipSuccess;
    if (ok && dict.empty()) ok = hipMalloc(&A->sl_val, ms * 8) == hipSuccess;
    if (ok && wide_slots > 0) ok = hipMalloc(&A->sl_col, ms * 4) == hipSuccess;
    if (ok && nwords > 0) ok = hipMalloc(&A->sl_pcol, (size_t)nwords * 4) == hipSuccess;
    if (ok && !dict.empty()) ok = hipMalloc(&A->sl_dict, kDictMax * 8) == hipSuccess;
    if (!ok) {
        (void)hipGetLastError();
        sliced_free(A);
        return force ? fail(PSK_ERR_ALLOC, "sliced layout: hipMalloc") : PSK_OK;
    }
    PSK_HIP(hipMemcpyAsync(A->sl_off, off.data(), (size_t)(nt + 1) * 8, hipMemcpyHostToDevice, s));
    PSK_HIP(hipMemcpyAsync(A->sl_woff, woff.data(), (size_t)(nt + 1) * 8, hipMemcpyHostToDevice, s));
    PSK_HIP(hipMemcpyAsync(A->sl_fmt, fmt.data(), (size_t)nt, hipMemcpyHostToDevice, s));
    if (!dict.empty()) {
        std::vector<double> padded(dict);
        padded.resize(kDictMax, 0.0);
        PSK_HIP(hipMemcpyAsync(A->sl_dict, padded.data(), kDictMax * 8, hipMemcpyHostToDevice, s));
    }
    A->sl_dict_n = (int32_t)dict.size();
    A->sl_uniform_w = uniform ? (int32_t)wmax : 0;
    A->sl_compact = compact ? 1 : 0;
    hipLaunchKernelGGL(sliced_fill_kernel, dim3((unsigned)nt), dim3(kBlock), 0, s, A->n, A->rowptr, A->colidx, A->vals,
                       A->sl_off, A->sl_woff, A->sl_fmt, A->sl_col, A->sl_pcol, A->sl_val, A->sl_dict,
                       A->sl_dict_n, compact ? 1 : 0);
    PSK_HIP(hipGetLastError());
    PSK_HIP(hipStreamSynchronize(s));
    A->sl_slots = slots;
    A->sl_packed_slots = packed_slots;
    A->sl_stream_bytes = stream;
    (void)wide_slots;
    return PSK_OK;
}

int launch_spmv_sliced(const psk_csr *A, int mode, const SpmvLaunch &L) {
    const dim3 bd(kBlock);
    const int uw = A->sl_uniform_w;
    if (A->sl_compact) {
        const int64_t nwg2 = (L.nwg + 1) / 2;
        const dim3 gd2((unsigned)(nwg2 > 0 ? nwg2 : 1));
        const TileMap tm2 = tile_map_for(nwg2, true, L.rev);
        return spmv_for_mode(mode, [&](auto m) {
            auto go = [&](auto w) {
                hipExtLaunchKernelGGL((spmv_uniform_multi_kernel<decltype(m)::value, 2, decltype(w)::value, 2>), gd2,
                                      bd, 0, L.s, L.ev0, L.ev1, 0, A->n, A->sl_pcol, A->sl_val, A->sl_dict, L.x, L.y,
                                      L.aux_d, L.aux_q, L.gs, L.done, tm2, L.nwg);
            };
            switch (uw) {
            case 1: go(SpmvInt<1>{}); break;
            case 3: go(SpmvInt<3>{}); break;
            case 5: go(SpmvInt<5>{}); break;
            default: go(SpmvInt<7>{}); break;
            }
        });
    }
    const dim3 gd((unsigned)L.nwg);
    const TileMap tm = tile_map_for(L.nwg, true, L.rev);
    const int dk = !A->sl_dict ? 0 : A->sl_dict_n <= 2 ? 2 : A->sl_dict_n <= 4 ? 4 : 8;
    return spmv_for_mode(mode, [&](auto m) {
        auto with_dk = [&](auto dkc) {
            constexpr int M = decltype(m)::value, DK = decltype(dkc)::value;
            auto uni = [&](auto w) {
                hipExtLaunchKernelGGL((spmv_uniform_kernel<M, DK, decltype(w)::value>), gd, bd, 0, L.s, L.ev0, L.ev1, 0,
                                      A->n, A->sl_pcol, A->sl_val, A->sl_dict, L.x, L.y, L.aux_d, L.aux_q, L.gs, L.done,
                                      tm);
            };
            switch (uw) {
            case 0:
                hipExtLaunchKernelGGL((spmv_sliced_kernel<M, DK>), gd, bd, 0, L.s, L.ev0, L.ev1, 0, A->n, A->sl_off,
                                      A->sl_woff, A->sl_fmt, A->sl_col, A->sl_pcol, A->sl_val, A->sl_dict, L.x, L.y,
                                      L.aux_d, L.aux_q, L.gs, L.done, tm);
                break;
            case 1: uni(SpmvInt<1>{}); break;
            case 2: uni(SpmvInt<2>{}); break;
            case 3: uni(SpmvInt<3>{}); break;
            case 4: uni(SpmvInt<4>{}); break;
            case 5: uni(SpmvInt<5>{}); break;
            case 6: uni(SpmvInt<6>{}); break;
            case 7: uni(SpmvInt<7>{}); break;
            default: uni(SpmvInt<8>{}); break;
            }
        };
        switch (dk) {
        case 0: with_dk(SpmvInt<0>{}); break;
        case 2: with_dk(SpmvInt<2>{}); break;
        case 4: with_dk(SpmvInt<4>{}); break;
        default: with_dk(SpmvInt<8>{}); break;
        }
    });
}

}
```

Before: 7524.

## Replace hipEvent kernel timing with in-kernel wall-clock stamps harvested on device

Per-iteration SpMV timing and the loop timer switch from hipEvent records on the stream to in-kernel wall_clock64 stamps written into a strided device buffer. A device harvest kernel copies them to host-mapped memory, and the finish kernel computes the loop clock. The intent is to remove event-record and event-synchronize overhead from the solve loop, which otherwise adds stream bubbles and host syncs. In exchange every instrumented kernel carries extra stamp loads, stores and atomics. The measured loop time now comes from device clocks rather than events, so it changes how the benchmark's own metric is computed.

New measurement: 7431. 0.988x the previous value.

```diff
diff --git a/include/psk_lab.h b/include/psk_lab.h
--- a/include/psk_lab.h
+++ b/include/psk_lab.h
@@ -29,6 +29,8 @@
 int psk_lab_pcg_flush_schedule(int32_t S, int64_t nv, int64_t tile, int64_t k, int32_t in_spmv, int32_t *blk,
                                int64_t *first_last);
 int psk_lab_pcg_flush(int64_t n, int64_t k, int32_t stag, double *x, const double *ring, const double *alphas);
+int psk_lab_stamp_interval(const uint64_t *lo, const uint64_t *hi, int64_t stride, int32_t *lines, int32_t *touched,
+                           double *ms);
 #define PSK_LAB_SOLVER_PCG 0
 #define PSK_LAB_SOLVER_GMRES 1
 #define PSK_LAB_SOLVER_VCYCLE 2
diff --git a/pysolvers_amd/_native.py b/pysolvers_amd/_native.py
--- a/pysolvers_amd/_native.py
+++ b/pysolvers_amd/_native.py
@@ -151,6 +151,7 @@
     "psk_lab_pcg_staggers": (ctypes.c_int, [P, P, ctypes.POINTER(I32)]),
     "psk_lab_pcg_flush_schedule": (ctypes.c_int, [I32, I64, I64, I64, I32, ctypes.POINTER(I32), ctypes.POINTER(I64)]),
     "psk_lab_pcg_flush": (ctypes.c_int, [I64, I64, I32, P, P, P]),
+    "psk_lab_stamp_interval": (ctypes.c_int, [P, P, I64, ctypes.POINTER(I32), ctypes.POINTER(I32), ctypes.POINTER(F64)]),
     "psk_lab_solver_layout": (ctypes.c_int, [I32, I64, I64, I64, I64, I32, I32, ctypes.POINTER(I64),
                                             ctypes.POINTER(I32), ctypes.POINTER(I64)]),
     "psk_lab_gmres_internals": (ctypes.c_int, [P, I64, I32, I32, I32, P, P, P, P, P, P, P]),
diff --git a/pysolvers_amd/csrc/lab.hip b/pysolvers_amd/csrc/lab.hip
--- a/pysolvers_amd/csrc/lab.hip
+++ b/pysolvers_amd/csrc/lab.hip
@@ -338,6 +338,18 @@
     return PSK_OK;
 }
 
+extern "C" int psk_lab_stamp_interval(const uint64_t *lo, const uint64_t *hi, int64_t stride, int32_t *lines,
+                                      int32_t *touched, double *ms) {
+    using namespace psk;
+    if (!lo || !hi || stride < 1 || !lines || !touched || !ms)
+        return fail(PSK_ERR_ARG, "psk_lab_stamp_interval: bad arguments");
+    uint64_t ticks = 0;
+    *lines = kStampLines;
+    *touched = stamp_interval(lo, hi, stride, &ticks) ? 1 : 0;
+    *ms = *touched ? (double)ticks * kStampTickMs : 0.0;
+    return PSK_OK;
+}
+
 extern "C" int psk_lab_pcg_flush(int64_t n, int64_t k, int32_t stag, double *x, const double *ring,
                                  const double *alphas) {
     using namespace psk;
diff --git a/pysolvers_amd/csrc/pcg.hip b/pysolvers_amd/csrc/pcg.hip
--- a/pysolvers_amd/csrc/pcg.hip
+++ b/pysolvers_amd/csrc/pcg.hip
@@ -15,7 +15,8 @@
 __global__ __launch_bounds__(kBlock) void pcg_init_kernel(int64_t n, const double *__restrict__ b,
                                                           const double *__restrict__ dinv, double ds,
                                                           double *__restrict__ p, GridSum gs, PcgInitFin fin,
-                                                          int64_t ntiles) {
+                                                          int64_t ntiles, LaunchStamps st) {
+    const uint64_t st0 = stamp_open(st);
     constexpr int TPW = 2;
     const int tid = threadIdx.x;
     int64_t tl[TPW];
@@ -50,6 +51,7 @@
         gridsum_tiles_publish<TPW, 2>(gs, gsl, acc, ticket, tl, tv, fin);
     else
         gridsum_tiles_publish<TPW, 2>(gs, gsl, acc, ticket, tl, tv);
+    stamp_close_lo(st, st0);
 }
 
 __global__ void pcg_init_finish_kernel(const double *g, int P, double tau, PcgState *st, double *udr,
@@ -239,9 +241,28 @@
 
 constexpr int kPcgStateWords = (int)(sizeof(PcgState) / 8);
 constexpr int kPcgFinishWord = 8;
-static_assert(sizeof(PcgState) % 8 == 0 && kPcgFinishWord + kPcgStateWords + 1 <= 64, "SolveKit::hmap words");
+constexpr int kPcgClockWord = kPcgStateWords + 1;
+static_assert(sizeof(PcgState) % 8 == 0 && kPcgFinishWord + kPcgStateWords + 3 <= 64, "SolveKit::hmap words");
+struct PcgHarvest {
+    uint64_t *lo0, *hi0;
+    uint64_t *host;
+    int32_t at[kTimedSlots];
+};
 __global__ __launch_bounds__(kBlock) void pcg_finish_kernel(const PcgState *st, const uint32_t *cnt, const int32_t *err,
-                                                            int64_t *hw) {
+                                                            int64_t *hw, LaunchStamps t0, PcgHarvest hs) {
+    if (blockIdx.x > 0) {
+        const int slot = (int)blockIdx.x - 1;
+        const int32_t at = hs.at[slot];
+        if (at < 0) return;
+        constexpr int64_t region = (int64_t)kStampLines * kStampStride;
+        stamp_harvest(LaunchStamps{hs.lo0 + slot * region, hs.hi0 + slot * region}, hs.host + (int64_t)at * kStampBlockWords);
+        return;
+    }
+    __shared__ unsigned long long t0min;
+    if (threadIdx.x == 0) t0min = ~0ull;
+    uint64_t *t0w = t0.lo + threadIdx.x * kStampStride;
+    const uint64_t mine = __hip_atomic_load(t0w, __ATOMIC_RELAXED, __HIP_MEMORY_SCOPE_AGENT);
+    __hip_atomic_store(t0w, UINT64_MAX, __ATOMIC_RELAXED, __HIP_MEMORY_SCOPE_AGENT);
     constexpr int kPer = (kGridSumMaxGroups + kBlock) / kBlock;
     uint32_t v[kPer];
 #pragma unroll
@@ -253,6 +274,12 @@
 #pragma unroll
     for (int i = 0; i < kPer; ++i) any |= v[i];
     const bool bad = __syncthreads_or(any != 0);
+    atomicMin(&t0min, (unsigned long long)mine);
+    __syncthreads();
+    if (threadIdx.x == 0) {
+        __hip_atomic_store(hw + kPcgClockWord, (int64_t)t0min, __ATOMIC_RELAXED, __HIP_MEMORY_SCOPE_SYSTEM);
+        __hip_atomic_store(hw + kPcgClockWord + 1, (int64_t)wall_clock64(), __ATOMIC_RELAXED, __HIP_MEMORY_SCOPE_SYSTEM);
+    }
     if (threadIdx.x < kPcgStateWords)
         __hip_atomic_store(hw + threadIdx.x, reinterpret_cast<const int64_t *>(st)[threadIdx.x], __ATOMIC_RELAXED,
                            __HIP_MEMORY_SCOPE_SYSTEM);
@@ -262,17 +289,21 @@
 }
 
 __global__ __launch_bounds__(kBlock) void pcg_gen_init_kernel(int64_t n, const double *__restrict__ b,
-                                                              double *__restrict__ x, double *__restrict__ r) {
+                                                              double *__restrict__ x, double *__restrict__ r,
+                                                              LaunchStamps st) {
+    const uint64_t st0 = stamp_open(st);
     const int64_t i = (int64_t)blockIdx.x * kBlock + threadIdx.x;
     if (i < n) {
         r[i] = b[i];
         x[i] = 0.0;
     }
+    stamp_close_lo(st, st0);
 }
 
 __global__ __launch_bounds__(kBlock) void pcg_gen_init2_kernel(int64_t n, const double *__restrict__ r,
                                                                const double *__restrict__ u, double *__restrict__ p,
-                                                               GridSum gs, PcgInitFin fin) {
+                                                               GridSum gs, PcgInitFin fin, LaunchStamps st) {
+    const uint64_t st0 = stamp_open(st);
     __shared__ double sh[kWaves];
     const int64_t i = (int64_t)blockIdx.x * kVecTile + 2 * threadIdx.x;
     const uint32_t ticket = gridsum_ticket(gs);
@@ -285,6 +316,7 @@
     }
     const double v[2] = {block_sum(bb, sh), block_sum(ur, sh)};
     gridsum_publish<2>(gs, v, sh, ticket, fin);
+    stamp_close_lo(st, st0);
 }
 
 __global__ __launch_bounds__(kBlock) void pcg_dot_kernel(int64_t n, const double *__restrict__ a,
@@ -478,6 +510,8 @@
     else on(std::integral_constant<int, 0>{});
 }
 
+__global__ __launch_bounds__(kBlock) void pcg_stamp_harvest_kernel(LaunchStamps st, uint64_t *dst) { stamp_harvest(st, dst); }
+
 struct PcgTimers {
     SolveKit *kit;
     int S;
@@ -494,17 +528,14 @@
         }
         if (S) spmv_ms.assign((size_t)maxiter, -1.0f);
     }
+    int prepare(int64_t maxiter) { return S ? stamps_host_ensure(kit, (maxiter + S - 1) / S) : PSK_OK; }
     int sample(hipEvent_t a, hipEvent_t b, float *ms) {
         PSK_HIP(hipEventSynchronize(b));
         PSK_HIP(hipEventElapsedTime(ms, a, b));
         return PSK_OK;
     }
-    int harvest(int slot) {
-        if (tk[slot] < 0) return PSK_OK;
+    int harvest_events(int slot) {
         float ms = 0.f;
-        PSK_TRY(sample(kit->ta[slot], kit->tb[slot], &ms));
-        spmv_ms[(size_t)tk[slot]] = ms;
-        tk[slot] = -1;
         if (tgat[slot]) {
             PSK_TRY(sample(kit->ga[slot], kit->gb[slot], &ms));
             gat_sum += ms;
@@ -519,12 +550,41 @@
         }
         return PSK_OK;
     }
-    int begin(int64_t k, int *slot, bool *timed) {
+    LaunchStamps stamps(int slot) const { return kit->stamp_block(slot); }
+    int begin(int64_t k, int *slot, bool *timed, hipStream_t s) {
         *timed = S > 0 && k % S == 0 && !(skip0 && k == 0);
         *slot = (int)((k / (S > 0 ? S : 1)) % kTimedSlots);
         if (*timed) {
-            PSK_TRY(harvest(*slot));
+            if (tk[*slot] >= 0) {
+                hipLaunchKernelGGL(pcg_stamp_harvest_kernel, dim3(1), dim3(kBlock), 0, s, stamps(*slot),
+                                   kit->hstamps + (tk[*slot] / S) * kStampBlockWords);
+                PSK_HIP(hipGetLastError());
+                PSK_TRY(harvest_events(*slot));
+            }
             tk[*slot] = k;
+            spmv_ms[(size_t)k] = -2.0f;
+        }
+        return PSK_OK;
+    }
+    PcgHarvest pending() const {
+        PcgHarvest h;
+        const LaunchStamps b0 = kit->stamp_block(0);
+        h.lo0 = b0.lo;
+        h.hi0 = b0.hi;
+        h.host = kit->hstamps;
+        for (int i = 0; i < kTimedSlots; ++i) h.at[i] = S > 0 && tk[i] >= 0 ? (int32_t)(tk[i] / S) : -1;
+        return h;
+    }
+    int resolve() {
+        for (int i = 0; i < kTimedSlots; ++i) {
+            PSK_TRY(harvest_events(i));
+            tk[i] = -1;
+        }
+        for (size_t k = 0; S > 0 && k < spmv_ms.size(); k += (size_t)S) {
+            if (spmv_ms[k] != -2.0f) continue;
+            const uint64_t *w = kit->hstamps + (k / (size_t)S) * kStampBlockWords;
+            uint64_t ticks = 0;
+            spmv_ms[k] = stamp_interval(w, w + kStampLines, 1, &ticks) ? (float)((double)ticks * kStampTickMs) : -1.0f;
         }
         return PSK_OK;
     }
@@ -562,21 +622,22 @@
         r.bd = pl.gen ? w.Ap : w.r;
     }
     const uint64_t seq0 = pl.mbc ? mbox_next(pl.mbc, &gs0) : 0;
-    PSK_HIP(hipEventRecord(r.kit->ev0, s));
+    const LaunchStamps t0 = r.kit->stamp_block(kTimedSlots);
     if (pl.gen) {
         const unsigned nb = (unsigned)((n + kBlock - 1) / kBlock);
-        if (n > 0) hipLaunchKernelGGL(pcg_gen_init_kernel, dim3(nb), dim3(kBlock), 0, s, n, r.bd, w.x, w.r);
+        if (n > 0) hipLaunchKernelGGL(pcg_gen_init_kernel, dim3(nb), dim3(kBlock), 0, s, n, r.bd, w.x, w.r, t0);
         PSK_TRY(prec_apply_dev(r.M, n, w.r, w.u, s));
-        hipLaunchKernelGGL(pcg_gen_init2_kernel, dim3((unsigned)pl.nv), dim3(kBlock), 0, s, n, w.r, w.u, w.p, gs0, fin);
+        hipLaunchKernelGGL(pcg_gen_init2_kernel, dim3((unsigned)pl.nv), dim3(kBlock), 0, s, n, w.r, w.u, w.p, gs0, fin,
+                           t0);
     } else if (pl.init_diag) {
         PcgInitFin fin3 = fin;
         fin3.off = 1;
-        PSK_TRY(launch_pcg_init_diag(r.A, r.bd, pl.jac == 2 ? pl.ds : 1.0, w.p, w.Ap, w.part1, fin3, s));
+        PSK_TRY(launch_pcg_init_diag(r.A, r.bd, pl.jac == 2 ? pl.ds : 1.0, w.p, w.Ap, w.part1, fin3, s, t0));
     } else {
         const dim3 gi((unsigned)((pl.nsl + 1) / 2));
         pcg_dispatch(pl.jac, !pl.sharded, [&](auto J, auto FUSED) {
             hipLaunchKernelGGL((pcg_init_kernel<decltype(J)::value, decltype(FUSED)::value>), gi, dim3(kBlock), 0, s, n,
-                               r.bd, pl.dinv, pl.ds, w.p, gs0, fin, pl.nsl);
+                               r.bd, pl.dinv, pl.ds, w.p, gs0, fin, pl.nsl, t0);
         });
     }
     PSK_HIP(hipGetLastError());
@@ -614,7 +675,7 @@
     double *pn = pl.gen ? w.p : w.pr.b[(k + 1) % kPcgDefer];
     int slot;
     bool timed;
-    PSK_TRY(tm.begin(k, &slot, &timed));
+    PSK_TRY(tm.begin(k, &slot, &timed, s));
     if (r.halo_pending) {
         PSK_HIP(hipStreamWaitEvent(s, kit->ev_b, 0));
         r.halo_pending = false;
@@ -630,8 +691,9 @@
     uint64_t seq1 = 0;
     const SpmvFlush fl{w.x, w.alphas, w.pr, k, pl.nv, 0, 0, 0, 0};
     if (!(pl.init_diag && k == 0))
-        PSK_TRY(launch_spmv(A, kSpmvDot, pk, w.Ap, nullptr, nullptr, w.part1, &w.st->done, s, timed ? kit->ta[slot] : nullptr,
-                            timed ? kit->tb[slot] : nullptr, 0, pl.mbc ? &seq1 : nullptr, pl.stag && k >= 1 ? &fl : nullptr));
+        PSK_TRY(launch_spmv(A, kSpmvDot, pk, w.Ap, nullptr, nullptr, w.part1, &w.st->done, s, nullptr, nullptr, 0,
+                            pl.mbc ? &seq1 : nullptr, pl.stag && k >= 1 ? &fl : nullptr,
+                            timed ? tm.stamps(slot) : LaunchStamps{}));
     const TileMap tm2 = tile_map_for(pl.nv, false);
     if (pl.sharded) {
         hipEvent_t g0 = timed ? kit->ga[slot] : nullptr, g1 = timed ? kit->gb[slot] : nullptr;
@@ -679,16 +741,17 @@
     SolveKit *kit = r.kit;
     if (r.halo_pending) PSK_HIP(hipStreamWaitEvent(r.s, kit->ev_b, 0));
     r.halo_pending = false;
-    PSK_HIP(hipEventRecord(kit->ev1, r.s));
     int64_t *hw = kit->hmap + kPcgFinishWord;
-    hipLaunchKernelGGL(pcg_finish_kernel, dim3(1), dim3(kBlock), 0, r.s, r.w.st, r.c->gs_cnt, r.c->gs_err, hw);
+    hipLaunchKernelGGL(pcg_finish_kernel, dim3(tm.S > 0 ? 1 + kTimedSlots : 1), dim3(kBlock), 0, r.s, r.w.st, r.c->gs_cnt,
+                       r.c->gs_err, hw, kit->stamp_block(kTimedSlots), tm.pending());
     PSK_HIP(hipGetLastError());
     PSK_HIP(hipStreamSynchronize(r.s));
     std::memcpy(hs, hw, sizeof(PcgState));
     PSK_TRY(gridsum_check_result(r.c, (int32_t)hw[kPcgStateWords]));
     if (r.pl.gen) PSK_TRY(prec_check_error(r.M, r.s));
-    for (int i = 0; i < kTimedSlots; ++i) PSK_TRY(tm.harvest(i));
-    res->loop_ms = loop_ms(kit);
+    PSK_TRY(tm.resolve());
+    const uint64_t c0 = (uint64_t)hw[kPcgClockWord], c1 = (uint64_t)hw[kPcgClockWord + 1];
+    res->loop_ms = c0 != UINT64_MAX && c1 >= c0 ? (double)(c1 - c0) * kStampTickMs : 0.0;
     return PSK_OK;
 }
 
@@ -760,6 +823,7 @@
     if (pl.overlap) PSK_TRY(comm_stream(r.c, &r.cs));
     StampPoll poll(r.kit);
     PcgTimers tm(r.kit, r.ctl->time_kernels, pl.init_diag, pl.maxiter);
+    PSK_TRY(tm.prepare(pl.maxiter));
     PSK_TRY(pcg_init(r, poll, b, loc));
     int64_t launched = 0, nk = 0;
     for (int64_t k = 0; k < pl.maxiter; ++k) {
@@ -799,6 +863,7 @@
     if (rc != PSK_OK) {
         if (r.halo_pending) (void)hipStreamWaitEvent(r.s, r.kit->ev_b, 0);
         (void)hipStreamSynchronize(r.s);
+        if (r.kit) (void)stamps_arm(r.kit, r.s);
     }
     return rc;
 }
diff --git a/pysolvers_amd/csrc/pcg_state.hpp b/pysolvers_amd/csrc/pcg_state.hpp
--- a/pysolvers_amd/csrc/pcg_state.hpp
+++ b/pysolvers_amd/csrc/pcg_state.hpp
@@ -151,7 +151,7 @@
 bool pcg_staggers(const psk_csr *A, const psk_prec *M);
 int launch_pcg_flush(int64_t n, double *x, const PRing &pr, const double *alphas, int64_t k, bool stag, hipStream_t s);
 int launch_pcg_init_diag(const psk_csr *A, const double *b, double xs, double *p, double *Ap, double *out3,
-                         const PcgInitFin &fin, hipStream_t s);
+                         const PcgInitFin &fin, hipStream_t s, LaunchStamps st = LaunchStamps{});
 
 struct PcgView {
     int64_t n, ncols;
diff --git a/pysolvers_amd/csrc/psk_internal.hpp b/pysolvers_amd/csrc/psk_internal.hpp
--- a/pysolvers_amd/csrc/psk_internal.hpp
+++ b/pysolvers_amd/csrc/psk_internal.hpp
@@ -38,6 +38,16 @@
 
 constexpr int kPollSlots = 4;
 constexpr int kTimedSlots = 64;
+
+constexpr int kStampLines = 256;
+constexpr int kStampStride = 32;
+constexpr double kStampTickMs = 1e-5;
+constexpr int kStampBlockWords = 2 * kStampLines;
+struct LaunchStamps {
+    uint64_t *lo = nullptr;
+    uint64_t *hi = nullptr;
+};
+bool stamp_interval(const uint64_t *lo, const uint64_t *hi, int64_t stride, uint64_t *ticks);
 struct SolveKit {
     bool ready = false;
     uint64_t solve_gen = 0;
@@ -49,7 +59,16 @@
     bool timed_ready = false;
     hipEvent_t ta[kTimedSlots] = {}, tb[kTimedSlots] = {};
     hipEvent_t ga[kTimedSlots] = {}, gb[kTimedSlots] = {}, ha[kTimedSlots] = {}, hb[kTimedSlots] = {};
-};
+    uint64_t *stamps = nullptr;
+    uint64_t *hstamps = nullptr;
+    int64_t hstamps_blocks = 0;
+    LaunchStamps stamp_block(int i) const {
+        constexpr int64_t region = (int64_t)kStampLines * kStampStride;
+        return LaunchStamps{stamps + i * region, stamps + (kTimedSlots + 1 + i) * region};
+    }
+};
+int stamps_arm(SolveKit *kit, hipStream_t s);
+int stamps_host_ensure(SolveKit *kit, int64_t blocks);
 constexpr size_t kStageBytes = 4096;
 struct Context {
     int device = -1;
@@ -306,6 +325,41 @@
     __threadfence_system();
 }
 
+__device__ __forceinline__ uint64_t stamp_open(const LaunchStamps &st) {
+    return st.lo != nullptr ? (uint64_t)wall_clock64() : 0;
+}
+__device__ __forceinline__ uint64_t *stamp_line(uint64_t *words) {
+    return words + (blockIdx.x & (kStampLines - 1)) * kStampStride;
+}
+__device__ __forceinline__ uint64_t stamp_scalar(uint64_t t0) {
+    uint32_t a = (uint32_t)t0, b = (uint32_t)(t0 >> 32);
+    __asm__ volatile("" : "+s"(a), "+s"(b));
+    return ((uint64_t)b << 32) | a;
+}
+__device__ __forceinline__ void stamp_close_lo(const LaunchStamps &st, uint64_t t0) {
+    t0 = stamp_scalar(t0);
+    if (st.lo != nullptr && threadIdx.x == 0)
+        (void)__hip_atomic_fetch_min(stamp_line(st.lo), t0, __ATOMIC_RELAXED, __HIP_MEMORY_SCOPE_AGENT);
+}
+__device__ __forceinline__ void stamp_close(const LaunchStamps &st, uint64_t t0) {
+    t0 = stamp_scalar(t0);
+    if (st.lo != nullptr && threadIdx.x == 0) {
+        const uint64_t t1 = (uint64_t)wall_clock64();
+        (void)__hip_atomic_fetch_min(stamp_line(st.lo), t0, __ATOMIC_RELAXED, __HIP_MEMORY_SCOPE_AGENT);
+        (void)__hip_atomic_fetch_max(stamp_line(st.hi), t1, __ATOMIC_RELAXED, __HIP_MEMORY_SCOPE_AGENT);
+    }
+}
+__device__ __forceinline__ void stamp_harvest(const LaunchStamps &st, uint64_t *dst) {
+    const int t = threadIdx.x;
+    const uint64_t a = __hip_atomic_load(st.lo + t * kStampStride, __ATOMIC_RELAXED, __HIP_MEMORY_SCOPE_AGENT);
+    const uint64_t b = __hip_atomic_load(st.hi + t * kStampStride, __ATOMIC_RELAXED, __HIP_MEMORY_SCOPE_AGENT);
+    __hip_atomic_store(dst + t, a, __ATOMIC_RELAXED, __HIP_MEMORY_SCOPE_SYSTEM);
+    __hip_atomic_store(dst + kStampLines + t, b, __ATOMIC_RELAXED, __HIP_MEMORY_SCOPE_SYSTEM);
+    __hip_atomic_store(st.lo + t * kStampStride, UINT64_MAX, __ATOMIC_RELAXED, __HIP_MEMORY_SCOPE_AGENT);
+    __hip_atomic_store(st.hi + t * kStampStride, (uint64_t)0, __ATOMIC_RELAXED, __HIP_MEMORY_SCOPE_AGENT);
+}
+static_assert(kStampLines == kBlock, "stamp_harvest: one thread per line");
+
 constexpr int kGridSumLLog = 8;
 constexpr int64_t kGridSumL = (int64_t)1 << kGridSumLLog;
 constexpr int kGridSumCntStride = 64;
@@ -760,6 +814,6 @@
 int launch_spmv(const psk_csr *A, int mode, const double *x, double *y, const double *aux_d,
                 const double *aux_q, double *partial, const int32_t *done_flag, hipStream_t s,
                 hipEvent_t ev0 = nullptr, hipEvent_t ev1 = nullptr, int rev = 0, uint64_t *mail_seq = nullptr,
-                const SpmvFlush *flush = nullptr);
-
-}
+                const SpmvFlush *flush = nullptr, LaunchStamps stamps = LaunchStamps{});
+
+}
diff --git a/pysolvers_amd/csrc/runtime.hip b/pysolvers_amd/csrc/runtime.hip
--- a/pysolvers_amd/csrc/runtime.hip
+++ b/pysolvers_amd/csrc/runtime.hip
@@ -25,8 +25,42 @@
 static std::atomic<int> g_live_rccl{0};
 void rccl_comm_count(int delta) { g_live_rccl += delta; }
 
+bool stamp_interval(const uint64_t *lo, const uint64_t *hi, int64_t stride, uint64_t *ticks) {
+    uint64_t a = UINT64_MAX, b = 0;
+    for (int i = 0; i < kStampLines; ++i) {
+        a = lo[i * stride] < a ? lo[i * stride] : a;
+        b = hi[i * stride] > b ? hi[i * stride] : b;
+    }
+    if (a == UINT64_MAX || b == 0 || b < a) return false;
+    *ticks = b - a;
+    return true;
+}
+
+int stamps_arm(SolveKit *kit, hipStream_t s) {
+    const size_t region = (size_t)(kTimedSlots + 1) * kStampLines * kStampStride * sizeof(uint64_t);
+    PSK_HIP(hipMemsetAsync(kit->stamps, 0xFF, region, s));
+    PSK_HIP(hipMemsetAsync(reinterpret_cast<char *>(kit->stamps) + region, 0, region, s));
+    return PSK_OK;
+}
+
+int stamps_host_ensure(SolveKit *kit, int64_t blocks) {
+    if (blocks <= kit->hstamps_blocks) return PSK_OK;
+    if (blocks < kTimedSlots) blocks = kTimedSlots;
+    if (blocks < 2 * kit->hstamps_blocks) blocks = 2 * kit->hstamps_blocks;
+    if (kit->hstamps) PSK_HIP(hipHostFree(kit->hstamps));
+    kit->hstamps = nullptr;
+    kit->hstamps_blocks = 0;
+    PSK_HIP(hipHostMalloc(&kit->hstamps, (size_t)blocks * kStampBlockWords * sizeof(uint64_t), hipHostMallocCoherent));
+    kit->hstamps_blocks = blocks;
+    return PSK_OK;
+}
+
 int solve_kit(Context *c, bool timed, SolveKit **out) {
     SolveKit &k = c->kit;
+    if (!k.stamps) {
+        PSK_HIP(hipMalloc(&k.stamps, (size_t)2 * (kTimedSlots + 1) * kStampLines * kStampStride * sizeof(uint64_t)));
+        PSK_TRY(stamps_arm(&k, c->stream));
+    }
     if (!k.ready) {
         PSK_HIP(hipHostMalloc(&k.hmap, 64 * sizeof(int64_t), hipHostMallocCoherent));
         std::memset(k.hmap, 0, 64 * sizeof(int64_t));
@@ -284,6 +318,8 @@
             (void)hipHostFree(k.hmap);
             (void)hipHostFree(k.hstage);
         }
+        if (k.stamps) (void)hipFree(k.stamps);
+        if (k.hstamps) (void)hipHostFree(k.hstamps);
         if (k.timed_ready)
             for (int i = 0; i < kTimedSlots; ++i) {
                 (void)hipEventDestroy(k.ta[i]);
diff --git a/pysolvers_amd/csrc/spmv.hip b/pysolvers_amd/csrc/spmv.hip
--- a/pysolvers_amd/csrc/spmv.hip
+++ b/pysolvers_amd/csrc/spmv.hip
@@ -40,7 +40,7 @@
 
 int launch_spmv(const psk_csr *A, int mode, const double *x, double *y, const double *aux_d,
                 const double *aux_q, double *partial, const int32_t *done_flag, hipStream_t s, hipEvent_t ev0,
-                hipEvent_t ev1, int rev, uint64_t *mail_seq, const SpmvFlush *flush) {
+                hipEvent_t ev1, int rev, uint64_t *mail_seq, const SpmvFlush *flush, LaunchStamps stamps) {
     Context *c;
     PSK_TRY(ctx(&c));
     if (flush && (mode != kSpmvDot || !partial || !spmv_flush_eligible(A) || kPcgStagger == 0 || flush->k < 1))
@@ -61,7 +61,7 @@
         }
         return PSK_OK;
     }
-    const SpmvLaunch L{x, y, aux_d, aux_q, gs, done_flag, s, ev0, ev1, rev != 0, nwg};
+    const SpmvLaunch L{x, y, aux_d, aux_q, gs, done_flag, s, ev0, ev1, rev != 0, nwg, stamps};
     if (A->dg_mask) return launch_spmv_diag(A, mode, L, flush);
     if (A->sl_off) return launch_spmv_sliced(A, mode, L);
     return launch_spmv_csr(A, mode, L);
diff --git a/pysolvers_amd/csrc/spmv.hpp b/pysolvers_amd/csrc/spmv.hpp
--- a/pysolvers_amd/csrc/spmv.hpp
+++ b/pysolvers_amd/csrc/spmv.hpp
@@ -23,6 +23,7 @@
     hipEvent_t ev0, ev1;
     bool rev;
     int64_t nwg;
+    LaunchStamps st;
 };
 struct SpmvFlush;
 int launch_spmv_csr(const psk_csr *A, int mode, const SpmvLaunch &L);
diff --git a/pysolvers_amd/csrc/spmv_csr.hip b/pysolvers_amd/csrc/spmv_csr.hip
--- a/pysolvers_amd/csrc/spmv_csr.hip
+++ b/pysolvers_amd/csrc/spmv_csr.hip
@@ -7,7 +7,8 @@
     int64_t n, int trows, const int32_t *__restrict__ rowptr, const int32_t *__restrict__ colidx,
     const double *__restrict__ vals, const double *__restrict__ x, double *__restrict__ y,
     const double *__restrict__ aux_d, const double *__restrict__ aux_q, GridSum gs,
-    const int32_t *__restrict__ done, int32_t nnz, TileMap tm) {
+    const int32_t *__restrict__ done, int32_t nnz, TileMap tm, LaunchStamps st) {
+    const uint64_t st0 = stamp_open(st);
     if (done != nullptr && *done != 0) return;
     constexpr int KU = kChunk / kBlock;
     __shared__ double prod[kChunk + kBlock];
@@ -90,6 +91,7 @@
     const double yv = spmv_row_value<MODE>(has, sum, eq, acc);
     if (spmv_publishes<MODE>(gs)) spmv_publish(gs, gsl, acc, ticket, t);
     spmv_store_row<MODE>(has, row, yv, y);
+    stamp_close(st, st0);
 }
 
 constexpr int64_t kCsrChunk = 128;
@@ -101,7 +103,7 @@
     const int32_t nz = (int32_t)A->nnz;
     return spmv_for_mode(mode, [&](auto m) {
         hipExtLaunchKernelGGL(spmv_kernel<decltype(m)::value>, gd, bd, 0, L.s, L.ev0, L.ev1, 0, A->n, tr, A->rowptr,
-                              A->colidx, A->vals, L.x, L.y, L.aux_d, L.aux_q, L.gs, L.done, nz, tm);
+                              A->colidx, A->vals, L.x, L.y, L.aux_d, L.aux_q, L.gs, L.done, nz, tm, L.st);
     });
 }
 
diff --git a/pysolvers_amd/csrc/spmv_diag.hip b/pysolvers_amd/csrc/spmv_diag.hip
--- a/pysolvers_amd/csrc/spmv_diag.hip
+++ b/pysolvers_amd/csrc/spmv_diag.hip
@@ -48,7 +48,8 @@
 __global__ __launch_bounds__(kBlock) void spmv_diag_kernel(
     int64_t n, const uint8_t *__restrict__ mask, DiagDesc dd, const double *__restrict__ x, double *__restrict__ y,
     const double *__restrict__ aux_d, const double *__restrict__ aux_q, GridSum gs, const int32_t *__restrict__ done,
-    TileMap tm, int64_t ntiles) {
+    TileMap tm, int64_t ntiles, LaunchStamps st) {
+    const uint64_t st0 = stamp_open(st);
     constexpr int JD = NB == 1 ? 0 : NB == 2 ? 2 : -1, JM1 = NB == 1 ? 3 : NB == 2 ? 1 : -1,
                   JP1 = NB == 1 ? 4 : NB == 2 ? 3 : -1;
     static_assert(NB == 0 || KM == 5, "NB: the 5-diagonal patterns only");
@@ -153,6 +154,7 @@
         const int64_t row = tl[q] * kSlice + tid;
         spmv_store_row<MODE>(tv[q] && row < n, row, yv[q], y);
     }
+    stamp_close(st, st0);
 }
 
 
@@ -239,11 +241,13 @@
     }
 }
 
-template <int MODE, int NB, typename... FLUSH>
+template <int MODE, int NB, bool STAMP, typename... FLUSH>
 __global__ __launch_bounds__(kBlock, (MODE != kSpmvPlain && MODE != kSpmvDot) ? 4 : 8) void spmv_diagp_kernel(
     int64_t n, const uint8_t *__restrict__ mask, DiagDesc dd, const double *__restrict__ x, double *__restrict__ y,
     const double *__restrict__ aux_d, const double *__restrict__ aux_q, GridSum gs, const int32_t *__restrict__ done,
-    TileMap tm, int64_t ntiles, FLUSH... flush) {
+    TileMap tm, int64_t ntiles, LaunchStamps stamps, FLUSH... flush) {
+    const LaunchStamps st = STAMP ? stamps : LaunchStamps{};
+    const uint64_t st0 = stamp_open(st);
     constexpr int KM = 5;
     constexpr int H = 2;
     constexpr bool FL = sizeof...(FLUSH) == 1;
@@ -266,6 +270,7 @@
             const uint32_t f = fb * 8 + (blockIdx.x & 7);
             if (f >= fl.nfl || __builtin_amdgcn_readfirstlane(dnv) != 0) return;
             spmv_flush_tile<kPcgStagger>(fl, f, n);
+            stamp_close(st, st0);
             return;
         }
         sidx = (int64_t)(o - fb) * 8 + (blockIdx.x & 7);
@@ -438,13 +443,16 @@
             spmv_store_row<MODE>(true, row, yv[h].x, y);
         }
     }
+    stamp_close(st, st0);
 }
 
 template <int NB>
 __global__ __launch_bounds__(kBlock) void pcg_init_diag_kernel(int64_t n, const uint8_t *__restrict__ mask, DiagDesc dd,
                                                                const double *__restrict__ b, double xs,
                                                                double *__restrict__ p, double *__restrict__ y,
-                                                               GridSum gs, PcgInitFin fin, TileMap tm, int64_t ntiles) {
+                                                               GridSum gs, PcgInitFin fin, TileMap tm, int64_t ntiles,
+                                                               LaunchStamps st) {
+    const uint64_t st0 = stamp_open(st);
     constexpr int TPW = kDiagTpw, KM = 5;
     static_assert(NB == 1 || NB == 2, "the DPP orders of spmv_diag_kernel");
     constexpr int JD = NB == 1 ? 0 : 2, JM1 = NB == 1 ? 3 : 1, JP1 = NB == 1 ? 4 : 3;
@@ -515,6 +523,7 @@
             p[row] = pv[q];
         }
     }
+    stamp_close_lo(st, st0);
 }
 
 
@@ -701,14 +710,15 @@
             const uint32_t grid = spmv_flush_grid(fl, nwgp);
             if (fl.nfl > 0) {
                 if (grid == 0) return fail(PSK_ERR_UNSUPPORTED, "launch_spmv: grid too large for the flush role");
-                if (nb == 1)
-                    hipExtLaunchKernelGGL((spmv_diagp_kernel<kSpmvDot, 1, SpmvFlush>), dim3(grid), bd, 0, L.s, L.ev0,
-                                          L.ev1, 0, A->n, A->dg_mask, dd, L.x, L.y, L.aux_d, L.aux_q, L.gs, L.done, tmp,
-                                          L.nwg, fl);
-                else
-                    hipExtLaunchKernelGGL((spmv_diagp_kernel<kSpmvDot, 2, SpmvFlush>), dim3(grid), bd, 0, L.s, L.ev0,
-                                          L.ev1, 0, A->n, A->dg_mask, dd, L.x, L.y, L.aux_d, L.aux_q, L.gs, L.done, tmp,
-                                          L.nwg, fl);
+                auto go = [&](auto nbc, auto stc) {
+                    hipExtLaunchKernelGGL((spmv_diagp_kernel<kSpmvDot, decltype(nbc)::value, decltype(stc)::value, SpmvFlush>),
+                                          dim3(grid), bd, 0, L.s, L.ev0, L.ev1, 0, A->n, A->dg_mask, dd, L.x, L.y, L.aux_d,
+                                          L.aux_q, L.gs, L.done, tmp, L.nwg, L.st, fl);
+                };
+                if (nb == 1 && L.st.lo) go(SpmvInt<1>{}, std::true_type{});
+                else if (nb == 1) go(SpmvInt<1>{}, std::false_type{});
+                else if (L.st.lo) go(SpmvInt<2>{}, std::true_type{});
+                else go(SpmvInt<2>{}, std::false_type{});
                 PSK_HIP(hipGetLastError());
                 return PSK_OK;
             }
@@ -716,12 +726,19 @@
 #endif
         return spmv_for_mode(mode, [&](auto m) {
             constexpr int M = decltype(m)::value;
-            if (nb == 1)
-                hipExtLaunchKernelGGL((spmv_diagp_kernel<M, 1>), gdp, bd, 0, L.s, L.ev0, L.ev1, 0, A->n, A->dg_mask, dd,
-                                      L.x, L.y, L.aux_d, L.aux_q, L.gs, L.done, tmp, L.nwg);
-            else
-                hipExtLaunchKernelGGL((spmv_diagp_kernel<M, 2>), gdp, bd, 0, L.s, L.ev0, L.ev1, 0, A->n, A->dg_mask, dd,
-                                      L.x, L.y, L.aux_d, L.aux_q, L.gs, L.done, tmp, L.nwg);
+            auto go = [&](auto nbc, auto stc) {
+                hipExtLaunchKernelGGL((spmv_diagp_kernel<M, decltype(nbc)::value, decltype(stc)::value>), gdp, bd, 0, L.s,
+                                      L.ev0, L.ev1, 0, A->n, A->dg_mask, dd, L.x, L.y, L.aux_d, L.aux_q, L.gs, L.done, tmp,
+                                      L.nwg, L.st);
+            };
+            if (M == kSpmvDot && L.st.lo) {
+                if (nb == 1) go(SpmvInt<1>{}, std::bool_constant<M == kSpmvDot>{});
+                else go(SpmvInt<2>{}, std::bool_constant<M == kSpmvDot>{});
+            } else if (nb == 1) {
+                go(SpmvInt<1>{}, std::false_type{});
+            } else {
+                go(SpmvInt<2>{}, std::false_type{});
+            }
         });
     }
     const int64_t nwgd = (L.nwg + kDiagTpw - 1) / kDiagTpw;
@@ -732,7 +749,7 @@
         auto one_row = [&](auto kmc, auto nbc) {
             hipExtLaunchKernelGGL((spmv_diag_kernel<M, decltype(kmc)::value, kDiagTpw, decltype(nbc)::value>), gdd, bd,
                                   0, L.s, L.ev0, L.ev1, 0, A->n, A->dg_mask, dd, L.x, L.y, L.aux_d, L.aux_q, L.gs,
-                                  L.done, tmd, L.nwg);
+                                  L.done, tmd, L.nwg, L.st);
         };
         if (nb == 1) one_row(SpmvInt<5>{}, SpmvInt<1>{});
         else if (nb == 2) one_row(SpmvInt<5>{}, SpmvInt<2>{});
@@ -743,7 +760,7 @@
 }
 
 int launch_pcg_init_diag(const psk_csr *A, const double *b, double xs, double *p, double *Ap, double *out3,
-                         const PcgInitFin &fin, hipStream_t s) {
+                         const PcgInitFin &fin, hipStream_t s, LaunchStamps st) {
     if (!pcg_init_diag_eligible(A)) return fail(PSK_ERR_ARG, "launch_pcg_init_diag: not eligible");
     Context *c;
     PSK_TRY(ctx(&c));
@@ -754,10 +771,10 @@
     const TileMap tmd = tile_map_for(nwgd, true);
     if (diag_nb(A) == 1)
         hipLaunchKernelGGL(pcg_init_diag_kernel<1>, dim3((unsigned)nwgd), dim3(kBlock), 0, s, A->n, A->dg_mask, dd, b, xs,
-                           p, Ap, gs, fin, tmd, nwg);
+                           p, Ap, gs, fin, tmd, nwg, st);
     else
         hipLaunchKernelGGL(pcg_init_diag_kernel<2>, dim3((unsigned)nwgd), dim3(kBlock), 0, s, A->n, A->dg_mask, dd, b, xs,
-                           p, Ap, gs, fin, tmd, nwg);
+                           p, Ap, gs, fin, tmd, nwg, st);
     PSK_HIP(hipGetLastError());
     return PSK_OK;
 }
diff --git a/pysolvers_amd/csrc/spmv_sliced.hip b/pysolvers_amd/csrc/spmv_sliced.hip
--- a/pysolvers_amd/csrc/spmv_sliced.hip
+++ b/pysolvers_amd/csrc/spmv_sliced.hip
@@ -73,7 +73,8 @@
 __global__ __launch_bounds__(kBlock) void spmv_uniform_kernel(
     int64_t n, const int32_t *__restrict__ spcol, const double *__restrict__ sval, const double *__restrict__ sdict,
     const double *__restrict__ x, double *__restrict__ y, const double *__restrict__ aux_d,
-    const double *__restrict__ aux_q, GridSum gs, const int32_t *__restrict__ done, TileMap tm) {
+    const double *__restrict__ aux_q, GridSum gs, const int32_t *__restrict__ done, TileMap tm, LaunchStamps st) {
+    const uint64_t st0 = stamp_open(st);
     constexpr int NP = (UW + 1) / 2;
     constexpr int NI = DK > 0 ? (UW + 3) / 4 : 0;
     const int32_t dn = *(done ? done : &g_spmv_never_done);
@@ -139,13 +140,16 @@
     const double yv = spmv_row_value<MODE>(has, sum, eq, acc);
     if (spmv_publishes<MODE>(gs)) spmv_publish(gs, gsl, acc, ticket, t);
     spmv_store_row<MODE>(has, row, yv, y);
+    stamp_close(st, st0);
 }
 
 template <int MODE, int DK, int UW, int TPW>
 __global__ __launch_bounds__(kBlock) void spmv_uniform_multi_kernel(
     int64_t n, const int32_t *__restrict__ spcol, const double *__restrict__ sval, const double *__restrict__ sdict,
     const double *__restrict__ x, double *__restrict__ y, const double *__restrict__ aux_d,
-    const double *__restrict__ aux_q, GridSum gs, const int32_t *__restrict__ done, TileMap tm, int64_t ntiles) {
+    const double *__restrict__ aux_q, GridSum gs, const int32_t *__restrict__ done, TileMap tm, int64_t ntiles,
+    LaunchStamps st) {
+    const uint64_t st0 = stamp_open(st);
     constexpr int NP = (UW + 1) / 2;
     static_assert(DK == 2 && (UW & 1), "compact stream: odd width, 2-entry dictionary");
     const int32_t dn = *(done ? done : &g_spmv_never_done);
@@ -231,6 +235,7 @@
         const int64_t row = tl[q] * kSlice + tid;
         spmv_store_row<MODE>(tv[q] && row < n, row, yv[q], y);
     }
+    stamp_close(st, st0);
 }
 
 template <int MODE, int DK>
@@ -239,7 +244,8 @@
     const int32_t *__restrict__ scol, const int32_t *__restrict__ spcol, const double *__restrict__ sval,
     const double *__restrict__ sdict,
     const double *__restrict__ x, double *__restrict__ y, const double *__restrict__ aux_d,
-    const double *__restrict__ aux_q, GridSum gs, const int32_t *__restrict__ done, TileMap tm) {
+    const double *__restrict__ aux_q, GridSum gs, const int32_t *__restrict__ done, TileMap tm, LaunchStamps st) {
+    const uint64_t st0 = stamp_open(st);
     if (done != nullptr && *done != 0) return;
     const int tid = threadIdx.x;
     const int64_t t = tile_of_block(tm), row = t * kSlice + tid;
@@ -339,6 +345,7 @@
     const double yv = spmv_row_value<MODE>(has, sum, eq, acc);
     if (spmv_publishes<MODE>(gs)) spmv_publish(gs, gsl, acc, ticket, t);
     spmv_store_row<MODE>(has, row, yv, y);
+    stamp_close(st, st0);
 }
 
 __global__ __launch_bounds__(kBlock) void sliced_shape_kernel(int64_t n, const int32_t *__restrict__ rowptr,
@@ -611,7 +618,7 @@
             auto go = [&](auto w) {
                 hipExtLaunchKernelGGL((spmv_uniform_multi_kernel<decltype(m)::value, 2, decltype(w)::value, 2>), gd2,
                                       bd, 0, L.s, L.ev0, L.ev1, 0, A->n, A->sl_pcol, A->sl_val, A->sl_dict, L.x, L.y,
-                                      L.aux_d, L.aux_q, L.gs, L.done, tm2, L.nwg);
+                                      L.aux_d, L.aux_q, L.gs, L.done, tm2, L.nwg, L.st);
             };
             switch (uw) {
             case 1: go(SpmvInt<1>{}); break;
@@ -630,13 +637,13 @@
             auto uni = [&](auto w) {
                 hipExtLaunchKernelGGL((spmv_uniform_kernel<M, DK, decltype(w)::value>), gd, bd, 0, L.s, L.ev0, L.ev1, 0,
                                       A->n, A->sl_pcol, A->sl_val, A->sl_dict, L.x, L.y, L.aux_d, L.aux_q, L.gs, L.done,
-                                      tm);
+                                      tm, L.st);
             };
             switch (uw) {
             case 0:
                 hipExtLaunchKernelGGL((spmv_sliced_kernel<M, DK>), gd, bd, 0, L.s, L.ev0, L.ev1, 0, A->n, A->sl_off,
                                       A->sl_woff, A->sl_fmt, A->sl_col, A->sl_pcol, A->sl_val, A->sl_dict, L.x, L.y,
-                                      L.aux_d, L.aux_q, L.gs, L.done, tm);
+                                      L.aux_d, L.aux_q, L.gs, L.done, tm, L.st);
                 break;
             case 1: uni(SpmvInt<1>{}); break;
             case 2: uni(SpmvInt<2>{}); break;
```
